# georgesterpu/avsr-tf1

Measured on AMD Instinct MI355X. Metric: utterances/sec (train step) at B=64 T_a=500 T_v=75, higher is better.
Workload: dtype f32; 1 GPU; c4: AV dual-attention (bimodal) video 1x256 + audio 3x256 uni-LSTM, scaled_luong, B=64 T_a=500x80 T_v=75 L=40; utterances_per_gpu=64, global_batch=64, T_a=500, F_a=80, T_v=75, F_v=128, T_dec=40, parallelism=dp1, video_frontend=resnet_cnn, launch=hipgraph, dropout=True

## Files before the change

### avsr-tf1_amd/_lib.py

```python
import ctypes as C
import os

import torch

from . import build as _build

MAX_LAYERS = 4
MAX_MECH = 4
MAX_STACKS = 4

_fp = C.POINTER(C.c_float)
_ip = C.POINTER(C.c_int32)


class AvsrError(RuntimeError):
    pass


class Mat(C.Structure):
    _fields_ = [("ptr", C.c_void_p), ("ld", C.c_int64), ("T", C.c_int32), ("pad_", C.c_int32), ("ldo", C.c_int64)]


class GemmDesc(C.Structure):
    _fields_ = [("A", Mat), ("B", Mat), ("C", Mat), ("bias", C.c_void_p),
                ("M", C.c_int32), ("N", C.c_int32), ("K", C.c_int32),
                ("trans_a", C.c_int32), ("trans_b", C.c_int32),
                ("alpha", C.c_float), ("beta", C.c_float), ("batch", C.c_int32),
                ("stride_a", C.c_int64), ("stride_b", C.c_int64), ("stride_c", C.c_int64),
                ("alpha_dev", C.c_void_p),
                ("splitk", C.c_int32), ("pad_", C.c_int32),
                ("workspace", C.c_void_p), ("workspace_floats", C.c_int64),
                ("colsum", C.c_void_p), ("colsum_beta", C.c_float), ("pad2_", C.c_int32)]


class RnnLayer(C.Structure):
    _fields_ = [("units", C.c_int32), ("in_dim", C.c_int32), ("hoisted", C.c_int32), ("out_col", C.c_int32),
                ("wt", C.c_void_p), ("w", C.c_void_p), ("bias", C.c_void_p),
                ("gates", C.c_void_p), ("cs", C.c_void_p), ("out", C.c_void_p), ("ld_out", C.c_int64),
                ("state", C.c_void_p), ("h_final", C.c_void_p), ("c_final", C.c_void_p),
                ("dgates", C.c_void_p), ("dstate", C.c_void_p), ("dout", C.c_void_p), ("ld_dout", C.c_int64),
                ("dout_col", C.c_int32), ("residual", C.c_int32), ("hs_seq", C.c_void_p), ("xt_seq", C.c_void_p),
                ("wt2", C.c_void_p), ("w2", C.c_void_p), ("bias2", C.c_void_p), ("rh_seq", C.c_void_p), ("dgates2", C.c_void_p)]


class RnnStack(C.Structure):
    _fields_ = [("B", C.c_int32), ("T", C.c_int32), ("reverse", C.c_int32), ("n_layers", C.c_int32),
                ("cell", C.c_int32), ("pad_", C.c_int32),
                ("len", C.c_void_p), ("dh_final", C.c_void_p), ("dc_final", C.c_void_p),
                ("seed", C.c_void_p), ("keep_in", C.c_float), ("keep_state", C.c_float), ("keep_out", C.c_float),
                ("consumer_keep", C.c_float), ("cell_id_base", C.c_int32), ("consumer_stream", C.c_int32),
                ("consumer_width", C.c_int32), ("pad2_", C.c_int32),
                ("layer", RnnLayer * MAX_LAYERS)]


class RnnLaunch(C.Structure):
    _fields_ = [(n, C.c_int32) for n in ("form", "stacks", "rows_per_group", "rows_per_slice", "launches", "wg_per_xcd", "crossing_edges",
                                         "top_tiles")]


class AttnMech(C.Structure):
    _fields_ = [("type", C.c_int32), ("T", C.c_int32), ("D", C.c_int32), ("chunk", C.c_int32),
                ("len", C.c_void_p), ("keys", C.c_void_p), ("values", C.c_void_p),
                ("values_sb", C.c_int64), ("values_st", C.c_int64),
                ("g", C.c_void_p), ("v", C.c_void_p), ("bq", C.c_void_p),
                ("wq_t", C.c_void_p), ("wq", C.c_void_p), ("watt_t", C.c_void_p), ("watt", C.c_void_p),
                ("scores", C.c_void_p), ("ctx", C.c_void_p), ("pq", C.c_void_p), ("pstat", C.c_void_p),
                ("pctx", C.c_void_p), ("dscores", C.c_void_p), ("dctx", C.c_void_p), ("dpq", C.c_void_p),
                ("pdq", C.c_void_p)]


class DecLayer(C.Structure):
    _fields_ = [("wt", C.c_void_p), ("w", C.c_void_p), ("bias", C.c_void_p), ("gates", C.c_void_p), ("cs", C.c_void_p),
                ("out", C.c_void_p), ("state", C.c_void_p), ("hs_seq", C.c_void_p), ("xin_seq", C.c_void_p),
                ("dgates", C.c_void_p), ("dstate", C.c_void_p), ("cell_id", C.c_int32), ("pad_", C.c_int32),
                ("wt2", C.c_void_p), ("w2", C.c_void_p), ("bias2", C.c_void_p), ("rh_seq", C.c_void_p), ("dgates2", C.c_void_p)]


MAX_DEC_EXTRA = 3


class AttnRnn(C.Structure):
    _fields_ = [("B", C.c_int32), ("L", C.c_int32), ("H", C.c_int32), ("E", C.c_int32),
                ("n_mech", C.c_int32), ("output_attention", C.c_int32), ("V", C.c_int32), ("mode", C.c_int32),
                ("go_id", C.c_int32), ("eos_id", C.c_int32),
                ("steplen", C.c_void_p), ("wt", C.c_void_p), ("w", C.c_void_p), ("bias", C.c_void_p),
                ("gates", C.c_void_p), ("cs", C.c_void_p), ("cell_out", C.c_void_p), ("att", C.c_void_p),
                ("h0", C.c_void_p), ("c0", C.c_void_p), ("state", C.c_void_p),
                ("h_final", C.c_void_p), ("c_final", C.c_void_p),
                ("mech", AttnMech * MAX_MECH),
                ("embedding", C.c_void_p), ("wout_t", C.c_void_p), ("bout", C.c_void_p),
                ("logits", C.c_void_p), ("ids", C.c_void_p), ("tok", C.c_void_p), ("n_unfinished", C.c_void_p),
                ("dgates", C.c_void_p), ("dstate", C.c_void_p), ("datt", C.c_void_p), ("dq", C.c_void_p),
                ("datt_ext", C.c_void_p), ("dcell_ext", C.c_void_p), ("dh0", C.c_void_p), ("dc0", C.c_void_p),
                ("dh_final", C.c_void_p), ("dc_final", C.c_void_p),
                ("seed", C.c_void_p), ("keep_in", C.c_float), ("keep_state", C.c_float), ("keep_out", C.c_float),
                ("sampling_prob", C.c_float), ("cell_id", C.c_int32), ("pad3_", C.c_int32),
                ("hs_seq", C.c_void_p), ("attd", C.c_void_p), ("xs", C.c_void_p), ("labels", C.c_void_p), ("fed", C.c_void_p),
                ("cell", C.c_int32), ("pad4_", C.c_int32), ("wt2", C.c_void_p), ("w2", C.c_void_p), ("bias2", C.c_void_p),
                ("rh_seq", C.c_void_p), ("dgates2", C.c_void_p),
                ("beam_width", C.c_int32), ("mem_shared", C.c_int32), ("length_penalty", C.c_float), ("pad6_", C.c_float),
                ("beam_logp", C.c_void_p), ("beam_fin", C.c_void_p), ("beam_len", C.c_void_p), ("step_ids", C.c_void_p),
                ("parent_ids", C.c_void_p), ("parent_rows", C.c_void_p),
                ("n_extra", C.c_int32), ("prof_tag", C.c_int32), ("out0", C.c_void_p), ("extra", DecLayer * MAX_DEC_EXTRA),
                ("fused_ws", C.c_void_p), ("fused_ws_floats", C.c_int64)]


MAX_LM_LAYERS = 4


class BeamLm(C.Structure):
    _fields_ = [("n_layers", C.c_int32), ("H", C.c_int32), ("E", C.c_int32), ("V", C.c_int32),
                ("one_hot", C.c_int32), ("n_rows", C.c_int32), ("lm_weight", C.c_float), ("pad_", C.c_int32),
                ("embedding", C.c_void_p), ("wt", C.c_void_p * MAX_LM_LAYERS), ("bias", C.c_void_p * MAX_LM_LAYERS),
                ("wout_t", C.c_void_p), ("bout", C.c_void_p), ("state_c", C.c_void_p), ("state_h", C.c_void_p), ("lm_logp", C.c_void_p)]


BEAM_CTC_MAX_T, BEAM_CTC_MAX_V = 2048, 256


class BeamCtc(C.Structure):
    _fields_ = [("n_utt", C.c_int32), ("beam_width", C.c_int32), ("T", C.c_int32), ("V", C.c_int32), ("eos_id", C.c_int32),
                ("weight", C.c_float), ("ld", C.c_int64)] + \
               [(n, C.c_void_p) for n in ("z", "in_len", "y", "state", "psi", "last", "term", "extra", "lm_logp")] + \
               [("lm_weight", C.c_float), ("pad_", C.c_int32)]


class ConvDesc(C.Structure):
    _fields_ = [(n, C.c_int32) for n in ("N", "H", "W", "Ci", "Co", "k", "stride", "pad_t", "pad_l", "Ho", "Wo", "pad_")] + \
               [("bn_scale", C.c_void_p), ("bn_shift", C.c_void_p)]


class ConvLaunch(C.Structure):
    _fields_ = [(n, C.c_int32) for n in ("kernel", "m", "ntc", "ch4", "rs", "fold", "ep", "nsp", "ntap", "t0", "F", "grid", "CsP", "lds_bytes",
                                         "slab", "pad_")]


class Conv3dDesc(C.Structure):
    _fields_ = [(n, C.c_int32) for n in ("B", "T", "H", "W", "Ci", "Co", "kt", "kh", "kw", "stride", "pad_f", "pad_t", "pad_l", "Ho", "Wo",
                                         "relu")] + [("scale", C.c_void_p), ("shift", C.c_void_p)]


class LogmelArgs(C.Structure):
    _fields_ = [(n, C.c_int32) for n in ("B", "N", "T_out", "F", "frame_length", "frame_step", "fft_length", "num_mel_bins", "window", "stride",
                                         "mel_nnz", "pad_")] + \
               [(n, C.c_void_p) for n in ("wav", "wav_len", "hann", "twiddle", "mel_lo", "mel_cnt", "mel_ptr", "mel_w", "out", "out_len")]


SPEC_AUGMENT_MAX_MASKS, SPEC_AUGMENT_MAX_T = 8, 65535


class SpecAugmentArgs(C.Structure):
    _fields_ = [(n, C.c_int32) for n in ("B", "T", "F_in", "F", "freq_masks", "freq_width", "freq_bins", "time_masks", "time_width",
                                         "ratio_q16", "video", "mean_fill")] + [("ld", C.c_int64)] + \
               [(n, C.c_void_p) for n in ("x", "len", "seed", "y", "ws")] + [("ws_floats", C.c_int64)]


class CtcArgs(C.Structure):
    _fields_ = [("B", C.c_int32), ("T", C.c_int32), ("L", C.c_int32), ("C", C.c_int32), ("ld", C.c_int64)] + \
               [(n, C.c_void_p) for n in ("z", "labels", "labels_len", "in_len", "denom")] + [("weight", C.c_float), ("pad_", C.c_int32)] + \
               [(n, C.c_void_p) for n in ("nll", "status", "utt_loss", "dz", "ws")] + [("ws_floats", C.c_int64)]


CTC_PREFIX_MAX_V, CTC_PREFIX_MAX_W, CTC_PREFIX_MAX_L = 256, 64, 512


class CtcPrefixArgs(C.Structure):
    _fields_ = [(n, C.c_int32) for n in ("B", "T", "V", "beam_width", "L_max", "pad_")] + [("ld", C.c_int64)] + \
               [(n, C.c_void_p) for n in ("z", "in_len", "ids", "lens", "score", "trace_parent", "trace_sym", "trace_pb", "trace_pnb")]


CTC_PREFIX_LM_MAX_W = 16


class CtcPrefixLm(C.Structure):
    _fields_ = [(n, C.c_int32) for n in ("n_layers", "H", "E", "V", "one_hot", "go_id", "eos_id")] + \
               [("weight", C.c_float), ("bonus", C.c_float), ("pad_", C.c_int32), ("embedding", C.c_void_p),
                ("wt", C.c_void_p * MAX_LM_LAYERS), ("bias", C.c_void_p * MAX_LM_LAYERS), ("wout_t", C.c_void_p), ("bout", C.c_void_p),
                ("ws", C.c_void_p), ("ws_bytes", C.c_int64), ("s_lm", C.c_void_p), ("lm_steps", C.c_void_p), ("lm_logp", C.c_void_p)]


CTC_PREFIX_NGRAM_MAX_ORDER = 16
CTC_PREFIX_NGRAM_MAX_NODES = 1 << 24
CTC_PREFIX_NGRAM_MAX_ARCS = 1 << 26


class CtcPrefixNgram(C.Structure):
    _fields_ = [(n, C.c_int32) for n in ("n_nodes", "n_arcs", "V", "start", "go_id", "eos_id")] + \
               [("weight", C.c_float), ("bonus", C.c_float)] + \
               [(n, C.c_void_p) for n in ("bow", "backoff", "arc_begin", "sym", "logp", "next", "s_lm", "lm_steps", "lm_logp")]


CTC_ALIGN_MAX_L = 512


class CtcAlignArgs(C.Structure):
    _fields_ = [(n, C.c_int32) for n in ("B", "T", "L", "V")] + [("ld", C.c_int64)] + \
               [(n, C.c_void_p) for n in ("z", "labels", "target_len", "in_len", "score", "status", "path", "frame_lp", "start", "end", "ws")] + \
               [("ws_bytes", C.c_int64)]


class ColsumJob(C.Structure):
    _fields_ = [("a", Mat), ("b", Mat), ("out", C.c_void_p), ("rows", C.c_int32), ("F", C.c_int32), ("alpha", C.c_float), ("beta", C.c_float)]


class TransposeJob(C.Structure):
    _fields_ = [("src", C.c_void_p), ("dst", C.c_void_p), ("rows", C.c_int32), ("cols", C.c_int32)]


_STRUCTS = {"avsr_dec_layer": DecLayer, "avsr_mat": Mat, "avsr_gemm_desc": GemmDesc, "avsr_rnn_layer": RnnLayer, "avsr_rnn_stack": RnnStack,
            "avsr_rnn_launch": RnnLaunch,
            "avsr_conv_desc": ConvDesc, "avsr_conv_launch": ConvLaunch, "avsr_conv3d_desc": Conv3dDesc, "avsr_logmel_args": LogmelArgs, "avsr_spec_augment_args": SpecAugmentArgs, "avsr_ctc_args": CtcArgs, "avsr_attn_mech": AttnMech, "avsr_attn_rnn": AttnRnn, "avsr_transpose_job": TransposeJob,
            "avsr_colsum_job": ColsumJob, "avsr_beam_lm": BeamLm, "avsr_beam_ctc": BeamCtc, "avsr_ctc_prefix_args": CtcPrefixArgs,
            "avsr_ctc_prefix_lm": CtcPrefixLm, "avsr_ctc_prefix_ngram": CtcPrefixNgram,
            "avsr_ctc_align_args": CtcAlignArgs}

_vp, _i32, _i64, _f32 = C.c_void_p, C.c_int32, C.c_int64, C.c_float
_SIGS = {
    "avsr_gemm": [C.POINTER(GemmDesc), _vp],
    "avsr_gemm_batch": [C.POINTER(GemmDesc), _i32, _vp],
    "avsr_rnn_fwd": [C.POINTER(RnnStack), _i32, _vp],
    "avsr_rnn_bwd": [C.POINTER(RnnStack), _i32, _vp],
    "avsr_rnn_set_persistent": [_vp, _i64],
    "avsr_rnn_set_persistent_mode": [_i32],
    "avsr_rnn_set_persistent_scratch": [_vp, _i64],
    "avsr_rnn_plan": [C.POINTER(RnnStack), _i32, _i32, _i32, _i64, _i64, C.POINTER(RnnLaunch), _i32],
    "avsr_attn_rnn_fwd": [C.POINTER(AttnRnn), _i32, _i32, _vp],
    "avsr_attn_rnn_fused_eligible": [C.POINTER(AttnRnn)],
    "avsr_attn_rnn_fused_fwd_active": [C.POINTER(AttnRnn)],
    "avsr_attn_rnn_set_fused": [_i32],
    "avsr_attn_rnn_set_beam_kernel": [_i32],
    "avsr_conv_set_mfma": [_i32],
    "avsr_conv_supported": [C.POINTER(ConvDesc)],
    "avsr_conv_fwd": [C.POINTER(ConvDesc), _vp, _vp, _vp, _vp, _vp, _vp, _vp, _vp, C.POINTER(_i32), _vp],
    "avsr_conv_bwd_data": [C.POINTER(ConvDesc), _vp, _vp, _vp, _f32, _vp],
    "avsr_conv_bwd_weight": [C.POINTER(ConvDesc), _vp, _vp, _vp, _vp, _f32, _vp, _i64, _vp],
    "avsr_conv_bwd_data_bn": [C.POINTER(ConvDesc), _vp, _vp, _vp, _f32, _vp, _vp, _vp, _vp, _vp, C.POINTER(_i32), _vp],
    "avsr_conv_bwd_data_bn_supported": [C.POINTER(ConvDesc)],
    "avsr_conv_bwd_weight_bn": [C.POINTER(ConvDesc), _vp, _vp, _vp, _vp, _vp, _vp, _vp, _f32, _vp, _i64, _vp],
    "avsr_conv_bwd_weight_bn_supported": [C.POINTER(ConvDesc)],
    "avsr_conv_plan": [C.POINTER(ConvDesc), _i32, _i32, _i64, C.POINTER(ConvLaunch), _i32],
    "avsr_bn_bwd_finalize": [_vp, _i32, _i32, _i64, _vp, _vp, _vp, _vp, _vp, _f32, _vp, _vp],
    "avsr_bn_bwd_apply": [_vp, _vp, _vp, _vp, _i64, _i32, _f32, _vp],
    "avsr_bn_bwd_stage1": [_vp, _vp, _vp, _vp, _vp, _vp, _i64, _i32, _vp, C.POINTER(_i32), _vp],
    "avsr_bn_partials_f64": [_vp, _i32, _i32, _vp, _vp],
    "avsr_bn_finalize_f64": [_vp, _i32, _f32, _f32, _vp, _vp, _vp, _vp, _vp, _vp, _vp, _vp, _vp],
    "avsr_bn_bwd_finalize_f64": [_vp, _vp, _i32, _vp, _vp, _vp, _vp, _vp, _f32, _vp, _vp],
    "avsr_bn_eval_affine": [_vp, _vp, _vp, _vp, _f32, _vp, _vp, _i32, _vp],
    "avsr_bn_finalize": [_vp, _i32, _i32, _i64, _f32, _f32, _vp, _vp, _vp, _vp, _vp, _vp, _vp, _vp, _vp],
    "avsr_conv3d_supported": [C.POINTER(Conv3dDesc)],
    "avsr_conv3d_fwd": [C.POINTER(Conv3dDesc), _vp, _vp, _vp, _vp, _vp, _vp, _vp, C.POINTER(_i32), _vp],
    "avsr_conv3d_bwd_data": [C.POINTER(Conv3dDesc), _vp, _vp, _vp, _f32, _vp],
    "avsr_conv3d_bwd_weight": [C.POINTER(Conv3dDesc), _vp, _vp, _vp, _f32, _vp, _i64, _vp],
    "avsr_conv3d_bn_finalize": [_vp, _i32, _i32, _i64, _f32, _f32, _vp, _vp, _vp, _vp, _vp, _vp, _vp, _vp, _vp],
    "avsr_logmel_supported": [_i32, _i32, _i32, _i32, _i32],
    "avsr_logmel_fwd": [C.POINTER(LogmelArgs), _vp],
    "avsr_spec_augment_supported": [_i32, _i32, _i32, _i32, _i32],
    "avsr_spec_augment": [C.POINTER(SpecAugmentArgs), _vp],
    "avsr_ctc_loss": [C.POINTER(CtcArgs), _vp],
    "avsr_ctc_best_path": [_vp, _i64, _vp, _i32, _i32, _i32, _vp, _vp],
    "avsr_ctc_prefix_search_supported": [_i32, _i32, _i32],
    "avsr_ctc_prefix_search": [C.POINTER(CtcPrefixArgs), _vp],
    "avsr_ctc_prefix_lm_supported": [_i32, _i32, _i32, _i32, _i32, _i32, _i32],
    "avsr_ctc_prefix_search_lm": [C.POINTER(CtcPrefixArgs), C.POINTER(CtcPrefixLm), _vp],
    "avsr_ctc_prefix_ngram_supported": [_i32, _i32, _i32, _i32, _i32],
    "avsr_ctc_prefix_search_ngram": [C.POINTER(CtcPrefixArgs), C.POINTER(CtcPrefixNgram), _vp],
    "avsr_ctc_align_supported": [_i32, _i32],
    "avsr_ctc_align": [C.POINTER(CtcAlignArgs), _vp],
    "avsr_seq_logprob": [_vp, _vp, _vp, _i32, _i32, _i32, _vp, _i64, _vp],
    "avsr_rescore_select": [_vp, _vp, _vp, _i32, _i32, _f32, _vp, _vp, _vp],
    "avsr_batchnorm_apply": [_vp, _vp, _i32, _i32, _vp, _vp, _vp, _vp, _i32, _vp],
    "avsr_attn_rnn_bwd": [C.POINTER(AttnRnn), _vp],
    "avsr_beam_gather_tree": [_vp, _vp, _vp, _vp, _i32, _i32, _i32, _i32, _vp],
    "avsr_beam_search_step": [_vp, _i32, _i32, _i32, _i32, _i32, _f32, _vp, _vp, _vp, _vp, _vp, _vp, _vp, _vp, _vp, _vp, _vp, _vp, _i64, _i32, _vp, _vp, _vp],
    "avsr_beam_lm_supported": [C.POINTER(BeamLm)],
    "avsr_beam_lm_step": [C.POINTER(BeamLm), _vp, _vp, _i32, _i32, _vp],
    "avsr_beam_search_step_lm": [_vp, _i32, _i32, _i32, _i32, _i32, _f32, _vp, _vp, _vp, _vp, _vp, _vp, _vp, _vp, _vp, _vp, _vp, _vp, _i64, _i32, _vp, _vp,
                                 _vp, _f32, _vp],
    "avsr_attn_rnn_fwd_lm": [C.POINTER(AttnRnn), C.POINTER(BeamLm), _i32, _i32, _vp],
    "avsr_beam_ctc_supported": [C.POINTER(BeamCtc)],
    "avsr_beam_ctc_begin": [C.POINTER(BeamCtc), _vp],
    "avsr_beam_ctc_step": [C.POINTER(BeamCtc), _vp, _vp, _vp, _i32, _vp],
    "avsr_beam_search_step_ctc": [_vp, _i32, _i32, _i32, _i32, _i32, _f32, _vp, _vp, _vp, _vp, _vp, _vp, _vp, _vp, _vp, _vp, _vp, _vp, _i64, _i32, _vp, _vp,
                                  _vp, _f32, _vp, _f32, _vp, _vp],
    "avsr_attn_rnn_fwd_ctc": [C.POINTER(AttnRnn), C.POINTER(BeamLm), C.POINTER(BeamCtc), _i32, _i32, _vp],
    "avsr_attn_alpha_rows": [_vp, _vp, _vp, _vp, _vp, _vp, _i32, _i32, _i32, _vp],
    "avsr_bahdanau_dkeys": [_vp, _vp, _i64, _i64, _vp, _vp, _vp, _vp, _vp, _vp, _i32, _i32, _i32, _i32, _vp],
    "avsr_transpose": [C.POINTER(TransposeJob), _i32, _vp],
    "avsr_colsum": [C.POINTER(Mat), C.POINTER(Mat), _i32, _i32, _f32, _f32, _vp, _vp, _i64, _vp],
    "avsr_batchnorm_fwd": [_vp, _vp, _i32, _i32, _vp, _vp, _vp, _vp, _vp, _vp, _i32, _vp, _i64, _vp],
    "avsr_batchnorm_xhat": [_vp, _vp, _vp, _vp, _i32, _i32, _vp],
    "avsr_batchnorm_fwd_ex": [_vp, _vp, _i32, _i32, _vp, _vp, _vp, _vp, _vp, _vp, _i32, _f32, _f32, _i32, _i32, _vp, _i64, _vp],
    "avsr_batchnorm_bwd": [_vp, _vp, _vp, _vp, _vp, _vp, _vp, _vp, _vp, _i32, _i32, _i32, _f32, _vp, _i64, _vp],
    "avsr_im2col": [_vp, _vp, _i32, _i32, _i32, _i32, _i32, _i32, _i32, _i32, _i32, _i32, _i32, _vp],
    "avsr_col2im": [_vp, _vp, _i32, _i32, _i32, _i32, _i32, _i32, _i32, _i32, _i32, _i32, _i32, _f32, _vp],
    "avsr_relu": [_vp, _vp, _i64, _vp],
    "avsr_relu_bwd": [_vp, _vp, _vp, _i64, _vp],
    "avsr_add": [_vp, _vp, _vp, _i64, _vp],
    "avsr_selu": [_vp, _vp, _i64, _vp],
    "avsr_selu_bwd": [_vp, _vp, _vp, _i64, _vp],
    "avsr_conv3x3_supported": [_i32, _i32, _i32, _i32],
    "avsr_conv3x3": [_vp, _vp, _vp, _vp, _i32, _i32, _i32, _i32, _i32, _i32, _i32, _i32, _i32, _i32, _i32, _f32, _vp],
    "avsr_conv3x3_bwd_data_s2": [_vp, _vp, _vp, _i32, _i32, _i32, _i32, _i32, _i32, _i32, _i32, _i32, _f32, _vp],
    "avsr_conv3x3_bwd_weight": [_vp, _vp, _vp, _i32, _i32, _i32, _i32, _i32, _i32, _i32, _i32, _i32, _i32, _f32, _vp, _i64, _vp],
    "avsr_embed_labels": [_vp, _vp, _i32, _vp, _vp, _i32, _i32, _i32, _i32, _vp],
    "avsr_embed_grad": [_vp, _vp, _vp, _i32, _i32, _i32, _i32, _vp, _i64, _vp],
    "avsr_dropout_rows": [C.POINTER(Mat), C.POINTER(Mat), _i32, _i32, _vp, _i32, _f32, _i32, _i32, _i32, _vp],
    "avsr_seq_loss": [_vp, _vp, _vp, _vp, _i32, _vp, _vp, _i32, _i32, _i32, _vp],
    "avsr_seq_loss_fun": [_vp, _vp, _vp, _vp, _i32, _vp, _vp, _i32, _i32, _i32, _i32, _f32, _vp],
    "avsr_au_loss": [_vp, _vp, _vp, _vp, _vp, _i32, _i32, _f32, _vp],
    "avsr_au_loss_dp": [_vp, _vp, _vp, _vp, _vp, _i32, _i32, _f32, _vp, _vp],
    "avsr_normed_v": [_vp, _vp, _vp, _i32, _vp],
    "avsr_normed_v_bwd": [_vp, _vp, _vp, _vp, _vp, _i32, _vp],
    "avsr_reduce_scalar": [_vp, _i32, _vp, _i32, _i32, _f32, _vp],
    "avsr_l2_regularise": [C.POINTER(_i64), C.POINTER(_i64), _i32, _vp, _vp, _f32, _vp, _vp, _vp],
    "avsr_global_norm": [_vp, _i64, _f32, _vp, _vp, _vp],
    "avsr_adam_step": [_vp, _vp, _vp, _vp, _i64, _vp, _vp, _f32, _i32, _f32, _f32, _vp],
    "avsr_batchnorm_sync_sum": [_vp, _i32, _i32, _vp, _vp, _i64, _vp],
    "avsr_batchnorm_sync_sqsum": [_vp, _i32, _i32, _vp, _vp, _vp, _vp, _vp, _i64, _vp],
    "avsr_batchnorm_sync_apply": [_vp, _vp, _i32, _i32, _vp, _vp, _vp, _vp, _vp, _vp, _vp, _vp, _f32, _f32, _i32, _vp],
    "avsr_batchnorm_sync_moments": [_vp, _i32, _i32, _vp, _vp, _i64, _vp],
    "avsr_dp_sync_unpack": [_vp, _vp, _i32, C.POINTER(_i32), C.POINTER(_i32), C.POINTER(_vp), C.POINTER(_vp), C.POINTER(_vp), _vp],
    "avsr_seq_loss_per_utterance": [_vp, _vp, _vp, _vp, _i32, _i32, _vp],
    "avsr_instnorm_fwd": [_vp, _vp, _i32, _i32, _i32, _vp, _vp, _vp, _vp, _f32, _vp],
    "avsr_instnorm_bwd": [_vp, _vp, _vp, _vp, _vp, _vp, _vp, _vp, _i32, _i32, _i32, _vp],
    "avsr_optimiser_step": [_vp, _vp, _vp, _vp, _i64, _vp, _vp, _f32, _i32, _i32, _f32, _f32, _i32, _f32, _vp],
    "avsr_highway_fwd": [_vp, _vp, _vp, _vp, _vp, _i32, _i32, _i32, _vp],
    "avsr_highway_bwd": [_vp, _vp, _vp, _vp, _vp, _vp, _vp, _vp, _i32, _i32, _i32, _i32, _vp],
    "avsr_copy_words": [_vp, _vp, _i64, _vp],
    "avsr_zero_words": [_vp, _i64, _vp],
    "avsr_zero_multi": [C.POINTER(_vp), C.POINTER(_i64), _i32, _vp],
    "avsr_add_int": [_vp, _i32, _vp, _vp],
    "avsr_colsum_multi": [C.POINTER(ColsumJob), _i32, _vp, _i64, _vp],
    "avsr_slab_defer_begin": [], "avsr_slab_defer_end": [_vp],
    "avsr_adam_step_decay": [_vp, _vp, _vp, _vp, _i64, _vp, _vp, _f32, _i32, _i32, _f32, _f32, _vp],
    "avsr_prof_begin": [_i32],
    "avsr_prof_end": [C.POINTER(_i32), C.POINTER(_f32), C.POINTER(C.c_double)],
}
EXPORTS = ["avsr_abi_version", "avsr_sizeof", "avsr_attn_rnn_fused_ws_floats", "avsr_conv3d_wgrad_scratch_floats", "avsr_ctc_ws_floats",
           "avsr_ctc_align_ws_bytes", "avsr_ctc_prefix_lm_ws_bytes", "avsr_spec_augment_ws_floats"] + list(_SIGS)

_lib = None


def lib_path():
    return _build.LIB


def load():
    global _lib
    if _lib is not None:
        return _lib
    path = os.environ.get("AVSR_LIB") or _build.LIB
    if path == _build.LIB and _build.needs_build():
        try:
            _build.build()
        except Exception as e:
            if not os.path.exists(path):
                raise AvsrError("libavsr_hip.so is missing and could not be built: %s" % e)
    lib = C.CDLL(path)
    lib.avsr_abi_version.restype = C.c_int
    lib.avsr_sizeof.restype = C.c_int64
    lib.avsr_sizeof.argtypes = [C.c_char_p]
    for sym in EXPORTS:
        if not hasattr(lib, sym):
            raise AvsrError("libavsr_hip.so does not export %s" % sym)
    for name, at in _SIGS.items():
        fn = getattr(lib, name)
        fn.argtypes = at
        fn.restype = C.c_int
    lib.avsr_attn_rnn_fused_ws_floats.argtypes = [_i32, _i32, _i32]
    lib.avsr_attn_rnn_fused_ws_floats.restype = C.c_int64
    lib.avsr_conv3d_wgrad_scratch_floats.argtypes = [C.POINTER(Conv3dDesc)]
    lib.avsr_conv3d_wgrad_scratch_floats.restype = C.c_int64
    lib.avsr_ctc_ws_floats.argtypes = [_i32, _i32, _i32]
    lib.avsr_ctc_ws_floats.restype = C.c_int64
    lib.avsr_spec_augment_ws_floats.argtypes = [_i32, _i32, _i32]
    lib.avsr_spec_augment_ws_floats.restype = C.c_int64
    lib.avsr_ctc_align_ws_bytes.argtypes = [_i32, _i32, _i32]
    lib.avsr_ctc_align_ws_bytes.restype = C.c_int64
    lib.avsr_ctc_prefix_lm_ws_bytes.argtypes = [_i32, _i32, _i32, _i32]
    lib.avsr_ctc_prefix_lm_ws_bytes.restype = C.c_int64
    for name, st in _STRUCTS.items():
        n = lib.avsr_sizeof(name.encode())
        if n != C.sizeof(st):
            raise AvsrError("ABI mismatch for %s: C %d vs ctypes %d" % (name, n, C.sizeof(st)))
    _lib = lib
    return lib


def check(rc, what):
    if rc != 0:
        raise AvsrError("%s failed with code %d" % (what, rc))


def ptr(t):
    return None if t is None else t.data_ptr()


def stream_ptr():
    return torch.cuda.current_stream().cuda_stream
```

### avsr-tf1_amd/csrc/conv_mfma.h

```cpp
#pragma once
#include "common.h"
#include "persist.h"
#include "prof.h"
#include "avsr_hip.h"

namespace avsr {

__device__ __forceinline__ int fdiv(int n, unsigned magic) { return magic ? (int)__umulhi((unsigned)n, magic) : n; }
static inline unsigned fmagic(int d) { return d <= 1 ? 0u : (unsigned)(((1ull << 32) / (unsigned)d) + 1ull); }
__device__ __forceinline__ unsigned fmagic_dev(int d) { return d <= 1 ? 0u : (unsigned)(((1ull << 32) / (unsigned)d) + 1ull); }

template <class SrcOff, class DstOff>
__device__ __forceinline__ void stage4(const float* __restrict__ src, float* __restrict__ lds, int nf4, int tid, SrcOff so, DstOff dof) {
  for (int base = 0; base < nf4; base += 256 * 16) {
    f32x4 v[16];
#pragma unroll
    for (int u = 0; u < 16; ++u) {
      const int idx = base + u * 256 + tid;
      v[u] = idx < nf4 ? ld4(src + so(idx)) : f32x4{0.f, 0.f, 0.f, 0.f};
    }
#pragma unroll
    for (int u = 0; u < 16; ++u) {
      const int idx = base + u * 256 + tid;
      if (idx < nf4) st4(lds + dof(idx), v[u]);
    }
  }
}

__device__ __forceinline__ void stage_rows(const float* __restrict__ src, float* __restrict__ dst, int rows, int rq, int dst_pitch, int tid,
                                           int my_row, int my_p4, int rpp) {
  if (my_row < 0) return;
  const float* sp = src + ((long)my_row * rq + my_p4) * 4;
  float* dp = dst + my_row * dst_pitch + my_p4 * 4;
  const int sstep = rpp * rq * 4, dstep = rpp * dst_pitch;
  int r = my_row;
  while (r < rows) {
    f32x4 v[16];
#pragma unroll
    for (int u = 0; u < 16; ++u) v[u] = (r + u * rpp < rows) ? ld4(sp + u * sstep) : f32x4{0.f, 0.f, 0.f, 0.f};
#pragma unroll
    for (int u = 0; u < 16; ++u) if (r + u * rpp < rows) st4(dp + u * dstep, v[u]);
    r += 16 * rpp; sp += 16 * sstep; dp += 16 * dstep;
  }
}

#define CG_MAXTAP 16
#define CONV_MAX_PARTS 512
struct CGTap { int da, db; short w[4]; };
static inline CGTap cgtap1(int da, int db, int widx) { CGTap t; t.da = da; t.db = db; t.w[0] = (short)widx; t.w[1] = t.w[2] = t.w[3] = -1; return t; }
struct CGArgs {
  const float* src; const float* w; const float* bias; float* dst; float* stats;
  const float* acc;
  const float* res;
  const float* bn_sc; const float* bn_sh;
  const float* res_sc; const float* res_sh;
  const float* bnb_x; const float* bnb_sc; const float* bnb_sh;
  int N, SH, SW, Cs, CsL;
  int CsP;
  int DH, DW, Cd;
  int OA, OB, S, OS, oh0, ow0;
  int nsp, SB, OSA, OSB, lin;
  signed char sp_dh[4], sp_dw[4];
  int ntap, wmode, F;
  float beta;
  unsigned m_opf, m_ob, m_rq, m_per, m_sw;
  CGTap tap[CG_MAXTAP];
};


#define WG_PAD 2
#define WG_WPC(tiles) ((tiles) > 16 ? 1 : ((tiles) <= 3 ? 4 : ((tiles) <= 6 ? 3 : 2)))
struct WGArgs {
  const float* x; const float* dy; float* part;
  int N, H, W, Ci, CiL, Ho, Wo, Co, S, pt, pl, F;
  int SW;
  int pad;
  unsigned m_opf, m_wo, m_rq, m_per, m_w;
  int t0, nt, kw;
  int slab, want_bias;
  const float* bn_sc; const float* bn_sh;
  const float* fy; const float* fk; int fC; float* fdx;
};


extern int g_conv_mfma;

struct ConvPlanRec { avsr_conv_launch* out; int cap, n; };
extern thread_local ConvPlanRec* g_conv_plan;
static inline void conv_plan_note(const avsr_conv_launch& L) {
  ConvPlanRec* R = g_conv_plan;
  if (!R) return;
  if (R->n < R->cap) R->out[R->n] = L;
  ++R->n;
}

}

#define S_(x) ((hipStream_t)(x))

static inline int cg_frames(int sh, int sw, int csl, int opf, int extra_floats_per_frame = 0) {
  const long per = (long)(sh + 2) * (sw + 2) * csl + extra_floats_per_frame;
  int F = (int)((63 * 1024 / 4) / per);
  if (F < 1) F = 1;
  int want = (1024 + opf - 1) / opf;
  if (want < 1) want = 1;
  if (F > want) F = want;
  if (F > 16) F = 16;
  return F;
}

static inline bool cd_ok(const avsr_conv_desc* c) {
  return c && c->N > 0 && (c->k == 1 || c->k == 3) && (c->stride == 1 || c->stride == 2) && c->Co % 4 == 0 && (c->Ci % 4 == 0 || c->Ci < 4) &&
         c->Ci > 0 && c->Co > 0 && c->Co <= 64 && c->pad_t >= 0 && c->pad_t <= 1 && c->pad_l >= 0 && c->pad_l <= 1 && (c->k == 3 || (c->pad_t == 0 && c->pad_l == 0));
}

int conv_fwd_impl(const avsr_conv_desc* c, const float* x, const float* w, const float* bias, const float* res, const float* res_sc,
                  const float* res_sh, float* y, float* stats, int32_t* nparts, void* stream, bool dry);
int conv_bwd_data_impl(const avsr_conv_desc* c, const float* dy, const float* w, float* dx, float beta, void* stream, bool dry,
                       const float* acc = nullptr, const float* bnb_x = nullptr, const float* bnb_sc = nullptr,
                       const float* bnb_sh = nullptr, float* stats = nullptr, int32_t* nparts = nullptr);
int conv_bwd_weight_impl(const avsr_conv_desc* c, const float* x, const float* dy, float* dw, float* dbias, float beta, float* scratch,
                         long scratch_floats, void* stream, bool dry, const float* fold_y = nullptr, const float* fold_k = nullptr,
                         float* fold_dx = nullptr);
```

### avsr-tf1_amd/csrc/conv_mfma.hip

```cpp
#include "conv_mfma.h"

namespace avsr {

template <int MAXCH, bool CH4, int EP>
__global__ __launch_bounds__(256, 2) void conv_gen_kernel(const CGArgs A) {
  extern __shared__ __attribute__((aligned(16))) float lds[];
  const int tid = threadIdx.x, lane = tid & 63, wave = __builtin_amdgcn_readfirstlane(tid >> 6);
  const int i = lane & 15, q = lane >> 4;
  const int Cs = A.Cs, CsL = A.CsL, CsP = A.CsP, Cd = A.Cd, C4 = CsL >> 2;
  const int PH = A.SH + 2, PW = A.SW + 2, fstride = PH * PW * CsP;
  const int KQ = A.ntap * C4, nch = (KQ + 3) >> 2;
  const int NC = A.nsp * Cd;
  const int NT = (NC + 15) >> 4;
  const int nt = wave % NT, mslot = wave / NT, mstep = 4 / NT;
  const f32x4 zero4 = {0.f, 0.f, 0.f, 0.f};
  const bool lin = A.lin != 0;
  const int opf = A.OA * A.OB;
  const int pixf = A.DH * A.DW;
  const int rows_all = A.F * opf, rows_pad = ((rows_all + 15) >> 4) << 4;
  int* const rowtab = reinterpret_cast<int*>(lds + A.F * fstride);
  int* const dsttab = rowtab + rows_pad;
  int* const taptab = dsttab + rows_pad;
  const int tapword = reinterpret_cast<const int*>(A.tap)[tid & (CG_MAXTAP * 4 - 1)];

  for (int idx = tid; idx < A.F * fstride; idx += 256) lds[idx] = 0.f;
  if (tid < CG_MAXTAP * 4) taptab[tid] = tapword;
  for (int m = tid; m < rows_pad; m += 256) {
    int ro = 0, dt = 4;
    if (m < rows_all) {
      const int f = fdiv(m, A.m_opf), r = m - f * opf, a = fdiv(r, A.m_ob), b = r - a * A.OB;
      ro = f * fstride + ((a * A.S + 1) * PW + (b * A.SB + 1)) * CsP;
      const int ph = a * A.OSA + A.oh0, pw = b * A.OSB + A.ow0;
      dt = lin ? (m * NC) << 2
               : (ph < A.DH && pw < A.DW) ? ((((f * A.DH + ph) * A.DW + pw) * Cd) << 2) | (ph + 1 >= A.DH ? 1 : 0) | (pw + 1 >= A.DW ? 2 : 0) : 4;
    }
    rowtab[m] = ro;
    dsttab[m] = dt;
  }

  __syncthreads();
  const __amdgpu_buffer_rsrc_t w_rs = make_rsrc(A.w);
  f32x4 wreg[MAXCH];
  int koff[MAXCH];
  {
    const int cn = nt * 16 + i;
    const bool colok = cn < NC;
    const int sp = colok ? cn / Cd : 0, co = colok ? cn - sp * Cd : 0;
#pragma unroll
    for (int c = 0; c < MAXCH; ++c) {
      const int kq = 4 * c + q;
      const bool in = c < nch && kq < KQ;
      const int t = in ? kq / C4 : 0, cs4 = in ? kq - t * C4 : 0;
      const i32x4_ tp = *reinterpret_cast<const i32x4_*>(taptab + 4 * t);
      koff[c] = in ? (tp[0] * PW + tp[1]) * CsP + cs4 * 4 : 0;
      const int wpair = (sp & 2) ? tp[3] : tp[2];
      const int widx = (int)(short)((sp & 1) ? (wpair >> 16) : (wpair & 0xffff));
      f32x4 wv;
#pragma unroll
      for (int e = 0; e < 4; ++e) {
        const int cs = cs4 * 4 + e;
        const long wo = A.wmode ? ((long)widx * Cd + co) * Cs + cs : ((long)widx * Cs + cs) * Cd + co;
        wv[e] = ldb1(w_rs, (in && colok && widx >= 0 && cs < Cs) ? (int)(wo * 4) : P_OOB);
      }
      wreg[c] = wv;
    }
  }
  const int cD0 = nt * 16 + q * 4;
  const bool colok = cD0 < NC;
  const int spD = colok ? cD0 / Cd : 0, coD = colok ? cD0 - spD * Cd : 0;
  int sdh = 0, sdw = 0;
#pragma unroll
  for (int k = 0; k < 4; ++k) { sdh = (k == spD) ? (int)A.sp_dh[k] : sdh; sdw = (k == spD) ? (int)A.sp_dw[k] : sdw; }
  const f32x4 bias4 = (A.bias && colok) ? ld4(A.bias + coD) : zero4;
  const bool bnb = A.bnb_x != nullptr;
  const bool rbn = !bnb && A.res_sc != nullptr;
  const float* const e_map = bnb ? A.bnb_x : A.res;
  const float* const e_scp = bnb ? A.bnb_sc : A.res_sc;
  const float* const e_shp = bnb ? A.bnb_sh : A.res_sh;
  const f32x4 esc4 = ((bnb || rbn) && colok) ? ld4(e_scp + coD) : zero4;
  const f32x4 esh4 = ((bnb || rbn) && colok) ? ld4(e_shp + coD) : zero4;
  f32x4 ssum = zero4, ssq = zero4;
  const __amdgpu_buffer_rsrc_t e_rs = make_rsrc(e_map), dst_rs = make_rsrc(A.dst), acc_rs = make_rsrc(A.acc ? A.acc : A.dst);
  const int lane_o = lin ? cD0 * 4 : ((sdh * A.DW + sdw) * Cd + coD) * 4;

  const int st_rq = (A.SW * Cs) >> 2;
  const int st_rpp = st_rq > 0 ? (256 / st_rq > 0 ? 256 / st_rq : 1) : 1;
  const int st_row = (st_rq > 0 && st_rq <= 256) ? (tid < st_rpp * st_rq ? fdiv(tid, A.m_rq) : -1) : -1;
  const int st_p4 = st_row >= 0 ? tid - st_row * st_rq : 0;
  const int st_px = (CH4 && CsP != Cs) ? (st_p4 * 4) / Cs : 0;
  const int st_lo = (CH4 && CsP != Cs) ? st_px * CsP + (st_p4 * 4 - st_px * Cs) : st_p4 * 4;
  f32x4 bsc = {1.f, 1.f, 1.f, 1.f}, bsh = zero4;
  const bool bn_on = CH4 && A.bn_sc != nullptr;
  if (bn_on && st_row >= 0) { const int cb = (st_p4 * 4) % Cs; bsc = ld4(A.bn_sc + cb); bsh = ld4(A.bn_sh + cb); }
  const int rowf = A.SW * Cs;

  constexpr int PF = CH4 ? (MAXCH > 9 ? 10 : 12) : 4;
  f32x4 pre[PF];
  constexpr bool c4 = CH4;
  const int ppf = c4 ? (A.SH + st_rpp - 1) / st_rpp : 0;
  const unsigned m_ppf = fmagic_dev(ppf > 0 ? ppf : 1);
  const int per3 = A.SH * A.SW * Cs;
  const i32x4_ src_rs = make_rsrc_words(A.src);
  const int fs_per = A.N / (int)gridDim.x, fs_extra = A.N - fs_per * (int)gridDim.x;
  const int fs_cnt = fs_per + ((int)blockIdx.x < fs_extra ? 1 : 0), fs_np = (fs_cnt + A.F - 1) / A.F;
  const bool fs_rr = A.F == 1;
  const int FP = fs_rr ? 1 : (fs_np > 0 ? (fs_cnt + fs_np - 1) / fs_np : A.F);
  const int n_begin = fs_rr ? (int)blockIdx.x : (int)blockIdx.x * fs_per + min((int)blockIdx.x, fs_extra);
  const int n_end = fs_rr ? A.N : n_begin + fs_cnt, n_step = fs_rr ? (int)gridDim.x : FP;
  auto fetch = [&](int n0) {
    const int fcur = min(FP, n_end - n0);
    if (c4) {
#pragma unroll
      for (int u = 0; u < PF; ++u) {
        const int f = fdiv(u, m_ppf), k = u - f * ppf, r = st_row + k * st_rpp;
        ldb4_hidden(pre[u], src_rs, (st_row >= 0 && f < fcur && r < A.SH) ? (int)((((unsigned)(n0 + f) * A.SH + r) * rowf + st_p4 * 4) * 4u) : P_OOB);
      }
    } else {
      const unsigned so = (unsigned)n0 * per3 * 4u;
      const int tot4 = (fcur * per3) >> 2;
#pragma unroll
      for (int u = 0; u < PF; ++u) {
        const int idx = u * 256 + tid;
        ldb4_hidden(pre[u], src_rs, idx < tot4 ? (int)(so + idx * 16u) : P_OOB);
      }
    }
  };
  auto commit = [&](int n0) {
    const int fcur = min(FP, n_end - n0);
    vm_wait_all();
#pragma unroll
    for (int u = 0; u < PF; ++u) vm_landed(pre[u]);
    if (c4) {
#pragma unroll
      for (int u = 0; u < PF; ++u) {
        const int f = fdiv(u, m_ppf), k = u - f * ppf, r = st_row + k * st_rpp;
        if (st_row >= 0 && f < fcur && r < A.SH) {
          f32x4 v = pre[u];
          if (bn_on) {
#pragma unroll
            for (int e = 0; e < 4; ++e) v[e] = fmaxf(fmaf(v[e], bsc[e], bsh[e]), 0.f);
          }
          st4(lds + f * fstride + ((r + 1) * PW + 1) * CsP + st_lo, v);
        }
      }
    } else {
      const int tot = fcur * per3, tot4 = tot >> 2;
      auto put = [&](int e, float v) {
        const int f = fdiv(e, A.m_per), r = e - f * per3, px = fdiv(r, A.m_rq), c = r - px * Cs, h = fdiv(px, A.m_sw), pw = px - h * A.SW;
        lds[f * fstride + ((h + 1) * PW + pw + 1) * CsP + c] = v;
      };
#pragma unroll
      for (int u = 0; u < PF; ++u) {
        const int idx = u * 256 + tid;
        if (idx < tot4) { put(idx * 4, pre[u][0]); put(idx * 4 + 1, pre[u][1]); put(idx * 4 + 2, pre[u][2]); put(idx * 4 + 3, pre[u][3]); }
      }
      const float* sp = A.src + (long)n0 * per3;
      for (int e = tot4 * 4 + tid; e < tot; e += 256) put(e, sp[e]);
    }
  };
  int n0 = n_begin;
  if (n0 < n_end) fetch(n0);
  for (; n0 < n_end; n0 += n_step) {
    const int fcur = min(FP, n_end - n0);
    __syncthreads();
    commit(n0);
    __syncthreads();
    if (n0 + n_step < n_end) fetch(n0 + n_step);
    const int Mtot = fcur * opf, mtiles = (Mtot + 15) >> 4;
    const unsigned pass_o = (unsigned)((long)n0 * pixf * Cd * 4);
    constexpr int CB = MAXCH <= 6 ? MAXCH : 3;
    constexpr bool XT = MAXCH <= 6;
    f32x4 bufa[CB], bufb[CB];
    const int last = mtiles - 1;
    int rb_cur = rowtab[(mslot < mtiles ? mslot : 0) * 16 + i];
    int rb_nxt = rowtab[(mslot + mstep < mtiles ? mslot + mstep : (last > 0 ? last : 0)) * 16 + i];
    int dt_cur = dsttab[(mslot < mtiles ? mslot : 0) * 16 + i];
    if (XT && mslot < mtiles) {
#pragma unroll
      for (int c = 0; c < CB; ++c) bufa[c] = ld4(lds + rb_cur + koff[c]);
    }
    typedef unsigned int u32x4_ __attribute__((ext_vector_type(4)));
    auto epilogue = [&](const f32x4 a0, const f32x4 a1, const int dbo, const bool ok, const f32x4 ev, const f32x4 ov) {
      f32x4 v = (a0 + a1) + bias4;
      if ((EP & 1) && !bnb) {
        if (rbn) {
#pragma unroll
          for (int r = 0; r < 4; ++r) v[r] += fmaxf(fmaf(ev[r], esc4[r], esh4[r]), 0.f);
        } else v += ev;
      }
      if (EP & 2) v += A.beta * ov;
      if ((EP & 1) && bnb) {
#pragma unroll
        for (int r = 0; r < 4; ++r) v[r] = fmaf(ev[r], esc4[r], esh4[r]) > 0.f ? v[r] : 0.f;
      }
      __builtin_amdgcn_raw_buffer_store_b128(__builtin_bit_cast(u32x4_, v), dst_rs, dbo, 0, 0);
      const f32x4 vs = ok ? v : zero4;
      ssum += vs;
      ssq += ((EP & 1) && bnb) ? vs * ev : vs * vs;
    };
    auto dest = [&](const int mt, const int dt, bool& ok) {
      const int bad = (dt & 4) | ((dt & 1) & sdh) | (((dt >> 1) & 1) & sdw);
      ok = (mt * 16 + i < Mtot) & colok & (bad == 0);
      return (int)(pass_o + (unsigned)((dt & ~15) + lane_o)) | (ok ? 0 : P_OOB);
    };
    auto tile = [&](f32x4 (&cur)[CB], f32x4 (&nxt)[CB], const int mt) {
      const int t1 = mt + mstep < mtiles ? mt + mstep : last;
      const int dt_nxt = dsttab[t1 * 16 + i];
      const float* base = lds + rb_cur;
      bool ok;
      const int dbo = dest(mt, dt_cur, ok);
      f32x4 ev = zero4, ov = zero4;
      if (EP & 1) ev = ldb4(e_rs, dbo);
      if (EP & 2) ov = ldb4(acc_rs, dbo);
      f32x4 acc0 = zero4, acc1 = zero4;
#pragma unroll
      for (int c = 0; c < CB; ++c) cur[c] = ld4(base + koff[c]);
#pragma unroll
      for (int b0 = 0; b0 < MAXCH; b0 += CB) {
#pragma unroll
        for (int c = 0; c < CB; ++c)
          if (b0 + CB + c < MAXCH) nxt[c] = ld4(base + koff[b0 + CB + c]);
        __builtin_amdgcn_sched_barrier(0);
#pragma unroll
        for (int c = 0; c < CB; ++c)
          if (b0 + c < MAXCH) {
#pragma unroll
            for (int e = 0; e < 4; ++e) {
              if (e & 1) acc1 = __builtin_amdgcn_mfma_f32_16x16x4f32(wreg[b0 + c][e], cur[c][e], acc1, 0, 0, 0);
              else acc0 = __builtin_amdgcn_mfma_f32_16x16x4f32(wreg[b0 + c][e], cur[c][e], acc0, 0, 0, 0);
              __builtin_amdgcn_sched_barrier(0x7F6);
            }
          }
        __builtin_amdgcn_sched_barrier(0);
#pragma unroll
        for (int c = 0; c < CB; ++c) cur[c] = nxt[c];
      }
      epilogue(acc0, acc1, dbo, ok, ev, ov);
      rb_cur = rb_nxt;
      rb_nxt = rowtab[(mt + 2 * mstep < mtiles ? mt + 2 * mstep : last) * 16 + i];
      dt_cur = dt_nxt;
    };
    f32x4 pa0 = zero4, pa1 = zero4, pev = zero4, pov = zero4;
    int pdbo = P_OOB, poki = 0;
    auto tile_x = [&](f32x4 (&cur)[CB], f32x4 (&nxt)[CB], const int mt) {
      const int t1 = mt + mstep < mtiles ? mt + mstep : last, t2 = mt + 2 * mstep < mtiles ? mt + 2 * mstep : last;
      int rb_nn = 0, dt_nxt = 0, dbo = P_OOB, oki = 0;
      bool ok = false;
      f32x4 ev = zero4, ov = zero4, v = zero4, vs = zero4, acc0 = zero4, acc1 = zero4;
      constexpr int W_RD = 1, W_DEST = W_RD + CB, W_EPI = W_DEST + 2, NWORK = W_EPI + 9, NM = 4 * MAXCH;
      auto work = [&](const int k) {
        if (k == 0) { rb_nn = rowtab[t2 * 16 + i]; dt_nxt = dsttab[t1 * 16 + i]; }
        else if (k < W_DEST) {
          nxt[k - W_RD] = ld4(lds + rb_nxt + koff[k - W_RD]);
        } else if (k == W_DEST) {
          dbo = dest(mt, dt_cur, ok);
          oki = ok ? 1 : 0;
          asm volatile("" : "+v"(dbo), "+v"(oki));
        }
        else if (k == W_DEST + 1) {
          if (EP & 1) ev = ldb4(e_rs, dbo);
          if (EP & 2) ov = ldb4(acc_rs, dbo);
        }
        else if (k == W_EPI) v = pa0 + pa1;
        else if (k == W_EPI + 1) v += bias4;
        else if (k == W_EPI + 2) {
          if ((EP & 1) && !bnb) {
            if (rbn) { v[0] += fmaxf(fmaf(pev[0], esc4[0], esh4[0]), 0.f); v[1] += fmaxf(fmaf(pev[1], esc4[1], esh4[1]), 0.f); }
            else v += pev;
          }
        } else if (k == W_EPI + 3) {
          if ((EP & 1) && !bnb && rbn) { v[2] += fmaxf(fmaf(pev[2], esc4[2], esh4[2]), 0.f); v[3] += fmaxf(fmaf(pev[3], esc4[3], esh4[3]), 0.f); }
        } else if (k == W_EPI + 4) {
          if (EP & 2) v += A.beta * pov;
        } else if (k == W_EPI + 5) {
          if ((EP & 1) && bnb) {
#pragma unroll
            for (int r = 0; r < 4; ++r) v[r] = fmaf(pev[r], esc4[r], esh4[r]) > 0.f ? v[r] : 0.f;
          }
        } else if (k == W_EPI + 6) {
          __builtin_amdgcn_raw_buffer_store_b128(__builtin_bit_cast(u32x4_, v), dst_rs, pdbo, 0, 0);
        } else if (k == W_EPI + 7) { vs = poki != 0 ? v : zero4; ssum += vs; }
        else if (k == W_EPI + 8) ssq += ((EP & 1) && bnb) ? vs * pev : vs * vs;
      };
#pragma unroll
      for (int k = 0; k < NM; ++k) {
        const int c = k >> 2, e = k & 3;
        if (e & 1) acc1 = __builtin_amdgcn_mfma_f32_16x16x4f32(wreg[c][e], cur[c][e], acc1, 0, 0, 0);
        else acc0 = __builtin_amdgcn_mfma_f32_16x16x4f32(wreg[c][e], cur[c][e], acc0, 0, 0, 0);
        if (k < NWORK) work(k);
        __builtin_amdgcn_sched_barrier(0);
      }
#pragma unroll
      for (int k = NM; k < NWORK; ++k) work(k);
      pa0 = acc0; pa1 = acc1; pdbo = dbo; poki = oki; pev = ev; pov = ov;
      rb_cur = rb_nxt; rb_nxt = rb_nn; dt_cur = dt_nxt;
    };
    if (XT) {
      for (int mt = mslot; mt < mtiles; mt += 2 * mstep) {
        tile_x(bufa, bufb, mt);
        if (mt + mstep < mtiles) tile_x(bufb, bufa, mt + mstep);
        else break;
      }
      epilogue(pa0, pa1, pdbo, poki != 0, pev, pov);
    } else {
      for (int mt = mslot; mt < mtiles; mt += mstep) tile(bufa, bufb, mt);
    }
  }
  if (A.stats) {
    __syncthreads();
#pragma unroll
    for (int r = 0; r < 4; ++r) { ssum[r] = group16_sum(ssum[r]); ssq[r] = group16_sum(ssq[r]); }
    float* red = lds;
    if (i == 0) {
#pragma unroll
      for (int r = 0; r < 4; ++r) { red[((wave * 4 + q) * 2) * 4 + r] = ssum[r]; red[((wave * 4 + q) * 2 + 1) * 4 + r] = ssq[r]; }
    }
    __syncthreads();
    if (tid < Cd) {
      float s = 0.f, s2 = 0.f;
      for (int w = 0; w < 4; ++w)
        for (int qq = 0; qq < 4; ++qq)
          for (int r = 0; r < 4; ++r) {
            const int cD = (w % NT) * 16 + qq * 4 + r;
            if (cD < NC && cD % Cd == tid) { s += red[((w * 4 + qq) * 2) * 4 + r]; s2 += red[((w * 4 + qq) * 2 + 1) * 4 + r]; }
          }
      A.stats[(long)blockIdx.x * 2 * Cd + tid] = s;
      A.stats[(long)blockIdx.x * 2 * Cd + Cd + tid] = s2;
    }
  }
}

template <int NTAP, int C4T, bool CH4, int EP>
__global__ __launch_bounds__(256, 2) void conv_q4_kernel(const CGArgs A) {
  extern __shared__ __attribute__((aligned(16))) float lds[];
  const int tid = threadIdx.x, lane = tid & 63, wave = __builtin_amdgcn_readfirstlane(tid >> 6);
  constexpr int NQ = NTAP * C4T, NA = (4 * NQ + 15) / 16, MAXCH = 6;
  const int Cs = A.Cs, CsL = A.CsL;
  constexpr int Cd = 8;
  const int PH = A.SH + 2, PW = A.SW + 2, fstride = PH * PW * CsL;
  const f32x4 zero4 = {0.f, 0.f, 0.f, 0.f};
  const int opf = A.OA * A.OB, pixf = A.DH * A.DW;
  const int rows_all = A.F * opf, rows_pad = ((rows_all + 63) >> 6) << 6;
  int* const rowtab = reinterpret_cast<int*>(lds + A.F * fstride);
  int* const taptab = rowtab + rows_pad;
  const int tapword = reinterpret_cast<const int*>(A.tap)[tid & (CG_MAXTAP * 4 - 1)];
  for (int idx = tid; idx < A.F * fstride; idx += 256) lds[idx] = 0.f;
  if (tid < CG_MAXTAP * 4) taptab[tid] = tapword;
  for (int m = tid; m < rows_pad; m += 256) {
    int ro = ((PW + 1) * CsL) | (1 << 24);
    if (m < rows_all) {
      const int f = fdiv(m, A.m_opf), r = m - f * opf, a = fdiv(r, A.m_ob), b = r - a * A.OB;
      ro = (f * fstride + ((a + 1) * PW + (b + 1)) * CsL) | ((b + 1) << 24);
    }
    rowtab[m] = ro;
  }
  __syncthreads();
  float wA[2][NA];
  {
    const int bb = lane >> 2, i = lane & 3;
    const __amdgpu_buffer_rsrc_t w_rs = make_rsrc(A.w);
#pragma unroll
    for (int a = 0; a < NA; ++a) {
      const int k = 16 * a + bb, kq = k >> 2, e = k & 3;
      const bool in = kq < NQ;
      const int t = in ? kq / C4T : 0, cs = (kq - t * C4T) * 4 + e;
      const int widx = in ? (int)(short)(taptab[4 * t + 2] & 0xffff) : -1;
#pragma unroll
      for (int h = 0; h < 2; ++h) {
        const int co = 4 * h + i;
        const long wo = A.wmode ? ((long)widx * Cd + co) * Cs + cs : ((long)widx * Cs + cs) * Cd + co;
        wA[h][a] = ldb1(w_rs, (in && widx >= 0 && cs < Cs) ? (int)(wo * 4) : P_OOB);
      }
    }
  }
  int koff[NQ];
#pragma unroll
  for (int t = 0; t < NTAP; ++t) {
#pragma unroll
    for (int c = 0; c < C4T; ++c) koff[t * C4T + c] = (A.tap[t].da * PW + A.tap[t].db) * CsL;
  }
  const f32x4 bias0 = A.bias ? ld4(A.bias) : zero4, bias1 = A.bias ? ld4(A.bias + 4) : zero4;
  const bool bnb = A.bnb_x != nullptr;
  const bool rbn = !bnb && A.res_sc != nullptr;
  const float* const e_map = bnb ? A.bnb_x : A.res;
  const float* const e_scp = bnb ? A.bnb_sc : A.res_sc;
  const float* const e_shp = bnb ? A.bnb_sh : A.res_sh;
  const f32x4 esc0 = (bnb || rbn) ? ld4(e_scp) : zero4, esc1 = (bnb || rbn) ? ld4(e_scp + 4) : zero4;
  const f32x4 esh0 = (bnb || rbn) ? ld4(e_shp) : zero4, esh1 = (bnb || rbn) ? ld4(e_shp + 4) : zero4;
  f32x4 ssum0 = zero4, ssum1 = zero4, ssq0 = zero4, ssq1 = zero4;
  const __amdgpu_buffer_rsrc_t e_rs = make_rsrc(e_map), dst_rs = make_rsrc(A.dst), acc_rs = make_rsrc(A.acc ? A.acc : A.dst);
  typedef unsigned int u32x4_ __attribute__((ext_vector_type(4)));

  const int st_rq = (A.SW * Cs) >> 2;
  const int st_rpp = st_rq > 0 ? (256 / st_rq > 0 ? 256 / st_rq : 1) : 1;
  const int st_row = (st_rq > 0 && st_rq <= 256) ? (tid < st_rpp * st_rq ? fdiv(tid, A.m_rq) : -1) : -1;
  const int st_p4 = st_row >= 0 ? tid - st_row * st_rq : 0;
  f32x4 bsc = {1.f, 1.f, 1.f, 1.f}, bsh = zero4;
  const bool bn_on = CH4 && A.bn_sc != nullptr;
  if (bn_on && st_row >= 0) { const int cb = (st_p4 * 4) % Cs; bsc = ld4(A.bn_sc + cb); bsh = ld4(A.bn_sh + cb); }
  const int rowf = A.SW * Cs;

  constexpr int PF = CH4 ? 12 : 4;
  f32x4 pre[PF];
  constexpr bool c4 = CH4;
  const int ppf = c4 ? (A.SH + st_rpp - 1) / st_rpp : 0;
  const unsigned m_ppf = fmagic_dev(ppf > 0 ? ppf : 1);
  const int per3 = A.SH * A.SW * Cs;
  const i32x4_ src_rs = make_rsrc_words(A.src);
  const int fs_per = A.N / (int)gridDim.x, fs_extra = A.N - fs_per * (int)gridDim.x;
  const int fs_cnt = fs_per + ((int)blockIdx.x < fs_extra ? 1 : 0), fs_np = (fs_cnt + A.F - 1) / A.F;
  const bool fs_rr = A.F == 1;
  const int FP = fs_rr ? 1 : (fs_np > 0 ? (fs_cnt + fs_np - 1) / fs_np : A.F);
  const int n_begin = fs_rr ? (int)blockIdx.x : (int)blockIdx.x * fs_per + min((int)blockIdx.x, fs_extra);
  const int n_end = fs_rr ? A.N : n_begin + fs_cnt, n_step = fs_rr ? (int)gridDim.x : FP;
  auto fetch = [&](int n0) {
    const int fcur = min(FP, n_end - n0);
    if (c4) {
#pragma unroll
      for (int u = 0; u < PF; ++u) {
        const int f = fdiv(u, m_ppf), k = u - f * ppf, r = st_row + k * st_rpp;
        ldb4_hidden(pre[u], src_rs, (st_row >= 0 && f < fcur && r < A.SH) ? (int)((((unsigned)(n0 + f) * A.SH + r) * rowf + st_p4 * 4) * 4u) : P_OOB);
      }
    } else {
      const unsigned so = (unsigned)n0 * per3 * 4u;
      const int tot4 = (fcur * per3) >> 2;
#pragma unroll
      for (int u = 0; u < PF; ++u) {
        const int idx = u * 256 + tid;
        ldb4_hidden(pre[u], src_rs, idx < tot4 ? (int)(so + idx * 16u) : P_OOB);
      }
    }
  };
  auto commit = [&](int n0) {
    const int fcur = min(FP, n_end - n0);
    vm_wait_all();
#pragma unroll
    for (int u = 0; u < PF; ++u) vm_landed(pre[u]);
    if (c4) {
#pragma unroll
      for (int u = 0; u < PF; ++u) {
        const int f = fdiv(u, m_ppf), k = u - f * ppf, r = st_row + k * st_rpp;
        if (st_row >= 0 && f < fcur && r < A.SH) {
          f32x4 v = pre[u];
          if (bn_on) {
#pragma unroll
            for (int e = 0; e < 4; ++e) v[e] = fmaxf(fmaf(v[e], bsc[e], bsh[e]), 0.f);
          }
          const int px1 = 1 + (st_p4 >> 1), qd = (st_p4 & 1) ^ (C4T == 2 ? (px1 >> 2) & 1 : 0);
          st4(lds + f * fstride + ((r + 1) * PW) * CsL + (C4T == 2 ? px1 * 8 + qd * 4 : 4 + st_p4 * 4), v);
        }
      }
    } else {
      const int tot = fcur * per3, tot4 = tot >> 2;
      auto put = [&](int e, float v) {
        const int f = fdiv(e, A.m_per), r = e - f * per3, px = fdiv(r, A.m_rq), c = r - px * Cs, h = fdiv(px, A.m_sw), pw = px - h * A.SW;
        lds[f * fstride + ((h + 1) * PW + pw + 1) * CsL + c] = v;
      };
#pragma unroll
      for (int u = 0; u < PF; ++u) {
        const int idx = u * 256 + tid;
        if (idx < tot4) { put(idx * 4, pre[u][0]); put(idx * 4 + 1, pre[u][1]); put(idx * 4 + 2, pre[u][2]); put(idx * 4 + 3, pre[u][3]); }
      }
      const float* sp = A.src + (long)n0 * per3;
      for (int e = tot4 * 4 + tid; e < tot; e += 256) put(e, sp[e]);
    }
  };
  int n0 = n_begin;
  if (n0 < n_end) fetch(n0);
  for (; n0 < n_end; n0 += n_step) {
    const int fcur = min(FP, n_end - n0);
    __syncthreads();
    commit(n0);
    __syncthreads();
    if (n0 + n_step < n_end) fetch(n0 + n_step);
    const int Mtot = fcur * opf, mtiles = (Mtot + 63) >> 6;
    const unsigned pass_o = (unsigned)((long)n0 * pixf * Cd * 4);
    constexpr int NH = (NQ + 1) / 2;
    f32x4 xq[NQ];
    int h0[3], h1[3];
    auto window = [&](const int rt) {
      const int rb = rt & 0xffffff, bcol = rt >> 24;
#pragma unroll
      for (int d = 0; d < 3; ++d) {
        const int o = C4T == 2 ? (((bcol + d - 1) >> 2) & 1) << 2 : 0;
        h0[d] = rb + o; h1[d] = rb + 4 - o;
      }
      if (A.wmode) { const int x0 = h0[0]; h0[0] = h0[2]; h0[2] = x0; const int x1 = h1[0]; h1[0] = h1[2]; h1[2] = x1; }
    };
#define Q4C_LD(KQ_) xq[KQ_] = ld4(lds + (((KQ_) % C4T ? h1[((KQ_) / C4T) % 3] : h0[((KQ_) / C4T) % 3]) + koff[KQ_]));
#define Q4C_E(KQ_, E_)                                                                                              \
        acc0 = __builtin_amdgcn_mfma_f32_4x4x1f32(wA[0][(4 * (KQ_) + (E_)) >> 4], x4[E_], acc0, 4, (4 * (KQ_) + (E_)) & 15, 0);   \
        acc1 = __builtin_amdgcn_mfma_f32_4x4x1f32(wA[1][(4 * (KQ_) + (E_)) >> 4], x4[E_], acc1, 4, (4 * (KQ_) + (E_)) & 15, 0);
#define Q4C_MFMA(KQ_) { const f32x4 x4 = xq[KQ_]; Q4C_E(KQ_, 0) Q4C_E(KQ_, 1) Q4C_E(KQ_, 2) Q4C_E(KQ_, 3) }
    int rt_cur = rowtab[(wave < mtiles ? wave : 0) * 64 + lane];
    window(rt_cur);
    if constexpr (NQ == 18) { Q4C_LD(0) Q4C_LD(1) Q4C_LD(2) Q4C_LD(3) Q4C_LD(4) Q4C_LD(5) Q4C_LD(6) Q4C_LD(7) Q4C_LD(8) } else { Q4C_LD(0) Q4C_LD(1) Q4C_LD(2) Q4C_LD(3) Q4C_LD(4) }
    for (int mt = wave; mt < mtiles; mt += 4) {
      const int rt_nxt = rowtab[(mt + 4 < mtiles ? mt + 4 : mt) * 64 + lane];
      const int m = mt * 64 + lane;
      const bool ok = m < Mtot;
      const int dbo = (int)(pass_o + (unsigned)(m * 32)) | (ok ? 0 : P_OOB);
      f32x4 ev0 = zero4, ev1 = zero4, ov0 = zero4, ov1 = zero4;
      if (EP & 1) { ev0 = ldb4(e_rs, dbo); ev1 = ldb4(e_rs, dbo | 16); }
      if (EP & 2) { ov0 = ldb4(acc_rs, dbo); ov1 = ldb4(acc_rs, dbo | 16); }
      f32x4 acc0 = zero4, acc1 = zero4;
      if constexpr (NQ == 18) { Q4C_LD(9) Q4C_LD(10) Q4C_LD(11) Q4C_LD(12) Q4C_LD(13) Q4C_LD(14) Q4C_LD(15) Q4C_LD(16) Q4C_LD(17) } else { Q4C_LD(5) Q4C_LD(6) Q4C_LD(7) Q4C_LD(8) }
      __builtin_amdgcn_sched_barrier(0);
      if constexpr (NQ == 18) { Q4C_MFMA(0) Q4C_MFMA(1) Q4C_MFMA(2) Q4C_MFMA(3) Q4C_MFMA(4) Q4C_MFMA(5) Q4C_MFMA(6) Q4C_MFMA(7) Q4C_MFMA(8) } else { Q4C_MFMA(0) Q4C_MFMA(1) Q4C_MFMA(2) Q4C_MFMA(3) Q4C_MFMA(4) }
      __builtin_amdgcn_sched_barrier(0);
      window(rt_nxt);
      if constexpr (NQ == 18) { Q4C_LD(0) Q4C_LD(1) Q4C_LD(2) Q4C_LD(3) Q4C_LD(4) Q4C_LD(5) Q4C_LD(6) Q4C_LD(7) Q4C_LD(8) } else { Q4C_LD(0) Q4C_LD(1) Q4C_LD(2) Q4C_LD(3) Q4C_LD(4) }
      __builtin_amdgcn_sched_barrier(0);
      if constexpr (NQ == 18) { Q4C_MFMA(9) Q4C_MFMA(10) Q4C_MFMA(11) Q4C_MFMA(12) Q4C_MFMA(13) Q4C_MFMA(14) Q4C_MFMA(15) Q4C_MFMA(16) Q4C_MFMA(17) } else { static_assert(NQ == 9, "3x3 taps, 4- or 8-channel sources"); Q4C_MFMA(5) Q4C_MFMA(6) Q4C_MFMA(7) Q4C_MFMA(8) }
      __builtin_amdgcn_sched_barrier(0);
      f32x4 v0 = acc0 + bias0, v1 = acc1 + bias1;
      if ((EP & 1) && !bnb) {
        if (rbn) {
#pragma unroll
          for (int r = 0; r < 4; ++r) { v0[r] += fmaxf(fmaf(ev0[r], esc0[r], esh0[r]), 0.f); v1[r] += fmaxf(fmaf(ev1[r], esc1[r], esh1[r]), 0.f); }
        } else { v0 += ev0; v1 += ev1; }
      }
      if (EP & 2) { v0 += A.beta * ov0; v1 += A.beta * ov1; }
      if ((EP & 1) && bnb) {
#pragma unroll
        for (int r = 0; r < 4; ++r) {
          v0[r] = fmaf(ev0[r], esc0[r], esh0[r]) > 0.f ? v0[r] : 0.f;
          v1[r] = fmaf(ev1[r], esc1[r], esh1[r]) > 0.f ? v1[r] : 0.f;
        }
      }
      __builtin_amdgcn_raw_buffer_store_b128(__builtin_bit_cast(u32x4_, v0), dst_rs, dbo, 0, 0);
      __builtin_amdgcn_raw_buffer_store_b128(__builtin_bit_cast(u32x4_, v1), dst_rs, dbo | 16, 0, 0);
      const f32x4 s0 = ok ? v0 : zero4, s1 = ok ? v1 : zero4;
      ssum0 += s0; ssum1 += s1;
      ssq0 += ((EP & 1) && bnb) ? s0 * ev0 : s0 * s0;
      ssq1 += ((EP & 1) && bnb) ? s1 * ev1 : s1 * s1;
    }
  }
#undef Q4C_LD
#undef Q4C_MFMA
#undef Q4C_E
  if (A.stats) {
    __syncthreads();
    float* red = lds;
#pragma unroll
    for (int r = 0; r < 4; ++r) {
      const float a0 = wave_sum(ssum0[r]), a1 = wave_sum(ssum1[r]), q0 = wave_sum(ssq0[r]), q1 = wave_sum(ssq1[r]);
      if (lane == 0) { red[wave * 16 + r] = a0; red[wave * 16 + 4 + r] = a1; red[wave * 16 + 8 + r] = q0; red[wave * 16 + 12 + r] = q1; }
    }
    __syncthreads();
    if (tid < 16) A.stats[(long)blockIdx.x * 2 * Cd + tid] = (red[tid] + red[16 + tid]) + (red[32 + tid] + red[48 + tid]);
  }
}

int g_conv_mfma = 1;
thread_local ConvPlanRec* g_conv_plan = nullptr;

}

using namespace avsr;

extern "C" int avsr_conv_set_mfma(int32_t on) { g_conv_mfma = on ? 1 : 0; return AVSR_OK; }

static bool cg_q4_ok(const CGArgs& A, int ntaps) {
  return A.Cd == 8 && A.S == 1 && A.OS == 1 && !A.oh0 && !A.ow0 && A.DH == A.OA && A.DW == A.OB && ntaps == 9 &&
         (A.Cs == 8 || A.Cs == 3) && A.SW + 1 < 256;
}
static bool cg_q4_taps_ok(const CGArgs& A) {
  for (int t = 0; t < 9; ++t)
    if (A.tap[t].db != (A.wmode ? 1 - t % 3 : t % 3 - 1)) return false;
  return true;
}
static int cg_dry(const CGArgs& A, int kernel, int m, int c4t, int grid, size_t lds) {
  if (!g_conv_plan) return grid;
  if (A.res && A.bnb_x) return AVSR_ERR_ARG;
  const int ep = ((A.res || A.bnb_x) ? 1 : 0) | (A.beta != 0.f ? 2 : 0);
  if (A.Cs % 4 && ep) return AVSR_ERR_UNSUPPORTED;
  avsr_conv_launch L = {};
  L.kernel = kernel; L.m = m; L.ntc = c4t; L.ch4 = A.Cs % 4 == 0; L.ep = ep; L.nsp = A.nsp; L.ntap = A.ntap; L.F = A.F; L.grid = grid;
  L.CsP = kernel == 0 ? A.CsP : A.CsL; L.lds_bytes = (int32_t)lds;
  conv_plan_note(L);
  return grid;
}
static int cg_launch_q4(CGArgs& A, hipStream_t s, int kind, double flops, bool dry) {
  int Fcap = 16;
  if (A.Cs == 8) {
    const int rq = A.SW * A.Cs / 4;
    if (rq > 256 || rq < 1) return AVSR_ERR_UNSUPPORTED;
    const int rpp = 256 / rq;
    Fcap = 12 / ((A.SH + rpp - 1) / rpp);
    A.m_rq = fmagic(rq); A.m_per = fmagic(A.SH * rq); A.m_sw = fmagic(A.SW);
  } else {
    Fcap = (4 * 256 * 4) / (A.SH * A.SW * A.Cs);
    while (Fcap > 0 && (long)Fcap * A.SH * A.SW * A.Cs >= 65536) --Fcap;
    A.m_rq = fmagic(A.Cs); A.m_per = fmagic(A.SH * A.SW * A.Cs); A.m_sw = fmagic(A.SW);
  }
  if (Fcap < 1) return AVSR_ERR_UNSUPPORTED;
  if ((long)A.N * A.DH * A.DW * A.Cd * 4 >= (1L << 31) || (long)A.N * A.SH * A.SW * A.Cs * 4 >= (1L << 31)) return AVSR_ERR_UNSUPPORTED;
  A.m_opf = fmagic(A.OA * A.OB); A.m_ob = fmagic(A.OB);
  const int opf = A.OA * A.OB;
  const size_t frame_b = sizeof(float) * (size_t)(A.SH + 2) * (A.SW + 2) * A.CsL;
  auto lds_bytes = [&](int F) { return F * frame_b + 4 * ((((size_t)F * opf + 63) / 64) * 64) + sizeof(CGTap) * CG_MAXTAP; };
  double best = -1.0;
  int bestF = 0;
  for (int F = (Fcap < 16 ? Fcap : 16); F >= 1; --F) {
    if (lds_bytes(F) > 64 * 1024 || (long)F * frame_b / 4 >= (1 << 14) * 4 || (long)F * opf >= (1 << 24)) continue;
    const long units = (A.N + F - 1) / F, grid = units < CONV_MAX_PARTS ? units : CONV_MAX_PARTS;
    const long cnt = (A.N + grid - 1) / grid, np = (cnt + F - 1) / F, fp = (cnt + np - 1) / np;
    const long tiles = (fp * opf + 63) / 64, per_wave = (tiles + 3) / 4;
    const double cost = (double)np * (double)(per_wave * 8 + 4);
    if (best < 0.0 || cost < 0.97 * best) { best = cost; bestF = F; }
  }
  if (!bestF) return AVSR_ERR_UNSUPPORTED;
  A.F = bestF;
  size_t lds = lds_bytes(A.F);
  if (lds < 256) lds = 256;
  int grid = (A.N + A.F - 1) / A.F;
  if (grid > CONV_MAX_PARTS) grid = CONV_MAX_PARTS;
  if (dry) return cg_dry(A, 1, 9, A.Cs == 3 ? 1 : 2, grid, lds);
  ProfScope ps(kind, s, flops);
  const bool emap = A.res != nullptr || A.bnb_x != nullptr;
  if (A.res && A.bnb_x) return AVSR_ERR_ARG;
  const int ep = (emap ? 1 : 0) | (A.beta != 0.f ? 2 : 0);
  if (A.Cs == 3) {
    if (ep) return AVSR_ERR_UNSUPPORTED;
    hipLaunchKernelGGL((conv_q4_kernel<9, 1, false, 0>), dim3(grid), dim3(256), lds, s, A);
  } else switch (ep) {
    case 0: hipLaunchKernelGGL((conv_q4_kernel<9, 2, true, 0>), dim3(grid), dim3(256), lds, s, A); break;
    case 1: hipLaunchKernelGGL((conv_q4_kernel<9, 2, true, 1>), dim3(grid), dim3(256), lds, s, A); break;
    case 2: hipLaunchKernelGGL((conv_q4_kernel<9, 2, true, 2>), dim3(grid), dim3(256), lds, s, A); break;
    default: hipLaunchKernelGGL((conv_q4_kernel<9, 2, true, 3>), dim3(grid), dim3(256), lds, s, A); break;
  }
  if (hipGetLastError() != hipSuccess) return AVSR_ERR_HIP;
  return grid;
}

static int cg_launch(CGArgs& A, hipStream_t s, int kind, double flops, bool dry = false) {
  if (A.nsp == 0) {
    A.nsp = 1; A.SB = A.S; A.OSA = A.OS; A.OSB = A.OS;
    A.lin = (A.OS == 1 && A.oh0 == 0 && A.ow0 == 0 && A.DH == A.OA && A.DW == A.OB) ? 1 : 0;
  }
  if (cg_q4_ok(A, A.ntap) && A.nsp == 1 && A.lin && cg_q4_taps_ok(A)) return cg_launch_q4(A, s, kind, flops, dry);
  const int KQ = A.ntap * (A.CsL / 4), nch = (KQ + 3) / 4;
  const int NT = (A.nsp * A.Cd + 15) / 16;
  if (!(NT == 1 || NT == 2 || NT == 4) || nch > 20) return AVSR_ERR_UNSUPPORTED;
  if (A.Cs % 4 && nch > 5) return AVSR_ERR_UNSUPPORTED;
  int Fcap = 16;
  if (A.Cs % 4 == 0) {
    const int rq = A.SW * A.Cs / 4;
    if (rq > 256 || rq < 1) return AVSR_ERR_UNSUPPORTED;
    const int rpp = 256 / rq, pfmax = nch > 9 ? 10 : 12;
    Fcap = pfmax / ((A.SH + rpp - 1) / rpp);
    A.m_rq = fmagic(rq); A.m_per = fmagic(A.SH * rq); A.m_sw = fmagic(A.SW);
  } else {
    Fcap = (4 * 256 * 4) / (A.SH * A.SW * A.Cs);
    while (Fcap > 0 && (long)Fcap * A.SH * A.SW * A.Cs >= 65536) --Fcap;
    A.m_rq = fmagic(A.Cs); A.m_per = fmagic(A.SH * A.SW * A.Cs); A.m_sw = fmagic(A.SW);
  }
  if (Fcap < 1) return AVSR_ERR_UNSUPPORTED;
  if ((long)A.N * A.DH * A.DW * A.Cd * 4 >= (1L << 31)) return AVSR_ERR_UNSUPPORTED;
  if ((long)A.N * A.SH * A.SW * A.Cs * 4 >= (1L << 31)) return AVSR_ERR_UNSUPPORTED;
  A.m_opf = fmagic(A.OA * A.OB); A.m_ob = fmagic(A.OB);
  const int opf = A.OA * A.OB, mstep = 4 / NT;
  A.CsP = A.CsL;
  if (A.Cs % 4 == 0) {
    for (int p = 0; p < 4; ++p)
      if ((A.SB * (A.CsL / 4 + p)) % 4 == 2) { A.CsP = A.CsL + 4 * p; break; }
  }
  size_t frame_b = sizeof(float) * (size_t)(A.SH + 2) * (A.SW + 2) * A.CsP;
  auto lds_bytes = [&](int F) {
    const size_t rows_pad = (((size_t)F * opf + 15) / 16) * 16;
    return F * frame_b + 4 * rows_pad * 2 + sizeof(CGTap) * CG_MAXTAP;
  };
  auto pick = [&](size_t budget, int slots) {
    double best = -1.0;
    int bestF = 0;
    for (int F = (Fcap < 16 ? Fcap : 16); F >= 1; --F) {
      if (lds_bytes(F) > budget || (long)F * opf >= 65536) continue;
      const long units = (A.N + F - 1) / F, grid = units < slots ? units : slots;
      const long cnt = (A.N + grid - 1) / grid, np = (cnt + F - 1) / F, fp = (cnt + np - 1) / np;
      const long tiles = (fp * opf + 15) / 16, per_wave = (tiles + mstep - 1) / mstep;
      const double cost = (double)np * (double)(per_wave * 8 + 16);
      if (best < 0.0 || cost < 0.97 * best) { best = cost; bestF = F; }
    }
    return bestF;
  };
  A.F = pick(64 * 1024, CONV_MAX_PARTS);
  if (!A.F && A.CsP != A.CsL) {
    A.CsP = A.CsL;
    frame_b = sizeof(float) * (size_t)(A.SH + 2) * (A.SW + 2) * A.CsP;
    A.F = pick(64 * 1024, CONV_MAX_PARTS);
  }
  if (!A.F) return AVSR_ERR_UNSUPPORTED;
  size_t lds = lds_bytes(A.F);
  if (lds < sizeof(float) * 4 * 4 * 2 * 4) lds = sizeof(float) * 4 * 4 * 2 * 4;
  int grid = (A.N + A.F - 1) / A.F;
  if (grid > CONV_MAX_PARTS) grid = CONV_MAX_PARTS;
  if (dry) return cg_dry(A, 0, A.Cs % 4 ? 5 : (nch <= 2 ? 2 : (nch <= 6 ? 6 : (nch <= 9 ? 9 : (nch <= 18 ? 18 : 20)))), 0, grid, lds);
  ProfScope ps(kind, s, flops);
  const bool emap = A.res != nullptr || A.bnb_x != nullptr;
  if (A.res && A.bnb_x) return AVSR_ERR_ARG;
  const int ep = (emap ? 1 : 0) | (A.beta != 0.f ? 2 : 0);
  if (A.Cs % 4 && ep != 0) return AVSR_ERR_UNSUPPORTED;
#define CG_ONE(M_, C_, E_)                                                                                          \
  {                                                                                                                 \
    hipLaunchKernelGGL((conv_gen_kernel<M_, C_, E_>), dim3(grid), dim3(256), lds, s, A);                            \
  }
#define CG_GO(M_, C_)                                                                                              \
  switch (ep) {                                                                                                    \
    case 0: CG_ONE(M_, C_, 0) break;                                                                               \
    case 1: CG_ONE(M_, C_, 1) break;                                                                               \
    case 2: CG_ONE(M_, C_, 2) break;                                                                               \
    default: CG_ONE(M_, C_, 3) break;                                                                              \
  }
  if (A.Cs % 4) CG_ONE(5, false, 0)
  else if (nch <= 2) { CG_GO(2, true) }
  else if (nch <= 6) { CG_GO(6, true) }
  else if (nch <= 9) { CG_GO(9, true) }
  else if (nch <= 18) { CG_GO(18, true) }
  else if (nch <= 20) { CG_GO(20, true) }
  else return AVSR_ERR_UNSUPPORTED;
#undef CG_GO
#undef CG_ONE
  if (hipGetLastError() != hipSuccess) return AVSR_ERR_HIP;
  return grid;
}


static int cg_run(CGArgs A, const CGTap* taps, int ntaps, hipStream_t s, int kind, double flops_per_tap, bool dry, int* grid_out) {
  const int C4 = A.CsL / 4;
  int G = (20 * 4) / C4;
  if (G < 1) return AVSR_ERR_UNSUPPORTED;
  if (G > CG_MAXTAP) G = CG_MAXTAP;
  { const int ng = (ntaps + G - 1) / G; G = (ntaps + ng - 1) / ng; }
  const float* res = A.res; float* stats = A.stats; const float* bias = A.bias; const float beta = A.beta;
  const float* acc = A.acc; const float* bnb_x = A.bnb_x;
  int grid = 0;
  for (int t0 = 0; t0 < ntaps; t0 += G) {
    const int nt = ntaps - t0 < G ? ntaps - t0 : G;
    const bool first = t0 == 0, last = t0 + nt >= ntaps;
    CGArgs B = A;
    for (int t = 0; t < nt; ++t) B.tap[t] = taps[t0 + t];
    B.ntap = nt;
    B.bias = first ? bias : nullptr; B.beta = first ? beta : 1.f; B.acc = first ? acc : nullptr;
    B.res = last ? res : nullptr; B.stats = last ? stats : nullptr; B.bnb_x = last ? bnb_x : nullptr;
    if (!last) { B.res_sc = nullptr; B.res_sh = nullptr; }
    const int rc = cg_launch(B, s, kind, flops_per_tap * nt, dry);
    if (rc < 0) return rc;
    grid = rc;
  }
  if (grid_out) *grid_out = grid;
  return AVSR_OK;
}

static int cg_pair_taps(CGArgs& A, const CGTap* taps, int ntaps, CGTap* wide) {
  if (A.Cd != 8 || A.S != 1 || A.OS != 1 || (A.OB & 1) || A.oh0 || A.ow0 || A.DH != A.OA || A.DW != A.OB) return 0;
  if (cg_q4_ok(A, ntaps)) return 0;
  int nw = 0;
  for (int t = 0; t < ntaps; ++t)
    for (int pp = 0; pp < 2; ++pp) {
      const int da = taps[t].da, db = taps[t].db + pp;
      int k = 0;
      for (; k < nw; ++k)
        if (wide[k].da == da && wide[k].db == db) break;
      if (k == nw) {
        if (nw == CG_MAXTAP) return 0;
        wide[nw] = cgtap1(da, db, -1);
        ++nw;
      }
      wide[k].w[pp] = taps[t].w[0];
    }
  A.nsp = 2; A.SB = 2; A.OSA = 1; A.OSB = 2; A.lin = 1;
  A.sp_dh[0] = A.sp_dh[1] = 0; A.sp_dw[0] = 0; A.sp_dw[1] = 1;
  A.OB /= 2;
  return nw;
}

static int cg_run_paired(CGArgs& A, const CGTap* taps, int nt, hipStream_t s, int kind, double flops_per_tap, bool dry, int* grid_out) {
  CGTap wide[CG_MAXTAP];
  const int nw = cg_pair_taps(A, taps, nt, wide);
  return nw ? cg_run(A, wide, nw, s, kind, flops_per_tap * nt / nw, dry, grid_out) : cg_run(A, taps, nt, s, kind, flops_per_tap, dry, grid_out);
}

int conv_fwd_impl(const avsr_conv_desc* c, const float* x, const float* w, const float* bias, const float* res, const float* res_sc,
                         const float* res_sh, float* y, float* stats, int32_t* nparts, void* stream, bool dry) {
  if (c->Ci % 4 && c->bn_scale) return AVSR_ERR_UNSUPPORTED;
  CGArgs A = {};
  A.src = x; A.w = w; A.bias = bias; A.dst = y; A.stats = stats; A.res = res; A.bn_sc = c->bn_scale; A.bn_sh = c->bn_shift;
  A.res_sc = res ? res_sc : nullptr; A.res_sh = res ? res_sh : nullptr;
  A.N = c->N; A.SH = c->H; A.SW = c->W; A.Cs = c->Ci; A.CsL = (c->Ci + 3) & ~3;
  A.DH = c->Ho; A.DW = c->Wo; A.Cd = c->Co; A.OA = c->Ho; A.OB = c->Wo; A.S = c->stride; A.OS = 1; A.oh0 = 0; A.ow0 = 0;
  A.wmode = 0; A.beta = 0.f;
  CGTap taps[9];
  const int nt = c->k * c->k;
  for (int t = 0; t < nt; ++t) taps[t] = cgtap1(t / c->k - c->pad_t, t % c->k - c->pad_l, t);
  A.F = cg_frames(c->H, c->W, A.CsL, c->Ho * c->Wo);
  return cg_run_paired(A, taps, nt, S_(stream), PROF_CONV_FWD, 2.0 * c->N * c->Ho * c->Wo * (double)c->Ci * c->Co, dry, nparts);
}

static int cg_class_taps(const avsr_conv_desc* c, int ph, int pw, CGTap* taps) {
  int nt = 0;
  for (int i = 0; i < c->k; ++i) {
    if ((ph + c->pad_t - i) & 1) continue;
    for (int j = 0; j < c->k; ++j) {
      if ((pw + c->pad_l - j) & 1) continue;
      taps[nt++] = cgtap1((ph + c->pad_t - i) >> 1, (pw + c->pad_l - j) >> 1, i * c->k + j);
    }
  }
  return nt;
}

int conv_bwd_data_impl(const avsr_conv_desc* c, const float* dy, const float* w, float* dx, float beta, void* stream, bool dry,
                              const float* acc, const float* bnb_x, const float* bnb_sc,
                              const float* bnb_sh, float* stats, int32_t* nparts) {
  if (c->Ci % 4) return AVSR_ERR_UNSUPPORTED;
  const int k = c->k;
  auto args = [&](int OA, int OB, int OS, int oh0, int ow0) {
    CGArgs A = {};
    A.src = dy; A.w = w; A.dst = dx;
    A.N = c->N; A.SH = c->Ho; A.SW = c->Wo; A.Cs = c->Co; A.CsL = c->Co;
    A.DH = c->H; A.DW = c->W; A.Cd = c->Ci; A.OA = OA; A.OB = OB; A.S = 1; A.OS = OS; A.oh0 = oh0; A.ow0 = ow0;
    A.wmode = 1; A.beta = beta;
    A.acc = acc; A.bnb_x = bnb_x; A.bnb_sc = bnb_sc; A.bnb_sh = bnb_sh; A.stats = stats;
    A.F = cg_frames(c->Ho, c->Wo, A.CsL, OA * OB);
    return A;
  };
  if (c->stride == 1) {
    CGArgs A = args(c->H, c->W, 1, 0, 0);
    CGTap taps[9];
    for (int t = 0; t < k * k; ++t) taps[t] = cgtap1(c->pad_t - t / k, c->pad_l - t % k, t);
    return cg_run_paired(A, taps, k * k, S_(stream), PROF_CONV_BWD_DATA, 2.0 * c->N * c->H * c->W * (double)c->Ci * c->Co, dry, nparts);
  }
  if (k == 3 && c->Ci * 4 <= 64) {
    CGArgs A = args((c->H + 1) / 2, (c->W + 1) / 2, 2, 0, 0);
    A.nsp = 4; A.SB = 1; A.OSA = 2; A.OSB = 2; A.lin = 0;
    CGTap wide[CG_MAXTAP], cls[9];
    int nw = 0, ntot = 0;
    bool fits = true;
    for (int sp = 0; sp < 4 && fits; ++sp) {
      const int ph = sp >> 1, pw = sp & 1;
      A.sp_dh[sp] = (signed char)ph; A.sp_dw[sp] = (signed char)pw;
      const int nc = cg_class_taps(c, ph, pw, cls);
      for (int t = 0; t < nc && fits; ++t) {
        int kk = 0;
        for (; kk < nw; ++kk)
          if (wide[kk].da == cls[t].da && wide[kk].db == cls[t].db) break;
        if (kk == nw) {
          if (nw == CG_MAXTAP) { fits = false; break; }
          wide[nw++] = cgtap1(cls[t].da, cls[t].db, -1);
        }
        wide[kk].w[sp] = cls[t].w[0];
        ++ntot;
      }
    }
    if (fits && nw > 0) {
      const int rc = cg_run(A, wide, nw, S_(stream), PROF_CONV_BWD_DATA, 2.0 * c->N * A.OA * A.OB * (double)c->Ci * c->Co * ntot / nw, dry, nparts);
      if (rc != AVSR_ERR_UNSUPPORTED) return rc;
    }
  }
  if (acc || bnb_x) return AVSR_ERR_UNSUPPORTED;
  if (beta != 1.f) {
    CGTap taps[9];
    for (int ph = 0; ph < 2; ++ph)
      for (int pw = 0; pw < 2; ++pw)
        if ((c->H - ph + 1) / 2 > 0 && (c->W - pw + 1) / 2 > 0 && cg_class_taps(c, ph, pw, taps) == 0) return AVSR_ERR_UNSUPPORTED;
  }
  for (int ph = 0; ph < 2; ++ph)
    for (int pw = 0; pw < 2; ++pw) {
      const int OA = (c->H - ph + 1) / 2, OB = (c->W - pw + 1) / 2;
      if (OA <= 0 || OB <= 0) continue;
      CGArgs A = args(OA, OB, 2, ph, pw);
      CGTap taps[9];
      const int nt = cg_class_taps(c, ph, pw, taps);
      if (nt == 0) continue;
      const int rc = cg_run(A, taps, nt, S_(stream), PROF_CONV_BWD_DATA, 2.0 * c->N * A.OA * A.OB * (double)c->Ci * c->Co, dry, nullptr);
      if (rc < 0) return rc;
    }
  return AVSR_OK;
}

extern "C" int avsr_conv_supported(const avsr_conv_desc* c) {
  if (!g_conv_mfma || !cd_ok(c)) return 0;
  if (conv_fwd_impl(c, nullptr, nullptr, nullptr, nullptr, nullptr, nullptr, nullptr, nullptr, nullptr, nullptr, true) != AVSR_OK) return 0;
  if (c->Ci >= 4 && conv_bwd_data_impl(c, nullptr, nullptr, nullptr, 1.f, nullptr, true) != AVSR_OK) return 0;
  if (conv_bwd_weight_impl(c, nullptr, nullptr, nullptr, nullptr, 1.f, nullptr, 1L << 40, nullptr, true) != AVSR_OK) return 0;
  return 1;
}

extern "C" int avsr_conv_plan(const avsr_conv_desc* c, int32_t op, int32_t flags, int64_t scratch_floats, avsr_conv_launch* out, int32_t cap) {
  if (!cd_ok(c) || op < 0 || op > 2 || cap < 0 || (cap > 0 && !out)) return AVSR_ERR_ARG;
  const int allowed = op == 0 ? (AVSR_CONV_PLAN_BIAS | AVSR_CONV_PLAN_RES | AVSR_CONV_PLAN_STATS)
                    : op == 1 ? (AVSR_CONV_PLAN_BETA | AVSR_CONV_PLAN_ACC | AVSR_CONV_PLAN_BNB)
                              : (AVSR_CONV_PLAN_BETA | AVSR_CONV_PLAN_DBIAS | AVSR_CONV_PLAN_FOLD | AVSR_CONV_PLAN_FOLD_DX);
  if (flags & ~allowed) return AVSR_ERR_ARG;
  if ((flags & AVSR_CONV_PLAN_FOLD_DX) && !(flags & AVSR_CONV_PLAN_FOLD)) return AVSR_ERR_ARG;
  if (!g_conv_mfma) return AVSR_ERR_UNSUPPORTED;
  static float dummy;
  auto opt = [&](int bit) -> float* { return (flags & bit) ? &dummy : nullptr; };
  const float beta = (flags & AVSR_CONV_PLAN_BETA) ? 1.f : 0.f;
  ConvPlanRec R = {out, cap, 0};
  int32_t n = 0;
  g_conv_plan = &R;
  int rc;
  if (op == 0)
    rc = conv_fwd_impl(c, &dummy, &dummy, opt(AVSR_CONV_PLAN_BIAS), opt(AVSR_CONV_PLAN_RES), nullptr, nullptr, &dummy, opt(AVSR_CONV_PLAN_STATS), &n,
                       nullptr, true);
  else if (op == 1)
    rc = conv_bwd_data_impl(c, &dummy, &dummy, &dummy, beta, nullptr, true, opt(AVSR_CONV_PLAN_ACC), opt(AVSR_CONV_PLAN_BNB), opt(AVSR_CONV_PLAN_BNB),
                            opt(AVSR_CONV_PLAN_BNB), opt(AVSR_CONV_PLAN_BNB), &n);
  else
    rc = conv_bwd_weight_impl(c, &dummy, &dummy, &dummy, opt(AVSR_CONV_PLAN_DBIAS), beta, &dummy, scratch_floats, nullptr, true,
                              opt(AVSR_CONV_PLAN_FOLD), opt(AVSR_CONV_PLAN_FOLD), opt(AVSR_CONV_PLAN_FOLD_DX));
  g_conv_plan = nullptr;
  return rc < 0 ? rc : R.n;
}

extern "C" int avsr_conv_fwd(const avsr_conv_desc* c, const float* x, const float* w, const float* bias, const float* res, const float* res_scale,
                             const float* res_shift, float* y, float* stats, int32_t* nparts, void* stream) {
  if (!cd_ok(c) || !x || !w || !y) return AVSR_ERR_ARG;
  if (!g_conv_mfma) return AVSR_ERR_UNSUPPORTED;
  return conv_fwd_impl(c, x, w, bias, res, res_scale, res_shift, y, stats, nparts, stream, false);
}

extern "C" int avsr_conv_bwd_data(const avsr_conv_desc* c, const float* dy, const float* w, float* dx, float beta, void* stream) {
  if (!cd_ok(c) || !dy || !w || !dx) return AVSR_ERR_ARG;
  if (!g_conv_mfma) return AVSR_ERR_UNSUPPORTED;
  return conv_bwd_data_impl(c, dy, w, dx, beta, stream, false);
}

extern "C" int avsr_conv_bwd_data_bn(const avsr_conv_desc* c, const float* dy, const float* w, float* dx, float beta, const float* acc,
                                     const float* bn_x, const float* bn_scale, const float* bn_shift, float* stats, int32_t* nparts,
                                     void* stream) {
  if (!cd_ok(c) || !dy || !w || !dx || (bn_x && (!bn_scale || !bn_shift || !stats || !nparts))) return AVSR_ERR_ARG;
  if (!g_conv_mfma) return AVSR_ERR_UNSUPPORTED;
  return conv_bwd_data_impl(c, dy, w, dx, beta, stream, false, acc, bn_x, bn_scale, bn_shift, bn_x ? stats : nullptr, nparts);
}

extern "C" int avsr_conv_bwd_data_bn_supported(const avsr_conv_desc* c) {
  if (!g_conv_mfma || !cd_ok(c) || c->Ci < 4) return 0;
  static float dummy;
  int32_t n = 0;
  return conv_bwd_data_impl(c, nullptr, nullptr, nullptr, 1.f, nullptr, true, &dummy, &dummy, &dummy, &dummy, &dummy, &n) == AVSR_OK;
}
```

### avsr-tf1_amd/csrc/conv_wgrad.hip

```cpp
#include "conv_mfma.h"
#include "reduce.h"

namespace avsr {

template <int MT, int NTC, bool CH4, bool RS = false, int FOLD = 0>
__global__ __launch_bounds__(256, WG_WPC(MT * NTC)) void conv_wgrad_kernel(const WGArgs A) {
  extern __shared__ __attribute__((aligned(16))) float lds[];
  const int tid = threadIdx.x, lane = tid & 63, wave = __builtin_amdgcn_readfirstlane(tid >> 6);
  const int i = lane & 15, q = lane >> 4;
  const int Ci = A.Ci, CiL = A.CiL, Co = A.Co;
  const int CsP = CiL + A.pad;
  const int PH = A.H + 2, PW = A.W + 2, xstride = PH * PW * CsP;
  const int opf = A.Ho * A.Wo;
  float* const xs = lds;
  const int Mrows = A.nt * CiL;
  const f32x4 zero4 = {0.f, 0.f, 0.f, 0.f};
  for (int idx = tid; idx < A.F * xstride; idx += 256) xs[idx] = 0.f;

  int roff[MT];
#pragma unroll
  for (int mt = 0; mt < MT; ++mt) {
    const int row = (RS ? wave * MT * 16 : 0) + mt * 16 + i;
    const bool ok = row < Mrows;
    const int tl = ok ? row / CiL : 0, ci = ok ? row - tl * CiL : 0, t = A.t0 + tl, ti = t / A.kw, tj = t - ti * A.kw;
    roff[mt] = ok ? ((ti - A.pt) * PW + (tj - A.pl)) * CsP + ci : 0;
  }
  f32x4 acc[MT][NTC];
#pragma unroll
  for (int mt = 0; mt < MT; ++mt)
#pragma unroll
    for (int nt = 0; nt < NTC; ++nt) acc[mt][nt] = zero4;
  const int rowf = A.W * Ci;
  const int st_rq = rowf >> 2;
  const int st_rpp = (CH4 && st_rq > 0) ? (256 / st_rq > 0 ? 256 / st_rq : 1) : 1;
  const int st_row = CH4 ? (tid < st_rpp * st_rq ? fdiv(tid, A.m_rq) : -1) : -1;
  const int st_p4 = st_row >= 0 ? tid - st_row * st_rq : 0;
  const int st_pad = (CH4 && st_row >= 0) ? (st_p4 / (Ci >> 2)) * A.pad : 0;
  const bool st_odd = (A.pad & 1) != 0;
  f32x4 bsc = {1.f, 1.f, 1.f, 1.f}, bsh = zero4;
  const bool bn_on = CH4 && A.bn_sc != nullptr;
  if (bn_on && st_row >= 0) { const int cb = (st_p4 * 4) % Ci; bsc = ld4(A.bn_sc + cb); bsh = ld4(A.bn_sh + cb); }
  float bsum[NTC];
#pragma unroll
  for (int nt = 0; nt < NTC; ++nt) bsum[nt] = 0.f;
  constexpr int PF = CH4 ? 12 : 4;
  f32x4 pre[PF];
  const int ppf = CH4 ? (A.H + st_rpp - 1) / st_rpp : 0;
  const unsigned m_ppf = fmagic_dev(ppf > 0 ? ppf : 1);
  const int per3 = A.H * A.W * Ci;
  const int fs_per = A.N / (int)gridDim.x, fs_extra = A.N - fs_per * (int)gridDim.x;
  const int fs_cnt = fs_per + ((int)blockIdx.x < fs_extra ? 1 : 0), fs_np = (fs_cnt + A.F - 1) / A.F;
  const bool fs_rr = A.F == 1;
  const int FP = fs_rr ? 1 : (fs_np > 0 ? (fs_cnt + fs_np - 1) / fs_np : A.F);
  const int n_begin = fs_rr ? (int)blockIdx.x : (int)blockIdx.x * fs_per + min((int)blockIdx.x, fs_extra);
  const int n_end = fs_rr ? A.N : n_begin + fs_cnt, n_step = fs_rr ? (int)gridDim.x : FP;
  auto fetch = [&](int n0) {
    const int fcur = min(FP, n_end - n0);
    if (CH4) {
#pragma unroll
      for (int u = 0; u < PF; ++u) {
        const int f = fdiv(u, m_ppf), k = u - f * ppf, r = st_row + k * st_rpp;
        pre[u] = (st_row >= 0 && f < fcur && r < A.H) ? ld4(A.x + ((long)(n0 + f) * A.H + r) * rowf + st_p4 * 4) : zero4;
      }
    } else {
      const float* sp = A.x + (long)n0 * per3;
      const int tot4 = (fcur * per3) >> 2;
#pragma unroll
      for (int u = 0; u < PF; ++u) { const int idx = u * 256 + tid; pre[u] = idx < tot4 ? ld4(sp + idx * 4) : zero4; }
    }
  };
  auto commit = [&](int n0) {
    const int fcur = min(FP, n_end - n0);
    if (CH4) {
#pragma unroll
      for (int u = 0; u < PF; ++u) {
        const int f = fdiv(u, m_ppf), k = u - f * ppf, r = st_row + k * st_rpp;
        if (st_row >= 0 && f < fcur && r < A.H) {
          f32x4 v = pre[u];
          if (bn_on) {
#pragma unroll
            for (int e = 0; e < 4; ++e) v[e] = fmaxf(fmaf(v[e], bsc[e], bsh[e]), 0.f);
          }
          float* const dpx = xs + f * xstride + ((r + 1) * PW + 1) * CsP + st_pad + st_p4 * 4;
          if (st_odd) { dpx[0] = v[0]; dpx[1] = v[1]; dpx[2] = v[2]; dpx[3] = v[3]; }
          else {
            *reinterpret_cast<float2*>(dpx) = float2{v[0], v[1]};
            *reinterpret_cast<float2*>(dpx + 2) = float2{v[2], v[3]};
          }
        }
      }
    } else {
      const int tot = fcur * per3, tot4 = tot >> 2;
      auto put = [&](int e, float v) {
        const int f = fdiv(e, A.m_per), r = e - f * per3, px = fdiv(r, A.m_rq), c = r - px * Ci, h = fdiv(px, A.m_w), pw = px - h * A.W;
        xs[f * xstride + ((h + 1) * PW + pw + 1) * CsP + c] = v;
      };
#pragma unroll
      for (int u = 0; u < PF; ++u) {
        const int idx = u * 256 + tid;
        if (idx < tot4) { put(idx * 4, pre[u][0]); put(idx * 4 + 1, pre[u][1]); put(idx * 4 + 2, pre[u][2]); put(idx * 4 + 3, pre[u][3]); }
      }
      const float* sp = A.x + (long)n0 * per3;
      for (int e = tot4 * 4 + tid; e < tot; e += 256) put(e, sp[e]);
    }
  };

  const __amdgpu_buffer_rsrc_t dy_rs = make_rsrc(A.dy);
  const __amdgpu_buffer_rsrc_t fy_rs = make_rsrc(FOLD ? A.fy : A.dy);
  const __amdgpu_buffer_rsrc_t fdx_rs = make_rsrc(FOLD == 2 ? A.fdx : A.part);
  float fk1[NTC], fk2[NTC], fk3[NTC];
#pragma unroll
  for (int nt = 0; nt < NTC; ++nt) {
    fk1[nt] = 1.f; fk2[nt] = 0.f; fk3[nt] = 0.f;
    if (FOLD) {
      const int col = nt * 16 + i, ch = col % A.fC;
      const bool okc = col < Co;
      fk1[nt] = okc ? A.fk[ch] : 0.f; fk2[nt] = okc ? A.fk[A.fC + ch] : 0.f; fk3[nt] = okc ? A.fk[2 * A.fC + ch] : 0.f;
    }
  }
  const int cpf = (opf + 15) >> 4;
  const unsigned m_cpf = fmagic_dev(cpf);
  int n0 = n_begin;
  if (n0 < n_end) fetch(n0);
  for (; n0 < n_end; n0 += n_step) {
    const int fcur = min(FP, n_end - n0);
    __syncthreads();
    commit(n0);
    const int kch = fcur * cpf;
    const unsigned dyo = (unsigned)((long)n0 * opf * Co * 4);
    float bn[NTC][4], byn[FOLD ? NTC : 1][4];
    auto load_b = [&](int kc, float (&b)[NTC][4]) {
      const int f = fdiv(kc, m_cpf), r0 = (kc - f * cpf) * 16 + q * 4;
      const unsigned o = dyo + (unsigned)(((f * opf + r0) * Co + i) * 4);
#pragma unroll
      for (int e = 0; e < 4; ++e)
#pragma unroll
        for (int nt = 0; nt < NTC; ++nt) {
          const int off = (r0 + e < opf && nt * 16 + i < Co) ? (int)(o + (unsigned)((e * Co + nt * 16) * 4)) : P_OOB;
          b[nt][e] = ldb1(dy_rs, off);
          if (FOLD) byn[nt][e] = ldb1(fy_rs, off);
        }
    };
    constexpr int KC0 = RS ? 0 : -1, KCS = RS ? 1 : 4;
    const int kc0 = KC0 < 0 ? wave : KC0;
    if (kc0 < kch) load_b(kc0, bn);
    __syncthreads();
    if (n0 + n_step < n_end) fetch(n0 + n_step);
    for (int kc = kc0; kc < kch; kc += KCS) {
      float av[MT][4], bv[NTC][4];
      const int f = fdiv(kc, m_cpf), r0 = (kc - f * cpf) * 16 + q * 4;
#pragma unroll
      for (int nt = 0; nt < NTC; ++nt)
#pragma unroll
        for (int e = 0; e < 4; ++e) {
          bv[nt][e] = bn[nt][e];
          if (FOLD) bv[nt][e] = (r0 + e < opf) ? fmaf(fk1[nt], bn[nt][e], fmaf(fk2[nt], byn[nt][e], fk3[nt])) : 0.f;
          if (FOLD == 2 && (!RS || wave == 0))
            __builtin_amdgcn_raw_buffer_store_b32(__builtin_bit_cast(unsigned, bv[nt][e]), fdx_rs,
                                                  (r0 + e < opf && nt * 16 + i < Co) ? (int)(dyo + (unsigned)(((f * opf + r0 + e) * Co + nt * 16 + i) * 4)) : P_OOB, 0, 0);
        }
#pragma unroll
      for (int nt = 0; nt < NTC; ++nt) bsum[nt] += (bv[nt][0] + bv[nt][1]) + (bv[nt][2] + bv[nt][3]);
      if (kc + KCS < kch) load_b(kc + KCS, bn);
      int ho = fdiv(min(r0, opf - 1), A.m_wo), wo = min(r0, opf - 1) - ho * A.Wo;
      const float* xf = xs + f * xstride + (PW + 1) * CsP;
#pragma unroll
      for (int e = 0; e < 4; ++e) {
        const float* xb = xf + (ho * A.S * PW + wo * (A.SW ? A.SW : A.S)) * CsP;
#pragma unroll
        for (int mt = 0; mt < MT; ++mt) av[mt][e] = xb[roff[mt]];
        if (++wo == A.Wo) { wo = 0; ++ho; }
        if (ho >= A.Ho) { ho = A.Ho - 1; }
      }
      __builtin_amdgcn_sched_barrier(0);
#pragma unroll
      for (int e = 0; e < 4; ++e)
#pragma unroll
        for (int mt = 0; mt < MT; ++mt)
#pragma unroll
          for (int nt = 0; nt < NTC; ++nt) acc[mt][nt] = __builtin_amdgcn_mfma_f32_16x16x4f32(av[mt][e], bv[nt][e], acc[mt][nt], 0, 0, 0);
      __builtin_amdgcn_sched_barrier(0);
    }
  }
  float* red = lds;
  const int rr = tid >> 4, cc = tid & 15;
  if (RS) {
    __syncthreads();
#pragma unroll
    for (int mt = 0; mt < MT; ++mt)
#pragma unroll
      for (int r = 0; r < 4; ++r) {
        const int row = wave * MT * 16 + mt * 16 + q * 4 + r;
        if (row < Mrows) {
          const int t = row / CiL, ci = row - t * CiL;
          if (ci < Ci) {
#pragma unroll
            for (int nt = 0; nt < NTC; ++nt)
              if (nt * 16 + i < Co) A.part[(long)blockIdx.x * A.slab + ((long)t * Ci + ci) * Co + nt * 16 + i] = acc[mt][nt][r];
          }
        }
      }
  } else
#pragma unroll
  for (int mt = 0; mt < MT; ++mt)
#pragma unroll
    for (int nt = 0; nt < NTC; ++nt) {
      __syncthreads();
#pragma unroll
      for (int r = 0; r < 4; ++r) red[(wave * 16 + q * 4 + r) * 16 + i] = acc[mt][nt][r];
      __syncthreads();
      const int row = mt * 16 + rr, co = nt * 16 + cc;
      if (row < Mrows && co < Co) {
        const int t = row / CiL, ci = row - t * CiL;
        if (ci < Ci) A.part[(long)blockIdx.x * A.slab + ((long)t * Ci + ci) * Co + co] = (red[rr * 16 + cc] + red[(16 + rr) * 16 + cc]) + (red[(32 + rr) * 16 + cc] + red[(48 + rr) * 16 + cc]);
      }
    }
  if (A.want_bias) {
    __syncthreads();
#pragma unroll
    for (int nt = 0; nt < NTC; ++nt) red[((wave * 4 + q) * NTC + nt) * 16 + i] = (RS && wave) ? 0.f : bsum[nt];
    __syncthreads();
    if (tid < NTC * 16) {
      const int nt = tid >> 4, ci = tid & 15;
      float s = 0.f;
      for (int g = 0; g < 16; ++g) s += red[(g * NTC + nt) * 16 + ci];
      if (nt * 16 + ci < Co) A.part[(long)blockIdx.x * A.slab + (long)A.nt * Ci * Co + nt * 16 + ci] = s;
    }
  }
}

}

using namespace avsr;

static int wg_occupancy(int tiles, int H, int W, int CiL, int* pad) {
  *pad = WG_PAD;
  const int cap = WG_WPC(tiles);
  auto frame = [&](int p) { return sizeof(float) * (size_t)(H + 2) * (W + 2) * (CiL + p); };
  if (2 * frame(WG_PAD) <= 64 * 1024) return 2;
  for (int w = cap; w > 2; --w) {
    if (w * (frame(WG_PAD) + 512) <= 160 * 1024) return w;
    if (w * (frame(1) + 512) <= 160 * 1024) { *pad = 1; return w; }
  }
  return 2;
}

static int wg_pick_frames(int N, int Fmax, int slots) {
  double best = -1.0;
  int bestF = Fmax;
  for (int F = Fmax; F >= 1; --F) {
    const long units = (N + F - 1) / F, grid = units < slots ? units : slots;
    const long cnt = (N + grid - 1) / grid, np = (cnt + F - 1) / F, fp = (cnt + np - 1) / np;
    const double cost = (double)np * (8.0 * fp + 1.0);
    if (best < 0.0 || cost < best) { best = cost; bestF = F; }
  }
  return bestF;
}

struct WGPlan { size_t lds; int wpc, wpc_cap; };
static bool wg_plan(WGArgs& A, int occ_tiles, int slab_floats, bool shrink, WGPlan* P) {
  const int N = A.N, H = A.H, W = A.W, Ci = A.Ci, opf = A.Ho * A.Wo;
  P->wpc_cap = occ_tiles ? wg_occupancy(occ_tiles, H, W, A.CiL, &A.pad) : (A.pad = WG_PAD, 2);
  A.F = cg_frames(H, W, A.CiL + A.pad, opf);
  A.m_opf = fmagic(opf); A.m_wo = fmagic(A.Wo); A.m_w = fmagic(W);
  if (Ci % 4 == 0) {
    const int rq = W * Ci / 4;
    if (rq > 256 || rq < 1) return false;
    const int rpp = 256 / rq;
    while (A.F > 1 && A.F * ((H + rpp - 1) / rpp) > 12) --A.F;
    if (A.F * ((H + rpp - 1) / rpp) > 12) return false;
    A.m_rq = fmagic(rq); A.m_per = fmagic(H * rq);
  } else {
    if (A.bn_sc) return false;
    while (A.F > 1 && (A.F * H * W * Ci / 4 + 255) / 256 > 4) --A.F;
    if ((A.F * H * W * Ci / 4 + 255) / 256 > 4 || (long)A.F * H * W * Ci >= 65536) return false;
    A.m_rq = fmagic(Ci); A.m_per = fmagic(H * W * Ci);
  }
  const size_t frame = sizeof(float) * (size_t)(H + 2) * (W + 2) * (A.CiL + A.pad);
  if (shrink) while (A.F > 1 && A.F * frame > 64 * 1024) --A.F;
  A.F = wg_pick_frames(N, A.F, slab_floats > 2048 ? 256 : 256 * P->wpc_cap);
  if ((long)A.F * ((opf + 15) / 16) >= 65536 || (long)N * opf * A.Co * 4 >= (1L << 31)) return false;
  P->lds = A.F * frame;
  if (P->lds < sizeof(float) * 4 * 256) P->lds = sizeof(float) * 4 * 256;
  if (P->lds > 64 * 1024) return false;
  P->wpc = (int)((160 * 1024) / (P->lds + 512));
  if (P->wpc > P->wpc_cap) P->wpc = P->wpc_cap;
  if (P->wpc < 1) P->wpc = 1;
  return true;
}

static int wg_grid(int N, int F, int slab, int wpc, long scratch_floats) {
  int grid = (N + F - 1) / F;
  const int cap = 256 * (slab > 2048 ? 1 : wpc);
  if (grid > cap) grid = cap;
  if ((long)grid * slab > scratch_floats) grid = (int)(scratch_floats / slab);
  return grid;
}

static void wg_note(const WGArgs& A, int m, int ntc, bool rs, int fold, int nsp, int grid, size_t lds) {
  if (!g_conv_plan) return;
  avsr_conv_launch L = {};
  L.kernel = 2; L.m = m; L.ntc = ntc; L.ch4 = A.Ci % 4 == 0; L.rs = rs; L.fold = fold; L.nsp = nsp; L.ntap = A.nt; L.t0 = A.t0; L.F = A.F;
  L.grid = grid; L.CsP = A.CiL + A.pad; L.lds_bytes = (int32_t)lds; L.slab = A.slab;
  conv_plan_note(L);
}

int conv_bwd_weight_impl(const avsr_conv_desc* c, const float* x, const float* dy, float* dw, float* dbias, float beta, float* scratch,
                                long scratch_floats, void* stream, bool dry, const float* fold_y, const float* fold_k,
                                float* fold_dx) {
  const int Ci = c->Ci, Co = c->Co, H = c->H, W = c->W, Ho = c->Ho, Wo = c->Wo, N = c->N, k = c->k;
  const bool fold = fold_k != nullptr;
  if (Co == 8 && c->stride == 1 && k == 3 && (Wo & 1) == 0 && Wo == W && Ho == H) {
    WGArgs A = {};
    A.x = x; A.dy = dy; A.part = scratch; A.N = N; A.H = H; A.W = W; A.Ci = Ci; A.CiL = (Ci + 3) & ~3; A.Ho = Ho; A.Wo = Wo / 2; A.Co = 16;
    A.S = 1; A.SW = 2; A.pt = c->pad_t; A.pl = c->pad_l; A.kw = 4; A.bn_sc = c->bn_scale; A.bn_sh = c->bn_shift;
    A.t0 = 0; A.nt = 12; A.want_bias = dbias ? 1 : 0;
    A.fy = fold_y; A.fk = fold_k; A.fC = 8; A.fdx = fold_dx;
    A.slab = 12 * Ci * 16 + (A.want_bias ? 16 : 0);
    const int MT = (12 * A.CiL + 15) / 16;
    WGPlan P;
    if ((Ci % 4 == 0 ? MT <= 6 : MT <= 3) && wg_plan(A, MT, A.slab, false, &P)) {
      const int grid = wg_grid(N, A.F, A.slab, P.wpc, scratch_floats);
      if (grid < 1) return AVSR_ERR_ARG;
      if (dry) { wg_note(A, Ci % 4 ? 3 : 6, 1, false, fold ? (fold_dx ? 2 : 1) : 0, 2, grid, P.lds); return AVSR_OK; }
      hipStream_t s = S_(stream);
      {
        ProfScope ps(PROF_CONV_BWD_WEIGHT, s, 2.0 * N * Ho * Wo * 9.0 * Ci * Co);
#define WG_PAIR(M_, C_, F_) hipLaunchKernelGGL((conv_wgrad_kernel<M_, 1, C_, false, F_>), dim3(grid), dim3(256), P.lds, s, A)
        const int fm = fold ? (fold_dx ? 2 : 1) : 0;
        if (Ci % 4) { if (fm == 2) WG_PAIR(3, false, 2); else if (fm == 1) WG_PAIR(3, false, 1); else WG_PAIR(3, false, 0); }
        else { if (fm == 2) WG_PAIR(6, true, 2); else if (fm == 1) WG_PAIR(6, true, 1); else WG_PAIR(6, true, 0); }
#undef WG_PAIR
        if (hipGetLastError() != hipSuccess) return AVSR_ERR_HIP;
      }
      return slab_reduce(scratch, A.slab, grid, 9 * Ci * 8 + 8, dw, dbias, 0, 1, Ci, 1.0f, beta, s);
    }
  }
  WGArgs A = {};
  A.x = x; A.dy = dy; A.part = scratch; A.N = N; A.H = H; A.W = W; A.Ci = Ci; A.CiL = (Ci + 3) & ~3; A.Ho = Ho; A.Wo = Wo; A.Co = Co;
  A.S = c->stride; A.pt = c->pad_t; A.pl = c->pad_l; A.kw = k; A.bn_sc = c->bn_scale; A.bn_sh = c->bn_shift;
  A.fy = fold_y; A.fk = fold_k; A.fC = Co; A.fdx = fold_dx;
  const int NTC = (Co + 15) / 16;
  if (NTC == 3) return AVSR_ERR_UNSUPPORTED;
  const int mt_max = NTC == 4 ? 9 : 18;
  int G = mt_max * 16 / A.CiL;
  if (G < 1) return AVSR_ERR_UNSUPPORTED;
  const int mt_first = ((k * k < G ? k * k : G) * A.CiL + 15) / 16;
  const int tiles_first = (mt_first <= 5 ? 5 : (mt_first <= 9 ? 9 : 18)) * (NTC == 1 ? 1 : (NTC == 2 ? 2 : 4));
  WGPlan P;
  {
    const int nt0 = k * k < G ? k * k : G;
    if (!wg_plan(A, Ci % 4 == 0 ? tiles_first : 0, nt0 * Ci * Co + Co, true, &P)) return AVSR_ERR_UNSUPPORTED;
  }
  const size_t lds = P.lds;
  hipStream_t s = S_(stream);
  bool bias_done = dbias == nullptr;
  const int Mall = k * k * A.CiL;
  const bool rs = NTC == 4 && Ci % 4 == 0 && G < k * k && Mall <= 4 * 9 * 16;
  if (rs) G = k * k;
  if (fold) {
    const int MT1 = rs ? ((k * k * A.CiL + 3) / 4 + 15) / 16 : (k * k * A.CiL + 15) / 16;
    const bool okf = G >= k * k && Ci % 4 == 0 && (rs ? MT1 <= 5 : (NTC == 1 ? MT1 <= 5 : (NTC == 2 && MT1 <= 9)));
    if (!okf) return AVSR_ERR_UNSUPPORTED;
  }
  for (int t0 = 0; t0 < k * k; t0 += G) {
    A.t0 = t0; A.nt = k * k - t0 < G ? k * k - t0 : G;
    A.want_bias = bias_done ? 0 : 1;
    const int wF = A.nt * Ci * Co;
    A.slab = wF + (A.want_bias ? Co : 0);
    const int MT = rs ? ((A.nt * A.CiL + 3) / 4 + 15) / 16 : (A.nt * A.CiL + 15) / 16;
    if (Ci % 4 && (MT > 3 || NTC != 1)) return AVSR_ERR_UNSUPPORTED;
    const int grid = wg_grid(N, A.F, A.slab, P.wpc, scratch_floats);
    if (grid < 1) return AVSR_ERR_ARG;
    if (dry) {
      const int m = fold ? (rs || NTC == 1 ? 5 : 9) : (Ci % 4 ? 3 : (MT <= 5 ? 5 : (MT <= 9 || NTC == 4 ? 9 : 18)));
      wg_note(A, m, Ci % 4 ? 1 : NTC, rs, fold ? (fold_dx ? 2 : 1) : 0, 1, grid, lds);
      bias_done = true;
      continue;
    }
    {
      ProfScope ps(PROF_CONV_BWD_WEIGHT, s, 2.0 * N * Ho * Wo * (double)A.nt * Ci * Co);
#define WG_GO(M_, N_, C_) hipLaunchKernelGGL((conv_wgrad_kernel<M_, N_, C_>), dim3(grid), dim3(256), lds, s, A)
      if (fold) {
#define WG_FOLD(M_, N_, R_) { if (fold_dx) hipLaunchKernelGGL((conv_wgrad_kernel<M_, N_, true, R_, 2>), dim3(grid), dim3(256), lds, s, A); \
                              else hipLaunchKernelGGL((conv_wgrad_kernel<M_, N_, true, R_, 1>), dim3(grid), dim3(256), lds, s, A); }
        if (rs) WG_FOLD(5, 4, true)
        else if (NTC == 1) WG_FOLD(5, 1, false)
        else WG_FOLD(9, 2, false)
#undef WG_FOLD
      } else if (rs) {
        if (MT <= 5) hipLaunchKernelGGL((conv_wgrad_kernel<5, 4, true, true>), dim3(grid), dim3(256), lds, s, A);
        else hipLaunchKernelGGL((conv_wgrad_kernel<9, 4, true, true>), dim3(grid), dim3(256), lds, s, A);
      } else if (Ci % 4) WG_GO(3, 1, false);
      else if (NTC == 1) { if (MT <= 5) WG_GO(5, 1, true); else if (MT <= 9) WG_GO(9, 1, true); else WG_GO(18, 1, true); }
      else if (NTC == 2) { if (MT <= 5) WG_GO(5, 2, true); else if (MT <= 9) WG_GO(9, 2, true); else WG_GO(18, 2, true); }
      else { if (MT <= 5) WG_GO(5, 4, true); else WG_GO(9, 4, true); }
#undef WG_GO
      if (hipGetLastError() != hipSuccess) return AVSR_ERR_HIP;
    }
    const int rc = slab_reduce(scratch, A.slab, grid, A.slab, dw + (long)t0 * Ci * Co, A.want_bias ? dbias : nullptr,
                               A.want_bias ? wF : 0x7fffffff, 0, 0, 1.0f, beta, s);
    bias_done = true;
    if (rc != AVSR_OK) return rc;
    if (avsr::slab_deferring()) { scratch += (long)grid * A.slab; scratch_floats -= (long)grid * A.slab; A.part = scratch; }
  }
  return AVSR_OK;
}

extern "C" int avsr_conv_bwd_weight_bn(const avsr_conv_desc* c, const float* x, const float* dz, const float* y, const float* k, float* dx_out,
                                       float* dw, float* dbias, float beta, float* scratch, int64_t scratch_floats, void* stream) {
  if (!cd_ok(c) || !x || !dz || !y || !k || !dw || !scratch) return AVSR_ERR_ARG;
  if (!g_conv_mfma) return AVSR_ERR_UNSUPPORTED;
  return conv_bwd_weight_impl(c, x, dz, dw, dbias, beta, scratch, scratch_floats, stream, false, y, k, dx_out);
}
extern "C" int avsr_conv_bwd_weight_bn_supported(const avsr_conv_desc* c) {
  if (!g_conv_mfma || !cd_ok(c)) return 0;
  static float dummy;
  return conv_bwd_weight_impl(c, nullptr, nullptr, nullptr, nullptr, 1.f, nullptr, 1L << 40, nullptr, true, &dummy, &dummy) == AVSR_OK;
}

extern "C" int avsr_conv_bwd_weight(const avsr_conv_desc* c, const float* x, const float* dy, float* dw, float* dbias, float beta, float* scratch,
                                    int64_t scratch_floats, void* stream) {
  if (!cd_ok(c) || !x || !dy || !dw || !scratch) return AVSR_ERR_ARG;
  if (!g_conv_mfma) return AVSR_ERR_UNSUPPORTED;
  return conv_bwd_weight_impl(c, x, dy, dw, dbias, beta, scratch, scratch_floats, stream, false);
}
```

### avsr-tf1_amd/ops.py

```python
import ctypes as C
import os

import torch

from . import _lib
from ._lib import (AttnMech, AttnRnn, GemmDesc, Mat, RnnLayer, RnnStack, TransposeJob, check, stream_ptr)


def fptr(t, offset=0):
    if t is None:
        return None
    assert t.is_cuda, "HIP engine buffers must live on the GPU"
    return t.data_ptr() + t.element_size() * int(offset)


def mat(t, ld, T=0, ldo=0, offset=0):
    assert t.dtype == torch.float32
    return Mat(fptr(t, offset), int(ld), int(T), 0, int(ldo))


def _L():
    return _lib.load()


# ... 317 lines not shown
    check(_L().avsr_dropout_rows(C.byref(x), C.byref(y), rows, cols, fptr(seed), int(stream_id), float(keep), int(idx_width),
                                 int(idx_coff), int(accumulate), _s()), "avsr_dropout_rows")


LOSS_FUN = {None: 0, "label_smoothing": 1, "focal_loss": 2, "mc_loss": 3}


def seq_loss(logits, labels, labels_len, denom, compute_denom, row_loss, dlogits, B, L, V, loss_fun=0, label_smoothing=0.0):
    check(_L().avsr_seq_loss_fun(fptr(logits), fptr(labels), fptr(labels_len), fptr(denom), int(compute_denom),
                                 fptr(row_loss), fptr(dlogits), B, L, V, int(loss_fun), float(label_smoothing), _s()), "avsr_seq_loss_fun")


def au_loss(z, aus, lens, row_loss, dz, B, T, weight, total_count=None):
    check(_L().avsr_au_loss_dp(fptr(z), fptr(aus), fptr(lens), fptr(row_loss), fptr(dz), B, T, float(weight), fptr(total_count), _s()),
          "avsr_au_loss_dp")


def ctc_ws_floats(B, T, L):
    return int(_L().avsr_ctc_ws_floats(int(B), int(T), int(L)))


def ctc_loss(z, ld, labels, labels_len, in_len, denom, weight, nll, status, utt_loss, dz, ws, B, T, L, n_classes):
    from ._lib import CtcArgs
    a = CtcArgs()
    a.B, a.T, a.L, a.C, a.ld = int(B), int(T), int(L), int(n_classes), int(ld)
    a.z, a.labels, a.labels_len, a.in_len, a.denom = fptr(z), fptr(labels), fptr(labels_len), fptr(in_len), fptr(denom)
    a.weight = float(weight)
    a.nll, a.status, a.utt_loss, a.dz, a.ws, a.ws_floats = fptr(nll), fptr(status), fptr(utt_loss), fptr(dz), fptr(ws), int(ws.numel())
    check(_L().avsr_ctc_loss(C.byref(a), _s()), "avsr_ctc_loss")


def ctc_best_path(z, ld, in_len, B, T, n_classes, ids):
    check(_L().avsr_ctc_best_path(fptr(z), int(ld), fptr(in_len), int(B), int(T), int(n_classes), fptr(ids), _s()), "avsr_ctc_best_path")


def ctc_prefix_search_supported(V, beam_width, L_max):
    return bool(_L().avsr_ctc_prefix_search_supported(int(V), int(beam_width), int(L_max)))


def _ctc_prefix_args(z, ld, in_len, B, T, V, beam_width, L_max, ids, lens, score, trace):
    from ._lib import CtcPrefixArgs
    a = CtcPrefixArgs()
    a.B, a.T, a.V, a.beam_width, a.L_max, a.ld = int(B), int(T), int(V), int(beam_width), int(L_max), int(ld)
    a.z, a.in_len, a.ids, a.lens, a.score = fptr(z), fptr(in_len), fptr(ids), fptr(lens), fptr(score)
    if trace is not None:
        a.trace_parent, a.trace_sym, a.trace_pb, a.trace_pnb = (fptr(t) for t in trace)
    return a


def ctc_prefix_search(z, ld, in_len, B, T, V, beam_width, L_max, ids, lens, score, trace=None):
    a = _ctc_prefix_args(z, ld, in_len, B, T, V, beam_width, L_max, ids, lens, score, trace)
    check(_L().avsr_ctc_prefix_search(C.byref(a), _s()), "avsr_ctc_prefix_search")


def ctc_prefix_lm_supported(V, beam_width, L_max, n_layers, H, E, one_hot):
    return bool(_L().avsr_ctc_prefix_lm_supported(int(V), int(beam_width), int(L_max), int(n_layers), int(H), int(E), int(one_hot)))


def ctc_prefix_lm_ws_bytes(B, beam_width, n_layers, H):
    return int(_L().avsr_ctc_prefix_lm_ws_bytes(int(B), int(beam_width), int(n_layers), int(H)))


def ctc_prefix_search_lm(z, ld, in_len, B, T, V, beam_width, L_max, ids, lens, score, lm, trace=None):
    a = _ctc_prefix_args(z, ld, in_len, B, T, V, beam_width, L_max, ids, lens, score, trace)
    check(_L().avsr_ctc_prefix_search_lm(C.byref(a), C.byref(lm), _s()), "avsr_ctc_prefix_search_lm")


def ctc_prefix_ngram_supported(V, beam_width, L_max, n_nodes, n_arcs):
    return bool(_L().avsr_ctc_prefix_ngram_supported(int(V), int(beam_width), int(L_max), int(n_nodes), int(n_arcs)))


def ctc_prefix_search_ngram(z, ld, in_len, B, T, V, beam_width, L_max, ids, lens, score, ng, trace=None):
    a = _ctc_prefix_args(z, ld, in_len, B, T, V, beam_width, L_max, ids, lens, score, trace)
    check(_L().avsr_ctc_prefix_search_ngram(C.byref(a), C.byref(ng), _s()), "avsr_ctc_prefix_search_ngram")


def ctc_align_supported(V, L):
    return bool(_L().avsr_ctc_align_supported(int(V), int(L)))


def ctc_align_ws_bytes(B, T, L):
    return int(_L().avsr_ctc_align_ws_bytes(int(B), int(T), int(L)))


def ctc_align(z, ld, labels, target_len, in_len, B, T, L, V, score, status, path, frame_lp, start, end, ws):
    from ._lib import CtcAlignArgs
    a = CtcAlignArgs()
    a.B, a.T, a.L, a.V, a.ld = int(B), int(T), int(L), int(V), int(ld)
    a.z, a.labels, a.target_len, a.in_len = fptr(z), fptr(labels), fptr(target_len), fptr(in_len)
    a.score, a.status, a.path, a.frame_lp, a.start, a.end = fptr(score), fptr(status), fptr(path), fptr(frame_lp), fptr(start), fptr(end)
    a.ws, a.ws_bytes = fptr(ws), int(ws.numel() * ws.element_size())
    check(_L().avsr_ctc_align(C.byref(a), _s()), "avsr_ctc_align")


def seq_logprob(logits, labels, labels_len, B, L, V, out, out_stride=1, out_offset=0):
    assert out_offset >= 0 and out_stride >= 1 and out_offset + (int(B) - 1) * int(out_stride) < out.numel()
    check(_L().avsr_seq_logprob(fptr(logits), fptr(labels), fptr(labels_len), int(B), int(L), int(V), fptr(out, out_offset),
                                int(out_stride), _s()), "avsr_seq_logprob")


def rescore_select(s_att, s_ctc, n, B, K, weight, order, final):
    assert min(s_att.numel(), s_ctc.numel(), order.numel(), final.numel()) >= int(B) * int(K) and n.numel() >= int(B)
    check(_L().avsr_rescore_select(fptr(s_att), fptr(s_ctc), fptr(n), int(B), int(K), float(weight), fptr(order), fptr(final), _s()),
          "avsr_rescore_select")


def normed_v(v, g, vn, H):
    check(_L().avsr_normed_v(fptr(v), fptr(g), fptr(vn), H, _s()), "avsr_normed_v")


def normed_v_bwd(v, g, dvn, dv, dg, H):
    check(_L().avsr_normed_v_bwd(fptr(v), fptr(g), fptr(dvn), fptr(dv), fptr(dg), H, _s()), "avsr_normed_v_bwd")


def reduce_scalar(part, n, out, do_sqrt=False, accumulate=False, scale=1.0, out_offset=0):
    check(_L().avsr_reduce_scalar(fptr(part), n, fptr(out, out_offset), int(do_sqrt), int(accumulate), float(scale),
                                  _s()), "avsr_reduce_scalar")


def l2_regularise(segments, params, grads, l2, loss_accum, scratch):
    n = len(segments)
    if n == 0:
        return
    off = (C.c_int64 * n)(*[int(o) for o, _ in segments])
    cnt = (C.c_int64 * n)(*[int(c) for _, c in segments])
    check(_L().avsr_l2_regularise(off, cnt, n, fptr(params), fptr(grads), float(l2), fptr(loss_accum), fptr(scratch),
                                  _s()), "avsr_l2_regularise")


def global_norm(grads, n, norm_out, scratch, grad_scale=1.0):
    check(_L().avsr_global_norm(fptr(grads), n, float(grad_scale), fptr(norm_out), fptr(scratch), _s()),
          "avsr_global_norm")


def seq_loss_per_utterance(row_loss, labels_len, denom, out, B, L):
    check(_L().avsr_seq_loss_per_utterance(fptr(row_loss), fptr(labels_len), fptr(denom), fptr(out), B, L, _s()),
          "avsr_seq_loss_per_utterance")


def highway_fwd(x, h, cpre, y, lens, B, T, H):
    check(_L().avsr_highway_fwd(C.byref(x), C.byref(h), C.byref(cpre), C.byref(y), fptr(lens), B, T, H, _s()), "avsr_highway_fwd")


def highway_bwd(x, h, cpre, dy, dh, dcpre, dx, lens, B, T, H, accumulate_dx=False):
    check(_L().avsr_highway_bwd(C.byref(x), C.byref(h), C.byref(cpre), C.byref(dy), C.byref(dh), C.byref(dcpre), C.byref(dx), fptr(lens),
                                B, T, H, int(accumulate_dx), _s()), "avsr_highway_bwd")


def copy_(dst, src):
    assert dst.is_cuda and src.is_cuda and dst.numel() == src.numel() and dst.element_size() == 4 and src.element_size() == 4
    assert dst.is_contiguous() and src.is_contiguous() and dst.dtype == src.dtype
    check(_L().avsr_copy_words(dst.data_ptr(), src.data_ptr(), dst.numel(), _s()), "avsr_copy_words")


def zero_(dst):
    assert dst.is_cuda and dst.element_size() == 4 and dst.is_contiguous()
    check(_L().avsr_zero_words(dst.data_ptr(), dst.numel(), _s()), "avsr_zero_words")


def zero_multi(tensors):
    ts = [t for t in tensors if t is not None and t.numel()]
    if not ts:
        return
    for t in ts:
        assert t.is_cuda and t.element_size() == 4 and t.is_contiguous()
    ptrs = (C.c_void_p * len(ts))(*[t.data_ptr() for t in ts])
    cnt = (C.c_int64 * len(ts))(*[t.numel() for t in ts])
    check(_L().avsr_zero_multi(ptrs, cnt, len(ts), _s()), "avsr_zero_multi")


def add_int(a, b, out):
    check(_L().avsr_add_int(fptr(a), int(b), fptr(out), _s()), "avsr_add_int")


def instnorm_fwd(x, y, B, T, F, gamma, beta, mean_out, invstd_out, eps=1e-6):
    check(_L().avsr_instnorm_fwd(fptr(x), fptr(y), B, T, F, fptr(gamma), fptr(beta), fptr(mean_out), fptr(invstd_out), float(eps), _s()),
          "avsr_instnorm_fwd")


def instnorm_bwd(x, dy, gamma, mean, invstd, dx, dgamma_part, dbeta_part, B, T, F):
    check(_L().avsr_instnorm_bwd(fptr(x), fptr(dy), fptr(gamma), fptr(mean), fptr(invstd), fptr(dx), fptr(dgamma_part), fptr(dbeta_part),
                                 B, T, F, _s()), "avsr_instnorm_bwd")


OPTIMISER = {"Adam": 0, "Nadam": 1, "AdamW": 2, "Momentum": 3}


def adam_step(params, grads, m, v, n, gnorm, step, lr, warmup_steps, clip_norm, grad_scale=1.0, first_decay_steps=0, optimiser="Adam",
              weight_decay=0.0):
    check(_L().avsr_optimiser_step(fptr(params), fptr(grads), fptr(m), fptr(v), n, fptr(gnorm), fptr(step), float(lr),
                                   int(warmup_steps), int(first_decay_steps), float(clip_norm), float(grad_scale), OPTIMISER[optimiser],
                                   float(weight_decay), _s()), "avsr_optimiser_step")


PROF_KINDS = ("gemm", "step_lstm_fwd", "step_lstm_bwd", "step_dense", "attn_fwd", "attn_bwd", "rnn_persist_fwd", "rnn_persist_bwd", "dec_persist_fwd", "dec_persist_bwd",
              "conv_fwd", "conv_bwd_data", "conv_bwd_weight", "align_persist_fwd", "align_persist_bwd")


def prof_begin(max_launches=65536):
    check(_L().avsr_prof_begin(int(max_launches)), "avsr_prof_begin")


def prof_end():
    cnt = (C.c_int32 * len(PROF_KINDS))()
    ms = (C.c_float * len(PROF_KINDS))()
    fl = (C.c_double * len(PROF_KINDS))()
    check(_L().avsr_prof_end(cnt, ms, fl), "avsr_prof_end")
    return {k: (int(cnt[i]), float(ms[i]), float(fl[i])) for i, k in enumerate(PROF_KINDS)}


_persist_sync = None
_persist_scratch = None


def rnn_set_persistent(on, device="cuda", ints=1 << 20, mode=3, scratch_floats=64 << 20):
    global _persist_sync, _persist_scratch
    check(_L().avsr_rnn_set_persistent_mode(int(mode)), "avsr_rnn_set_persistent_mode")
    if on:
        if _persist_sync is None:
            _persist_sync = torch.zeros(ints, dtype=torch.int32, device=device)
        if (mode & 6) == 2 and _persist_scratch is None:
            _persist_scratch = torch.zeros(scratch_floats, dtype=torch.float32, device=device)
        if _persist_scratch is not None:
            check(_L().avsr_rnn_set_persistent_scratch(_persist_scratch.data_ptr(), _persist_scratch.numel()), "avsr_rnn_set_persistent_scratch")
        _persist_sync[:1].zero_()
        check(_L().avsr_rnn_set_persistent(_persist_sync.data_ptr(), ints), "avsr_rnn_set_persistent")
    else:
        check(_L().avsr_rnn_set_persistent(None, 0), "avsr_rnn_set_persistent")


def rnn_persistent_clear():
    if _persist_sync is not None:
        _persist_sync[:1].zero_()


def attn_rnn_fused_ws_floats(B, n_mech, Dmax=256):
    return int(_L().avsr_attn_rnn_fused_ws_floats(int(B), int(n_mech), int(Dmax)))


def attn_rnn_fused_eligible(desc):
    return bool(_L().avsr_attn_rnn_fused_eligible(C.byref(desc)))


def attn_rnn_fused_fwd_active(desc):
    return bool(_L().avsr_attn_rnn_fused_fwd_active(C.byref(desc)))


def attn_rnn_set_fused(on):
    check(_L().avsr_attn_rnn_set_fused(int(on)), "avsr_attn_rnn_set_fused")


def attn_rnn_set_beam_kernel(on):
    check(_L().avsr_attn_rnn_set_beam_kernel(int(on)), "avsr_attn_rnn_set_beam_kernel")


def rnn_persistent_error():
    return bool(_persist_sync is not None and int(_persist_sync[:1].item()) != 0)


def batchnorm_fwd_ex(x, y, rows, F, gamma, beta, mov_mean, mov_var, save_mean, save_invstd, training, eps, momentum, relu, scratch, bessel=1):
    check(_L().avsr_batchnorm_fwd_ex(fptr(x), fptr(y), rows, F, fptr(gamma), fptr(beta), fptr(mov_mean), fptr(mov_var), fptr(save_mean),
                                     fptr(save_invstd), int(training), float(eps), float(momentum), int(relu), int(bessel), fptr(scratch),
                                     scratch.numel(), _s()), "avsr_batchnorm_fwd_ex")


def batchnorm_bwd(x, dy, gamma, beta, mean, invstd, dx, dgamma, dbeta, rows, F, relu, scratch, dx_beta=0.0):
    check(_L().avsr_batchnorm_bwd(fptr(x), fptr(dy), fptr(gamma), fptr(beta), fptr(mean), fptr(invstd), fptr(dx), fptr(dgamma), fptr(dbeta),
                                  rows, F, int(relu), float(dx_beta), fptr(scratch), scratch.numel(), _s()), "avsr_batchnorm_bwd")


def im2col(x, col, N, H, W, Cc, kh, kw, stride, pad_t, pad_l, Ho, Wo):
    check(_L().avsr_im2col(fptr(x), fptr(col), N, H, W, Cc, kh, kw, stride, pad_t, pad_l, Ho, Wo, _s()), "avsr_im2col")


def col2im(dcol, dx, N, H, W, Cc, kh, kw, stride, pad_t, pad_l, Ho, Wo, beta=0.0):
    check(_L().avsr_col2im(fptr(dcol), fptr(dx), N, H, W, Cc, kh, kw, stride, pad_t, pad_l, Ho, Wo, float(beta), _s()), "avsr_col2im")


def relu(x, y, n):
    check(_L().avsr_relu(fptr(x), fptr(y), int(n), _s()), "avsr_relu")


def relu_bwd(y, dy, dx, n):
    check(_L().avsr_relu_bwd(fptr(y), fptr(dy), fptr(dx), int(n), _s()), "avsr_relu_bwd")


def add(a, b, out, n):
    check(_L().avsr_add(fptr(a), fptr(b), fptr(out), int(n), _s()), "avsr_add")


def conv3x3_supported(Ci, Co, H, W):
    return bool(_L().avsr_conv3x3_supported(Ci, Co, H, W))


def conv3x3(x, w, bias, y, N, H, W, Ci, Co, stride, pad_t, pad_l, Ho, Wo, flip=0, beta=0.0):
    check(_L().avsr_conv3x3(fptr(x), fptr(w), fptr(bias), fptr(y), N, H, W, Ci, Co, stride, pad_t, pad_l, Ho, Wo, int(flip), float(beta), _s()),
          "avsr_conv3x3")


def conv_set_mfma(on):
    check(_L().avsr_conv_set_mfma(int(on)), "avsr_conv_set_mfma")


def conv_desc(N, H, W, Ci, Co, k, stride, pad_t, pad_l, Ho, Wo, bn=None):
    from ._lib import ConvDesc
    d = ConvDesc(N, H, W, Ci, Co, k, stride, pad_t, pad_l, Ho, Wo, 0, None, None)
    if bn is not None:
        d.bn_scale, d.bn_shift = fptr(bn[0]), fptr(bn[1])
    return d


def conv_supported(d):
    return bool(_L().avsr_conv_supported(C.byref(d)))


def conv_fwd(d, x, w, bias, y, res=None, res_bn=None, stats=None):
    n = C.c_int32(0)
    check(_L().avsr_conv_fwd(C.byref(d), fptr(x), fptr(w), fptr(bias), fptr(res), fptr(res_bn[0]) if res_bn else None,
                             fptr(res_bn[1]) if res_bn else None, fptr(y), fptr(stats), C.byref(n), _s()), "avsr_conv_fwd")
    return int(n.value)


def conv_bwd_data(d, dy, w, dx, beta=0.0):
    check(_L().avsr_conv_bwd_data(C.byref(d), fptr(dy), fptr(w), fptr(dx), float(beta), _s()), "avsr_conv_bwd_data")


def conv_bwd_data_bn_supported(d):
    return bool(_L().avsr_conv_bwd_data_bn_supported(C.byref(d)))


def conv_bwd_data_bn(d, dy, w, dx, beta=0.0, acc=None, bn_x=None, bn=None, stats=None):
    n = C.c_int32(0)
    check(_L().avsr_conv_bwd_data_bn(C.byref(d), fptr(dy), fptr(w), fptr(dx), float(beta), fptr(acc), fptr(bn_x),
                                     fptr(bn[0]) if bn else None, fptr(bn[1]) if bn else None, fptr(stats), C.byref(n), _s()), "avsr_conv_bwd_data_bn")
    return int(n.value)


def bn_bwd_finalize(part, nparts, Cn, count, mean, invstd, gamma, dgamma, dbeta, k, grad_beta=1.0):
    check(_L().avsr_bn_bwd_finalize(fptr(part), int(nparts), int(Cn), int(count), fptr(mean), fptr(invstd), fptr(gamma), fptr(dgamma), fptr(dbeta),
                                    float(grad_beta), fptr(k), _s()), "avsr_bn_bwd_finalize")


def bn_partials_f64(part, nparts, Cn, out64):
    check(_L().avsr_bn_partials_f64(fptr(part), int(nparts), int(Cn), out64.data_ptr(), _s()), "avsr_bn_partials_f64")


def bn_finalize_f64(sums64, Cn, eps, momentum, mean, invstd, mov_mean, mov_var, gamma=None, beta=None, scale=None, shift=None):
    check(_L().avsr_bn_finalize_f64(sums64.data_ptr(), int(Cn), float(eps), float(momentum), fptr(mean), fptr(invstd), fptr(mov_mean), fptr(mov_var),
                                    fptr(gamma), fptr(beta), fptr(scale), fptr(shift), _s()), "avsr_bn_finalize_f64")


def bn_bwd_finalize_f64(local64, global64, Cn, mean, invstd, gamma, dgamma, dbeta, k, grad_beta=1.0):
    check(_L().avsr_bn_bwd_finalize_f64(local64.data_ptr(), global64.data_ptr(), int(Cn), fptr(mean), fptr(invstd), fptr(gamma), fptr(dgamma),
                                        fptr(dbeta), float(grad_beta), fptr(k), _s()), "avsr_bn_bwd_finalize_f64")


def bn_eval_affine(gamma, beta, mov_mean, mov_var, eps, scale, shift, Cn):
    check(_L().avsr_bn_eval_affine(fptr(gamma), fptr(beta), fptr(mov_mean), fptr(mov_var), float(eps), fptr(scale), fptr(shift), int(Cn), _s()),
          "avsr_bn_eval_affine")


def bn_bwd_apply(dz, x, k, dx, rows, Cn, beta=0.0):
    check(_L().avsr_bn_bwd_apply(fptr(dz), fptr(x), fptr(k), fptr(dx), int(rows), int(Cn), float(beta), _s()), "avsr_bn_bwd_apply")


def bn_bwd_stage1(dy, x, dz, rows, Cn, part, scale=None, shift=None, y=None):
    n = C.c_int32(0)
    check(_L().avsr_bn_bwd_stage1(fptr(dy), fptr(x), fptr(scale), fptr(shift), fptr(y), fptr(dz), int(rows), int(Cn), fptr(part), C.byref(n), _s()),
          "avsr_bn_bwd_stage1")
    return int(n.value)


def conv_bwd_weight(d, x, dy, dw, dbias, scratch, beta=1.0):
    check(_L().avsr_conv_bwd_weight(C.byref(d), fptr(x), fptr(dy), fptr(dw), fptr(dbias), float(beta), fptr(scratch), scratch.numel(), _s()),
          "avsr_conv_bwd_weight")


def conv_bwd_weight_bn(d, x, dz, y, k, dw, dbias, scratch, beta=1.0, dx_out=None):
    check(_L().avsr_conv_bwd_weight_bn(C.byref(d), fptr(x), fptr(dz), fptr(y), fptr(k), fptr(dx_out), fptr(dw), fptr(dbias), float(beta),
                                       fptr(scratch), scratch.numel(), _s()), "avsr_conv_bwd_weight_bn")


def conv_bwd_weight_bn_supported(d):
    return bool(_L().avsr_conv_bwd_weight_bn_supported(C.byref(d)))


CONV_PLAN_OPS = {"fwd": 0, "bwd_data": 1, "bwd_weight": 2}
CONV_PLAN_FLAGS = {"bias": 1, "res": 2, "stats": 4, "beta": 8, "acc": 16, "bnb": 32, "fold": 64, "fold_dx": 128, "dbias": 256}


def conv_plan(d, op, flags=(), scratch_floats=1 << 40, cap=16):
    from ._lib import ConvLaunch
    bits = flags if isinstance(flags, int) else sum(CONV_PLAN_FLAGS[f] for f in set(flags))
    out = (ConvLaunch * cap)()
    n = _L().avsr_conv_plan(C.byref(d), CONV_PLAN_OPS[op] if isinstance(op, str) else int(op), bits, int(scratch_floats), out, cap)
    if n < 0:
        check(n, "avsr_conv_plan")
    assert n <= cap
    return [{f: getattr(out[i], f) for f, _ in ConvLaunch._fields_ if f != "pad_"} for i in range(n)]


def slab_defer_begin():
    check(_L().avsr_slab_defer_begin(), "avsr_slab_defer_begin")


def conv3d_desc(B, T, H, W, Ci, Co, k, stride, pads, Ho, Wo, tf=None, relu=1):
    from ._lib import Conv3dDesc
    d = Conv3dDesc(B, T, H, W, Ci, Co, k[0], k[1], k[2], stride, pads[0], pads[1], pads[2], Ho, Wo, int(relu), None, None)
    if tf is not None:
        d.scale, d.shift = fptr(tf[0]), fptr(tf[1])
    return d


def conv3d_supported(d):
    return bool(_L().avsr_conv3d_supported(C.byref(d)))


def conv3d_wgrad_scratch_floats(d):
    n = int(_L().avsr_conv3d_wgrad_scratch_floats(C.byref(d)))
    if n < 0:
        raise _lib.AvsrError("avsr_conv3d_wgrad_scratch_floats: unsupported geometry")
    return n


def conv3d_fwd(d, x, w, y, res=None, res_tf=None, stats=None):
    n = C.c_int32(0)
    check(_L().avsr_conv3d_fwd(C.byref(d), fptr(x), fptr(w), fptr(res), fptr(res_tf[0]) if res_tf else None, fptr(res_tf[1]) if res_tf else None,
                               fptr(y), fptr(stats), C.byref(n), _s()), "avsr_conv3d_fwd")
    return int(n.value)


def conv3d_bwd_data(d, dy, w, dx, beta=0.0):
    check(_L().avsr_conv3d_bwd_data(C.byref(d), fptr(dy), fptr(w), fptr(dx), float(beta), _s()), "avsr_conv3d_bwd_data")


def conv3d_bwd_weight(d, x, dy, dw, scratch, beta=1.0):
    check(_L().avsr_conv3d_bwd_weight(C.byref(d), fptr(x), fptr(dy), fptr(dw), float(beta), fptr(scratch), scratch.numel(), _s()),
          "avsr_conv3d_bwd_weight")


def logmel_supported(frame_length, fft_length, num_mel_bins, window, stride):
    return bool(_L().avsr_logmel_supported(int(frame_length), int(fft_length), int(num_mel_bins), int(window), int(stride)))


def logmel_fwd(spec, tables, wav, wav_len, out, out_len=None):
    a = _lib.LogmelArgs(B=wav.shape[0], N=wav.shape[1], T_out=out.shape[1], F=out.shape[2], frame_length=spec.frame_length,
                        frame_step=spec.frame_step, fft_length=spec.fft_length, num_mel_bins=spec.num_mel_bins, window=spec.window,
                        stride=spec.stride, mel_nnz=tables["mel_w"].numel(), wav=fptr(wav), wav_len=fptr(wav_len), hann=fptr(tables["hann"]),
                        twiddle=fptr(tables["twiddle"]), mel_lo=fptr(tables["mel_lo"]), mel_cnt=fptr(tables["mel_cnt"]),
                        mel_ptr=fptr(tables["mel_ptr"]), mel_w=fptr(tables["mel_w"]), out=fptr(out), out_len=fptr(out_len))
    check(_L().avsr_logmel_fwd(C.byref(a), _s()), "avsr_logmel_fwd")


def spec_augment_supported(B, T, F, freq_masks, time_masks):
    return bool(_L().avsr_spec_augment_supported(int(B), int(T), int(F), int(freq_masks), int(time_masks)))


def spec_augment_ws_floats(B, T, F_in):
    return int(_L().avsr_spec_augment_ws_floats(int(B), int(T), int(F_in)))


def spec_augment(x, F_in, lens, seed, y, ws, video=False, freq_masks=0, freq_width=0, freq_bins=0, time_masks=0, time_width=0,
                 ratio_q16=65536, mean_fill=True):
    assert x.dim() == 3 and y.dim() == 3 and x.is_contiguous() and y.is_contiguous() and x.dtype == y.dtype == torch.float32
    assert x.shape[:2] == y.shape[:2] and F_in <= x.shape[2] and F_in <= y.shape[2] and x.data_ptr() != y.data_ptr()
    assert lens.dtype == torch.int32 and lens.is_contiguous() and lens.numel() == x.shape[0] and seed.dtype == torch.int32
    a = _lib.SpecAugmentArgs(B=x.shape[0], T=x.shape[1], F_in=int(F_in), F=y.shape[2], freq_masks=int(freq_masks), freq_width=int(freq_width),
                             freq_bins=int(freq_bins), time_masks=int(time_masks), time_width=int(time_width), ratio_q16=int(ratio_q16),
                             video=int(bool(video)), mean_fill=int(bool(mean_fill)), ld=x.shape[2], x=fptr(x), len=fptr(lens),
                             seed=fptr(seed), y=fptr(y), ws=fptr(ws), ws_floats=0 if ws is None else ws.numel())
    check(_L().avsr_spec_augment(C.byref(a), _s()), "avsr_spec_augment")


def conv3d_bn_finalize(part, nparts, Cn, count, eps, momentum, mean, invstd, mov_mean, mov_var, gamma=None, beta=None, scale=None, shift=None):
    check(_L().avsr_conv3d_bn_finalize(fptr(part), int(nparts), int(Cn), int(count), float(eps), float(momentum), fptr(mean), fptr(invstd),
                                       fptr(mov_mean), fptr(mov_var), fptr(gamma), fptr(beta), fptr(scale), fptr(shift), _s()),
          "avsr_conv3d_bn_finalize")


def slab_defer_end():
    check(_L().avsr_slab_defer_end(_s()), "avsr_slab_defer_end")


def bn_finalize(part, nparts, Cn, count, eps, momentum, mean, invstd, mov_mean, mov_var, gamma=None, beta=None, scale=None, shift=None):
    check(_L().avsr_bn_finalize(fptr(part), int(nparts), int(Cn), int(count), float(eps), float(momentum), fptr(mean), fptr(invstd),
                                fptr(mov_mean), fptr(mov_var), fptr(gamma), fptr(beta), fptr(scale), fptr(shift), _s()), "avsr_bn_finalize")


def batchnorm_apply(x, y, rows, F, gamma, beta, mean, invstd, relu):
    check(_L().avsr_batchnorm_apply(fptr(x), fptr(y), rows, F, fptr(gamma), fptr(beta), fptr(mean), fptr(invstd), int(relu), _s()),
          "avsr_batchnorm_apply")


def conv3x3_bwd_data_s2(dy, w, dx, N, H, W, Ci, Co, pad_t, pad_l, Ho, Wo, beta=0.0):
    check(_L().avsr_conv3x3_bwd_data_s2(fptr(dy), fptr(w), fptr(dx), N, H, W, Ci, Co, pad_t, pad_l, Ho, Wo, float(beta), _s()),
          "avsr_conv3x3_bwd_data_s2")


def conv3x3_bwd_weight(x, dy, dw, N, H, W, Ci, Co, stride, pad_t, pad_l, Ho, Wo, scratch, beta=1.0):
    check(_L().avsr_conv3x3_bwd_weight(fptr(x), fptr(dy), fptr(dw), N, H, W, Ci, Co, stride, pad_t, pad_l, Ho, Wo, float(beta), fptr(scratch),
                                       scratch.numel(), _s()), "avsr_conv3x3_bwd_weight")


def selu(z, y, n):
    check(_L().avsr_selu(fptr(z), fptr(y), int(n), _s()), "avsr_selu")


def selu_bwd(z, dy, dz, n):
    check(_L().avsr_selu_bwd(fptr(z), fptr(dy), fptr(dz), int(n), _s()), "avsr_selu_bwd")
```

### include/avsr_hip.h

```cpp
#ifndef AVSR_HIP_H
#define AVSR_HIP_H
#include <stdint.h>

#ifdef __cplusplus
extern "C" {
#endif
#if defined(__GNUC__) || defined(__clang__)
#pragma GCC visibility push(default)
#endif

#define AVSR_OK 0
#define AVSR_ERR_ARG (-1)
#define AVSR_ERR_HIP (-2)
#define AVSR_ERR_UNSUPPORTED (-3)

#define AVSR_MAX_LAYERS 4
#define AVSR_MAX_MECH 4
#define AVSR_MAX_STACKS 4
#define AVSR_HAVE_ATTN 1
#define AVSR_MAX_TRANSPOSE 16
#define AVSR_MAX_SEGMENTS 32

int avsr_abi_version(void);
int64_t avsr_sizeof(const char* name);
// ... 100 lines not shown
  const float* bq;
  const float* wq_t;
  const float* wq;
  const float* watt_t;
  const float* watt;
  float* scores;
  float* ctx;
  float* pq;
  float* pstat;
  float* pctx;
  float* dscores;
  float* dctx;
  float* dpq;
  float* pdq;
} avsr_attn_mech;

typedef struct avsr_dec_layer {
  const float* wt;
  const float* w;
  const float* bias;
  float* gates;
  float* cs;
  float* out;
  float* state;
  float* hs_seq;
  float* xin_seq;
  float* dgates;
  float* dstate;
  int32_t cell_id, pad_;
  const float* wt2;
  const float* w2;
  const float* bias2;
  float* rh_seq;
  float* dgates2;
} avsr_dec_layer;
#define AVSR_MAX_DEC_EXTRA 3

typedef struct avsr_attn_rnn {
  int32_t B, L, H, E, n_mech, output_attention, V, mode;
  int32_t go_id, eos_id;
  int32_t* steplen;
  const float* wt;
  const float* w;
  const float* bias;
  float* gates;
  float* cs;
  float* cell_out;
  float* att;
  const float* h0;
  const float* c0;
  float* state;
  float* h_final;
  float* c_final;
  avsr_attn_mech mech[AVSR_MAX_MECH];
  const float* embedding;
  const float* wout_t;
  const float* bout;
  float* logits;
  int32_t* ids;
  int32_t* tok;
  int32_t* n_unfinished;
  float* dgates;
  float* dstate;
  float* datt;
  float* dq;
  const float* datt_ext;
  const float* dcell_ext;
  float* dh0;
  float* dc0;
  const float* dh_final;
  const float* dc_final;
  const int32_t* seed;
  float keep_in, keep_state, keep_out, sampling_prob;
  int32_t cell_id, pad3_;
  float* hs_seq;
  float* attd;
  float* xs;
  const int32_t* labels;
  int32_t* fed;
  int32_t cell, pad4_;
  const float* wt2;
  const float* w2;
  const float* bias2;
  float* rh_seq;
  float* dgates2;
  int32_t beam_width, mem_shared;
  float length_penalty;
  float pad6_;
  float* beam_logp;
  int32_t* beam_fin;
  int32_t* beam_len;
  int32_t* step_ids;
  int32_t* parent_ids;
  int32_t* parent_rows;
  int32_t n_extra, prof_tag;
  float* out0;
  avsr_dec_layer extra[AVSR_MAX_DEC_EXTRA];
  float* fused_ws;
  int64_t fused_ws_floats;
} avsr_attn_rnn;
int64_t avsr_attn_rnn_fused_ws_floats(int32_t B, int32_t n_mech, int32_t Dmax);
int avsr_attn_rnn_fused_eligible(const avsr_attn_rnn* d);
int avsr_attn_rnn_fused_fwd_active(const avsr_attn_rnn* d);
int avsr_attn_rnn_set_fused(int32_t on);
int avsr_attn_rnn_set_beam_kernel(int32_t on);

int avsr_attn_rnn_fwd(const avsr_attn_rnn* d, int32_t l_begin, int32_t l_end, void* stream);
int avsr_attn_rnn_bwd(const avsr_attn_rnn* d, void* stream);
int avsr_beam_gather_tree(const int32_t* step_ids, const int32_t* parent_ids, const int32_t* beam_len, int32_t* out,
                          int32_t n_utt, int32_t beam_width, int32_t T, int32_t eos_id, void* stream);

int avsr_beam_search_step(float* logits, int32_t n_utt, int32_t beam_width, int32_t V, int32_t step, int32_t eos_id,
                          float length_penalty_weight, const float* logp_in, const int32_t* fin_in, const int32_t* len_in,
                          float* logp_out, int32_t* fin_out, int32_t* len_out, int32_t* tok, int32_t* parent_rows,
                          int32_t* step_ids, int32_t* parent_ids, int32_t* n_unfinished, const float* x, int64_t x_stride,
                          int32_t O, const float* wout_t, const float* bout, void* stream);

#define AVSR_MAX_LM_LAYERS 4
typedef struct avsr_beam_lm {
  int32_t n_layers, H, E, V;
  int32_t one_hot, n_rows;
  float lm_weight;
  int32_t pad_;
  const float* embedding;
  const float* wt[AVSR_MAX_LM_LAYERS];
  const float* bias[AVSR_MAX_LM_LAYERS];
  const float* wout_t;
  const float* bout;
  float* state_c;
  float* state_h;
  float* lm_logp;
} avsr_beam_lm;
int avsr_beam_lm_supported(const avsr_beam_lm* lm);
int avsr_beam_lm_step(const avsr_beam_lm* lm, const int32_t* tok, const int32_t* parent_rows, int32_t n_rows, int32_t step, void* stream);
int avsr_beam_search_step_lm(float* logits, int32_t n_utt, int32_t beam_width, int32_t V, int32_t step, int32_t eos_id,
                             float length_penalty_weight, const float* logp_in, const int32_t* fin_in, const int32_t* len_in,
                             float* logp_out, int32_t* fin_out, int32_t* len_out, int32_t* tok, int32_t* parent_rows,
                             int32_t* step_ids, int32_t* parent_ids, int32_t* n_unfinished, const float* x, int64_t x_stride,
                             int32_t O, const float* wout_t, const float* bout, const float* lm_logp, float lm_weight, void* stream);
int avsr_attn_rnn_fwd_lm(const avsr_attn_rnn* d, const avsr_beam_lm* lm, int32_t l_begin, int32_t l_end, void* stream);

#define AVSR_BEAM_CTC_MAX_T 2048
#define AVSR_BEAM_CTC_MAX_V 256
typedef struct avsr_beam_ctc {
  int32_t n_utt, beam_width, T, V;
  int32_t eos_id;
  float weight;
  int64_t ld;
  const float* z;
  const int32_t* in_len;
  float* y;
  float* state;
  float* psi;
  int32_t* last;
  float* term;
  float* extra;
  const float* lm_logp;
  float lm_weight;
  int32_t pad_;
} avsr_beam_ctc;
int avsr_beam_ctc_supported(const avsr_beam_ctc* ctc);
int avsr_beam_ctc_begin(const avsr_beam_ctc* ctc, void* stream);
int avsr_beam_ctc_step(const avsr_beam_ctc* ctc, const int32_t* tok, const int32_t* parent_rows, const int32_t* fin, int32_t step,
                       void* stream);
int avsr_beam_search_step_ctc(float* logits, int32_t n_utt, int32_t beam_width, int32_t V, int32_t step, int32_t eos_id,
                              float length_penalty_weight, const float* logp_in, const int32_t* fin_in, const int32_t* len_in,
                              float* logp_out, int32_t* fin_out, int32_t* len_out, int32_t* tok, int32_t* parent_rows,
                              int32_t* step_ids, int32_t* parent_ids, int32_t* n_unfinished, const float* x, int64_t x_stride,
                              int32_t O, const float* wout_t, const float* bout, const float* lm_logp, float lm_weight,
                              const float* ctc_term, float ctc_weight, float* extra, void* stream);
int avsr_attn_rnn_fwd_ctc(const avsr_attn_rnn* d, const avsr_beam_lm* lm, const avsr_beam_ctc* ctc, int32_t l_begin, int32_t l_end,
                          void* stream);

#define AVSR_CTC_PREFIX_MAX_V 256
#define AVSR_CTC_PREFIX_MAX_W 64
#define AVSR_CTC_PREFIX_MAX_L 512
typedef struct avsr_ctc_prefix_args {
  int32_t B, T, V, beam_width, L_max;
  int32_t pad_;
  int64_t ld;
  const float* z;
  const int32_t* in_len;
  int32_t* ids;
  int32_t* lens;
  float* score;
  int32_t* trace_parent;
  int32_t* trace_sym;
  float* trace_pb;
  float* trace_pnb;
} avsr_ctc_prefix_args;
int avsr_ctc_prefix_search_supported(int32_t V, int32_t beam_width, int32_t L_max);
int avsr_ctc_prefix_search(const avsr_ctc_prefix_args* a, void* stream);

#define AVSR_CTC_PREFIX_LM_MAX_W 16
typedef struct avsr_ctc_prefix_lm {
  int32_t n_layers, H, E, V;
  int32_t one_hot, go_id, eos_id;
  float weight, bonus;
  int32_t pad_;
  const float* embedding;
  const float* wt[AVSR_MAX_LM_LAYERS];
  const float* bias[AVSR_MAX_LM_LAYERS];
  const float* wout_t;
  const float* bout;
  void* ws;
  int64_t ws_bytes;
  float* s_lm;
  int32_t* lm_steps;
  float* lm_logp;
} avsr_ctc_prefix_lm;
int avsr_ctc_prefix_lm_supported(int32_t V, int32_t beam_width, int32_t L_max, int32_t n_layers, int32_t H, int32_t E, int32_t one_hot);
int64_t avsr_ctc_prefix_lm_ws_bytes(int32_t B, int32_t beam_width, int32_t n_layers, int32_t H);
int avsr_ctc_prefix_search_lm(const avsr_ctc_prefix_args* a, const avsr_ctc_prefix_lm* lm, void* stream);

#define AVSR_CTC_PREFIX_NGRAM_MAX_ORDER 16
#define AVSR_CTC_PREFIX_NGRAM_MAX_NODES (1 << 24)
#define AVSR_CTC_PREFIX_NGRAM_MAX_ARCS (1 << 26)
typedef struct avsr_ctc_prefix_ngram {
  int32_t n_nodes, n_arcs, V, start;
  int32_t go_id, eos_id;
  float weight, bonus;
  const float* bow;
  const int32_t* backoff;
  const int32_t* arc_begin;
  const int32_t* sym;
  const float* logp;
  const int32_t* next;
  float* s_lm;
  int32_t* lm_steps;
  float* lm_logp;
} avsr_ctc_prefix_ngram;
int avsr_ctc_prefix_ngram_supported(int32_t V, int32_t beam_width, int32_t L_max, int32_t n_nodes, int32_t n_arcs);
int avsr_ctc_prefix_search_ngram(const avsr_ctc_prefix_args* a, const avsr_ctc_prefix_ngram* ng, void* stream);

#define AVSR_CTC_ALIGN_MAX_L 512
typedef struct avsr_ctc_align_args {
  int32_t B, T, L, V;
  int64_t ld;
  const float* z;
  const int32_t* labels;
  const int32_t* target_len;
  const int32_t* in_len;
  float* score;
  int32_t* status;
  int32_t* path;
  float* frame_lp;
  int32_t* start;
  int32_t* end;
  void* ws;
  int64_t ws_bytes;
} avsr_ctc_align_args;
int avsr_ctc_align_supported(int32_t V, int32_t L);
int64_t avsr_ctc_align_ws_bytes(int32_t B, int32_t T, int32_t L);
int avsr_ctc_align(const avsr_ctc_align_args* a, void* stream);

int avsr_seq_logprob(const float* logits, const int32_t* labels, const int32_t* labels_len, int32_t B, int32_t L, int32_t V,
                     float* out, int64_t out_stride, void* stream);
int avsr_rescore_select(const float* s_att, const float* s_ctc, const int32_t* n, int32_t B, int32_t K, float weight,
                        int32_t* order, float* final_out, void* stream);

int avsr_attn_alpha_rows(float* scores, const float* dscores, const int32_t* len, const int32_t* steplen,
                         const float* g, float* rowdot, int32_t B, int32_t L, int32_t T, void* stream);
int avsr_bahdanau_dkeys(const float* keys, const float* pq, int64_t pq_sb, int64_t pq_sl, const float* dscores,
                        const float* v, const float* bq, const int32_t* len, float* dkeys, float* dv_part,
                        int32_t B, int32_t L, int32_t T, int32_t H, void* stream);

typedef struct avsr_transpose_job {
  const float* src;
  float* dst;
  int32_t rows, cols;
} avsr_transpose_job;
int avsr_transpose(const avsr_transpose_job* jobs, int32_t n, void* stream);

int avsr_colsum(const avsr_mat* a, const avsr_mat* b, int32_t rows, int32_t F, float alpha, float beta, float* out,
                float* scratch, int64_t scratch_floats, void* stream);

int avsr_batchnorm_fwd(const float* x, float* y, int32_t rows, int32_t F, const float* gamma, const float* beta,
                       float* moving_mean, float* moving_var, float* save_mean, float* save_invstd, int32_t training,
                       float* scratch, int64_t scratch_floats, void* stream);
int avsr_batchnorm_fwd_ex(const float* x, float* y, int32_t rows, int32_t F, const float* gamma, const float* beta,
                          float* moving_mean, float* moving_var, float* save_mean, float* save_invstd, int32_t training,
                          float eps, float momentum, int32_t relu, int32_t bessel, float* scratch, int64_t scratch_floats,
                          void* stream);
int avsr_batchnorm_sync_sum(const float* x, int32_t rows, int32_t F, float* sum_out, float* scratch, int64_t scratch_floats,
                            void* stream);
int avsr_batchnorm_sync_sqsum(const float* x, int32_t rows, int32_t F, const float* sum_global, const float* total_rows,
                              float* mean_out, float* sq_out, float* scratch, int64_t scratch_floats, void* stream);
int avsr_batchnorm_sync_moments(const float* x, int32_t rows, int32_t F, double* out64, float* scratch, int64_t scratch_floats, void* stream);
int avsr_dp_sync_unpack(const double* buf, float* dp_norm, int32_t nstream, const int32_t* off, const int32_t* F, float* const* mean,
                        float* const* sq, float* const* rows, void* stream);
int avsr_batchnorm_sync_apply(const float* x, float* y, int32_t rows, int32_t F, const float* gamma, const float* beta,
                              float* moving_mean, float* moving_var, const float* mean, const float* sq_global,
                              const float* total_rows, float* invstd_out, float eps, float momentum, int32_t relu, void* stream);
int avsr_batchnorm_bwd(const float* x, const float* dy, const float* gamma, const float* beta, const float* mean,
                       const float* invstd, float* dx, float* dgamma, float* dbeta, int32_t rows, int32_t F, int32_t relu,
                       float dx_beta, float* scratch, int64_t scratch_floats, void* stream);

int avsr_im2col(const float* x, float* col, int32_t N, int32_t H, int32_t W, int32_t C, int32_t kh, int32_t kw, int32_t stride,
                int32_t pad_t, int32_t pad_l, int32_t Ho, int32_t Wo, void* stream);
int avsr_col2im(const float* dcol, float* dx, int32_t N, int32_t H, int32_t W, int32_t C, int32_t kh, int32_t kw, int32_t stride,
                int32_t pad_t, int32_t pad_l, int32_t Ho, int32_t Wo, float beta, void* stream);
int avsr_conv3x3_supported(int32_t Ci, int32_t Co, int32_t H, int32_t W);
int avsr_conv_set_mfma(int32_t on);
typedef struct avsr_conv_desc {
  int32_t N, H, W, Ci, Co, k, stride, pad_t, pad_l, Ho, Wo, pad_;
  const float* bn_scale;
  const float* bn_shift;
} avsr_conv_desc;
int avsr_conv_supported(const avsr_conv_desc* c);
int avsr_conv_fwd(const avsr_conv_desc* c, const float* x, const float* w, const float* bias, const float* res, const float* res_scale,
                  const float* res_shift, float* y, float* stats, int32_t* nparts, void* stream);
int avsr_conv_bwd_data(const avsr_conv_desc* c, const float* dy, const float* w, float* dx, float beta, void* stream);
int avsr_conv_bwd_weight(const avsr_conv_desc* c, const float* x, const float* dy, float* dw, float* dbias, float beta, float* scratch,
                         int64_t scratch_floats, void* stream);
int avsr_conv_bwd_data_bn(const avsr_conv_desc* c, const float* dy, const float* w, float* dx, float beta, const float* acc,
                          const float* bn_x, const float* bn_scale, const float* bn_shift, float* stats, int32_t* nparts, void* stream);
int avsr_conv_bwd_data_bn_supported(const avsr_conv_desc* c);
int avsr_conv_bwd_weight_bn(const avsr_conv_desc* c, const float* x, const float* dz, const float* y, const float* k, float* dx_out,
                            float* dw, float* dbias, float beta, float* scratch, int64_t scratch_floats, void* stream);
int avsr_conv_bwd_weight_bn_supported(const avsr_conv_desc* c);
#define AVSR_CONV_PLAN_BIAS 1
#define AVSR_CONV_PLAN_RES 2
#define AVSR_CONV_PLAN_STATS 4
#define AVSR_CONV_PLAN_BETA 8
#define AVSR_CONV_PLAN_ACC 16
#define AVSR_CONV_PLAN_BNB 32
#define AVSR_CONV_PLAN_FOLD 64
#define AVSR_CONV_PLAN_FOLD_DX 128
#define AVSR_CONV_PLAN_DBIAS 256
typedef struct avsr_conv_launch {
  int32_t kernel, m, ntc, ch4, rs, fold, ep, nsp;
  int32_t ntap, t0, F, grid, CsP, lds_bytes, slab, pad_;
} avsr_conv_launch;
int avsr_conv_plan(const avsr_conv_desc* c, int32_t op, int32_t flags, int64_t scratch_floats, avsr_conv_launch* out, int32_t cap);
int avsr_bn_bwd_finalize(const float* part, int32_t nparts, int32_t C, int64_t count, const float* mean, const float* invstd,
                         const float* gamma, float* dgamma, float* dbeta, float grad_beta, float* k, void* stream);
int avsr_bn_bwd_apply(const float* dz, const float* x, const float* k, float* dx, int64_t rows, int32_t C, float beta, void* stream);
int avsr_bn_bwd_stage1(const float* dy, const float* x, const float* scale, const float* shift, const float* y, float* dz, int64_t rows,
                       int32_t C, float* part, int32_t* nparts, void* stream);
int avsr_bn_finalize(const float* part, int32_t nparts, int32_t C, int64_t count, float eps, float momentum, float* mean, float* invstd,
                     float* mov_mean, float* mov_var, const float* gamma, const float* beta, float* scale, float* shift, void* stream);
int avsr_bn_partials_f64(const float* part, int32_t nparts, int32_t C, double* out64, void* stream);
int avsr_bn_finalize_f64(const double* sums, int32_t C, float eps, float momentum, float* mean, float* invstd, float* mov_mean,
                         float* mov_var, const float* gamma, const float* beta, float* scale, float* shift, void* stream);
int avsr_bn_bwd_finalize_f64(const double* local, const double* global, int32_t C, const float* mean, const float* invstd,
                             const float* gamma, float* dgamma, float* dbeta, float grad_beta, float* k, void* stream);
int avsr_bn_eval_affine(const float* gamma, const float* beta, const float* mov_mean, const float* mov_var, float eps, float* scale,
                        float* shift, int32_t C, void* stream);
int avsr_batchnorm_apply(const float* x, float* y, int32_t rows, int32_t F, const float* gamma, const float* beta, const float* mean,
                         const float* invstd, int32_t relu, void* stream);
int avsr_conv3x3(const float* x, const float* w, const float* bias, float* y, int32_t N, int32_t H, int32_t W, int32_t Ci, int32_t Co,
                 int32_t stride, int32_t pad_t, int32_t pad_l, int32_t Ho, int32_t Wo, int32_t flip, float beta, void* stream);
int avsr_conv3x3_bwd_data_s2(const float* dy, const float* w, float* dx, int32_t N, int32_t H, int32_t W, int32_t Ci, int32_t Co,
                             int32_t pad_t, int32_t pad_l, int32_t Ho, int32_t Wo, float beta, void* stream);
int avsr_conv3x3_bwd_weight(const float* x, const float* dy, float* dw, int32_t N, int32_t H, int32_t W, int32_t Ci, int32_t Co,
                            int32_t stride, int32_t pad_t, int32_t pad_l, int32_t Ho, int32_t Wo, float beta, float* scratch,
                            int64_t scratch_floats, void* stream);
typedef struct avsr_conv3d_desc {
  int32_t B, T, H, W, Ci, Co;
  int32_t kt, kh, kw, stride;
  int32_t pad_f, pad_t, pad_l, Ho, Wo, relu;
  const float* scale;
  const float* shift;
} avsr_conv3d_desc;
int avsr_conv3d_supported(const avsr_conv3d_desc* c);
int64_t avsr_conv3d_wgrad_scratch_floats(const avsr_conv3d_desc* c);
int avsr_conv3d_fwd(const avsr_conv3d_desc* c, const float* x, const float* w, const float* res, const float* res_scale, const float* res_shift,
                    float* y, float* stats, int32_t* nparts, void* stream);
int avsr_conv3d_bwd_data(const avsr_conv3d_desc* c, const float* dy, const float* w, float* dx, float beta, void* stream);
int avsr_conv3d_bwd_weight(const avsr_conv3d_desc* c, const float* x, const float* dy, float* dw, float beta, float* scratch,
                           int64_t scratch_floats, void* stream);
int avsr_conv3d_bn_finalize(const float* part, int32_t nparts, int32_t C, int64_t count, float eps, float momentum, float* mean,
                            float* invstd, float* mov_mean, float* mov_var, const float* gamma, const float* beta, float* scale,
                            float* shift, void* stream);
typedef struct avsr_logmel_args {
  int32_t B, N, T_out, F;
  int32_t frame_length, frame_step, fft_length, num_mel_bins;
  int32_t window, stride, mel_nnz, pad_;
  const float* wav;
  const int32_t* wav_len;
  const float* hann;
  const float* twiddle;
  const int32_t* mel_lo;
  const int32_t* mel_cnt;
  const int32_t* mel_ptr;
  const float* mel_w;
  float* out;
  int32_t* out_len;
} avsr_logmel_args;
int avsr_logmel_supported(int32_t frame_length, int32_t fft_length, int32_t num_mel_bins, int32_t window, int32_t stride);
int avsr_logmel_fwd(const avsr_logmel_args* a, void* stream);
#define AVSR_SPEC_AUGMENT_MAX_MASKS 8
#define AVSR_SPEC_AUGMENT_MAX_T 65535
typedef struct avsr_spec_augment_args {
  int32_t B, T, F_in, F;
  int32_t freq_masks, freq_width, freq_bins, time_masks;
  int32_t time_width, ratio_q16, video, mean_fill;
  int64_t ld;
  const float* x;
  const int32_t* len;
  const int32_t* seed;
  float* y;
  float* ws;
  int64_t ws_floats;
} avsr_spec_augment_args;
int avsr_spec_augment_supported(int32_t B, int32_t T, int32_t F, int32_t freq_masks, int32_t time_masks);
int64_t avsr_spec_augment_ws_floats(int32_t B, int32_t T, int32_t F_in);
int avsr_spec_augment(const avsr_spec_augment_args* a, void* stream);
typedef struct avsr_ctc_args {
  int32_t B, T, L, C;
  int64_t ld;
  const float* z;
  const int32_t* labels;
  const int32_t* labels_len;
  const int32_t* in_len;
  const float* denom;
  float weight;
  int32_t pad_;
  float* nll;
  int32_t* status;
  float* utt_loss;
  float* dz;
  float* ws;
  int64_t ws_floats;
} avsr_ctc_args;
int avsr_ctc_loss(const avsr_ctc_args* a, void* stream);
int64_t avsr_ctc_ws_floats(int32_t B, int32_t T, int32_t L);
int avsr_ctc_best_path(const float* z, int64_t ld, const int32_t* in_len, int32_t B, int32_t T, int32_t C, int32_t* ids, void* stream);
int avsr_relu(const float* x, float* y, int64_t n, void* stream);
int avsr_relu_bwd(const float* y, const float* dy, float* dx, int64_t n, void* stream);
int avsr_add(const float* a, const float* b, float* out, int64_t n, void* stream);
int avsr_selu(const float* z, float* y, int64_t n, void* stream);
int avsr_selu_bwd(const float* z, const float* dy, float* dz, int64_t n, void* stream);

int avsr_batchnorm_xhat(const float* x, const float* mean, const float* invstd, float* xhat, int32_t rows, int32_t F,
                        void* stream);

int avsr_embed_labels(const float* emb, const int32_t* labels, int32_t go_id, float* out, int32_t* fed, int32_t B,
                      int32_t L, int32_t E, int32_t n_steps, void* stream);
int avsr_embed_grad(const float* dx, const int32_t* fed, float* demb, int32_t B, int32_t L, int32_t E, int32_t V,
                    float* scratch, int64_t scratch_floats, void* stream);

int avsr_dropout_rows(const avsr_mat* x, const avsr_mat* y, int32_t rows, int32_t cols, const int32_t* seed,
                      int32_t stream_id, float keep, int32_t idx_width, int32_t idx_coff, int32_t accumulate, void* stream);

int avsr_seq_loss(float* logits, const int32_t* labels, const int32_t* labels_len, float* denom,
                  int32_t compute_denom, float* row_loss, float* dlogits, int32_t B, int32_t L, int32_t V, void* stream);
int avsr_seq_loss_fun(float* logits, const int32_t* labels, const int32_t* labels_len, float* denom, int32_t compute_denom,
                      float* row_loss, float* dlogits, int32_t B, int32_t L, int32_t V, int32_t loss_fun,
                      float label_smoothing, void* stream);

int avsr_seq_loss_per_utterance(const float* row_loss, const int32_t* labels_len, const float* denom, float* out, int32_t B,
                                int32_t L, void* stream);
int avsr_instnorm_fwd(const float* x, float* y, int32_t B, int32_t T, int32_t F, const float* gamma, const float* beta,
                      float* mean_out, float* invstd_out, float eps, void* stream);
int avsr_instnorm_bwd(const float* x, const float* dy, const float* gamma, const float* mean, const float* invstd, float* dx,
                      float* dgamma_part, float* dbeta_part, int32_t B, int32_t T, int32_t F, void* stream);
int avsr_highway_fwd(const avsr_mat* x, const avsr_mat* h, const avsr_mat* carry_pre, const avsr_mat* y, const int32_t* len,
                     int32_t B, int32_t T, int32_t H, void* stream);
int avsr_highway_bwd(const avsr_mat* x, const avsr_mat* h, const avsr_mat* carry_pre, const avsr_mat* dy, const avsr_mat* dh,
                     const avsr_mat* dcarry_pre, const avsr_mat* dx, const int32_t* len, int32_t B, int32_t T, int32_t H,
                     int32_t accumulate_dx, void* stream);
int avsr_copy_words(void* dst, const void* src, int64_t n_words, void* stream);
int avsr_zero_words(void* dst, int64_t n_words, void* stream);
int avsr_zero_multi(void* const* ptrs, const int64_t* n_words, int32_t count, void* stream);
int avsr_add_int(const int32_t* a, int32_t b, int32_t* out, void* stream);
typedef struct avsr_colsum_job {
  avsr_mat a;
  avsr_mat b;
  float* out;
  int32_t rows, F;
  float alpha, beta;
} avsr_colsum_job;
int avsr_colsum_multi(const avsr_colsum_job* jobs, int32_t n, float* scratch, int64_t scratch_floats, void* stream);
int avsr_slab_defer_begin(void);
int avsr_slab_defer_end(void* stream);
int avsr_au_loss(const float* z, const float* aus, const int32_t* len, float* row_loss, float* dz, int32_t B, int32_t T,
                 float weight, void* stream);
int avsr_au_loss_dp(const float* z, const float* aus, const int32_t* len, float* row_loss, float* dz, int32_t B, int32_t T,
                    float weight, const float* total_count, void* stream);

int avsr_normed_v(const float* v, const float* g, float* vn, int32_t H, void* stream);
int avsr_normed_v_bwd(const float* v, const float* g, const float* dvn, float* dv, float* dg, int32_t H, void* stream);

int avsr_reduce_scalar(const float* part, int32_t n, float* out, int32_t do_sqrt, int32_t accumulate, float scale,
                       void* stream);

int avsr_l2_regularise(const int64_t* seg_off, const int64_t* seg_n, int32_t nseg, const float* params, float* grads,
                       float l2, float* loss_accum, float* scratch, void* stream);
int avsr_global_norm(const float* grads, int64_t n, float grad_scale, float* norm_out, float* scratch, void* stream);
int avsr_adam_step(float* params, float* grads, float* m, float* v, int64_t n, const float* global_norm, int32_t* step,
                   float lr, int32_t warmup_steps, float clip_norm, float grad_scale, void* stream);
int avsr_adam_step_decay(float* params, float* grads, float* m, float* v, int64_t n, const float* global_norm,
                         int32_t* step, float lr, int32_t warmup_steps, int32_t first_decay_steps, float clip_norm,
                         float grad_scale, void* stream);
int avsr_optimiser_step(float* params, float* grads, float* m, float* v, int64_t n, const float* global_norm, int32_t* step,
                        float lr, int32_t warmup_steps, int32_t first_decay_steps, float clip_norm, float grad_scale,
                        int32_t optimiser, float weight_decay, void* stream);

#define AVSR_PROF_NKIND 15
int avsr_prof_begin(int32_t max_launches);
int avsr_prof_end(int32_t* out_count, float* out_ms, double* out_flops);

#if defined(__GNUC__) || defined(__clang__)
#pragma GCC visibility pop
#endif
#ifdef __cplusplus
}
#endif
#endif
```

Measured before the change: 5692 utterances/sec.

## Add K-split 512-thread variant of generic MFMA conv kernel for deep layers

Adds a K-split form of the generic conv kernel in which pairs of waves split the channel/tap reduction in half. The partner wave hands its partial accumulator over through an LDS slot guarded by workgroup-scope atomic flags, and the wave that owns the tile runs the epilogue. The goal is to halve per-wave register pressure (weights and koff arrays) and double the waves per workgroup, so latency is hidden better on deep 64-channel stride-2 backward-data layers. The cost is spin-wait handoffs between waves, extra LDS use and smaller prefetch depth. It is gated by a heuristic (wmode==1, stride-2, Cs==64) and a global mode switch that defaults to on.

New measurement: 5709 utterances/sec (median of 4 runs). Within noise of the previous version (+0.3%).

```diff
diff --git a/avsr-tf1_amd/_lib.py b/avsr-tf1_amd/_lib.py
--- a/avsr-tf1_amd/_lib.py
+++ b/avsr-tf1_amd/_lib.py
@@ -230,6 +230,7 @@
     "avsr_attn_rnn_set_fused": [_i32],
     "avsr_attn_rnn_set_beam_kernel": [_i32],
     "avsr_conv_set_mfma": [_i32],
+    "avsr_conv_set_ksplit": [_i32],
     "avsr_conv_supported": [C.POINTER(ConvDesc)],
     "avsr_conv_fwd": [C.POINTER(ConvDesc), _vp, _vp, _vp, _vp, _vp, _vp, _vp, _vp, C.POINTER(_i32), _vp],
     "avsr_conv_bwd_data": [C.POINTER(ConvDesc), _vp, _vp, _vp, _f32, _vp],
diff --git a/avsr-tf1_amd/csrc/conv_mfma.h b/avsr-tf1_amd/csrc/conv_mfma.h
--- a/avsr-tf1_amd/csrc/conv_mfma.h
+++ b/avsr-tf1_amd/csrc/conv_mfma.h
@@ -45,6 +45,8 @@
 }
 
 #define CG_MAXTAP 16
+#define CG_KS_FLAGS 16
+#define CG_KS_LDS (CG_KS_FLAGS * 4 + 4 * 64 * 16)
 #define CONV_MAX_PARTS 512
 struct CGTap { int da, db; short w[4]; };
 static inline CGTap cgtap1(int da, int db, int widx) { CGTap t; t.da = da; t.db = db; t.w[0] = (short)widx; t.w[1] = t.w[2] = t.w[3] = -1; return t; }
@@ -84,6 +86,7 @@
 
 
 extern int g_conv_mfma;
+extern int g_conv_ksplit;
 
 struct ConvPlanRec { avsr_conv_launch* out; int cap, n; };
 extern thread_local ConvPlanRec* g_conv_plan;
diff --git a/avsr-tf1_amd/csrc/conv_mfma.hip b/avsr-tf1_amd/csrc/conv_mfma.hip
--- a/avsr-tf1_amd/csrc/conv_mfma.hip
+++ b/avsr-tf1_amd/csrc/conv_mfma.hip
@@ -2,17 +2,21 @@
 
 namespace avsr {
 
-template <int MAXCH, bool CH4, int EP>
-__global__ __launch_bounds__(256, 2) void conv_gen_kernel(const CGArgs A) {
+template <int MAXCH, bool CH4, int EP, bool KS = false>
+__global__ __launch_bounds__(KS ? 512 : 256, KS ? 4 : 2) void conv_gen_kernel(const CGArgs A) {
+  static_assert(!KS || (CH4 && MAXCH > 6), "the K-split form serves the deep 4-channel-multiple layers");
+  constexpr int NTHR = KS ? 512 : 256;
+  constexpr int HC = KS ? (MAXCH + 1) / 2 : MAXCH;
   extern __shared__ __attribute__((aligned(16))) float lds[];
   const int tid = threadIdx.x, lane = tid & 63, wave = __builtin_amdgcn_readfirstlane(tid >> 6);
+  const int pair = KS ? wave >> 1 : wave, kh = KS ? (wave ^ pair ^ (pair >> 1)) & 1 : 0;
   const int i = lane & 15, q = lane >> 4;
   const int Cs = A.Cs, CsL = A.CsL, CsP = A.CsP, Cd = A.Cd, C4 = CsL >> 2;
   const int PH = A.SH + 2, PW = A.SW + 2, fstride = PH * PW * CsP;
   const int KQ = A.ntap * C4, nch = (KQ + 3) >> 2;
   const int NC = A.nsp * Cd;
   const int NT = (NC + 15) >> 4;
-  const int nt = wave % NT, mslot = wave / NT, mstep = 4 / NT;
+  const int nt = pair % NT, mslot = pair / NT, mstep = 4 / NT;
   const f32x4 zero4 = {0.f, 0.f, 0.f, 0.f};
   const bool lin = A.lin != 0;
   const int opf = A.OA * A.OB;
@@ -23,9 +27,13 @@
   int* const taptab = dsttab + rows_pad;
   const int tapword = reinterpret_cast<const int*>(A.tap)[tid & (CG_MAXTAP * 4 - 1)];
 
-  for (int idx = tid; idx < A.F * fstride; idx += 256) lds[idx] = 0.f;
+  for (int idx = tid; idx < A.F * fstride; idx += NTHR) lds[idx] = 0.f;
   if (tid < CG_MAXTAP * 4) taptab[tid] = tapword;
-  for (int m = tid; m < rows_pad; m += 256) {
+  int* const ks_flag = taptab + CG_MAXTAP * 4;
+  float* const ks_slot = reinterpret_cast<float*>(ks_flag + CG_KS_FLAGS) + (pair * 64 + lane) * 4;
+  if (KS && tid < CG_KS_FLAGS) ks_flag[tid] = 0;
+  int ks_seq = 0;
+  for (int m = tid; m < rows_pad; m += NTHR) {
     int ro = 0, dt = 4;
     if (m < rows_all) {
       const int f = fdiv(m, A.m_opf), r = m - f * opf, a = fdiv(r, A.m_ob), b = r - a * A.OB;
@@ -40,19 +48,21 @@
 
   __syncthreads();
   const __amdgpu_buffer_rsrc_t w_rs = make_rsrc(A.w);
-  f32x4 wreg[MAXCH];
-  int koff[MAXCH];
+  f32x4 wreg[HC];
+  int koff[HC];
   {
     const int cn = nt * 16 + i;
     const bool colok = cn < NC;
     const int sp = colok ? cn / Cd : 0, co = colok ? cn - sp * Cd : 0;
 #pragma unroll
-    for (int c = 0; c < MAXCH; ++c) {
-      const int kq = 4 * c + q;
-      const bool in = c < nch && kq < KQ;
+    for (int c = 0; c < HC; ++c) {
+      const int cg = KS ? 2 * c + kh : c;
+      const int kq = 4 * cg + q;
+      const bool in = cg < nch && kq < KQ;
       const int t = in ? kq / C4 : 0, cs4 = in ? kq - t * C4 : 0;
       const i32x4_ tp = *reinterpret_cast<const i32x4_*>(taptab + 4 * t);
       koff[c] = in ? (tp[0] * PW + tp[1]) * CsP + cs4 * 4 : 0;
+      if (KS) koff[c] = __builtin_amdgcn_readfirstlane(in ? koff[c] - q * 4 : 0);
       const int wpair = (sp & 2) ? tp[3] : tp[2];
       const int widx = (int)(short)((sp & 1) ? (wpair >> 16) : (wpair & 0xffff));
       f32x4 wv;
@@ -84,17 +94,18 @@
   const int lane_o = lin ? cD0 * 4 : ((sdh * A.DW + sdw) * Cd + coD) * 4;
 
   const int st_rq = (A.SW * Cs) >> 2;
-  const int st_rpp = st_rq > 0 ? (256 / st_rq > 0 ? 256 / st_rq : 1) : 1;
+  const int st_rpp = st_rq > 0 ? (NTHR / st_rq > 0 ? NTHR / st_rq : 1) : 1;
   const int st_row = (st_rq > 0 && st_rq <= 256) ? (tid < st_rpp * st_rq ? fdiv(tid, A.m_rq) : -1) : -1;
   const int st_p4 = st_row >= 0 ? tid - st_row * st_rq : 0;
   const int st_px = (CH4 && CsP != Cs) ? (st_p4 * 4) / Cs : 0;
   const int st_lo = (CH4 && CsP != Cs) ? st_px * CsP + (st_p4 * 4 - st_px * Cs) : st_p4 * 4;
   f32x4 bsc = {1.f, 1.f, 1.f, 1.f}, bsh = zero4;
   const bool bn_on = CH4 && A.bn_sc != nullptr;
-  if (bn_on && st_row >= 0) { const int cb = (st_p4 * 4) % Cs; bsc = ld4(A.bn_sc + cb); bsh = ld4(A.bn_sh + cb); }
+  const int bn_cb = (bn_on && st_row >= 0) ? (st_p4 * 4) % Cs : 0;
+  if (!KS && bn_on && st_row >= 0) { bsc = ld4(A.bn_sc + bn_cb); bsh = ld4(A.bn_sh + bn_cb); }
   const int rowf = A.SW * Cs;
 
-  constexpr int PF = CH4 ? (MAXCH > 9 ? 10 : 12) : 4;
+  constexpr int PF = KS ? (MAXCH > 9 ? 4 : 6) : CH4 ? (MAXCH > 9 ? 10 : 12) : 4;
   f32x4 pre[PF];
   constexpr bool c4 = CH4;
   const int ppf = c4 ? (A.SH + st_rpp - 1) / st_rpp : 0;
@@ -120,13 +131,18 @@
       const int tot4 = (fcur * per3) >> 2;
 #pragma unroll
       for (int u = 0; u < PF; ++u) {
-        const int idx = u * 256 + tid;
+        const int idx = u * NTHR + tid;
         ldb4_hidden(pre[u], src_rs, idx < tot4 ? (int)(so + idx * 16u) : P_OOB);
       }
     }
   };
   auto commit = [&](int n0) {
     const int fcur = min(FP, n_end - n0);
+    if (KS && bn_on && st_row >= 0) {
+      int z = 0;
+      asm volatile("" : "+v"(z));
+      bsc = ld4(A.bn_sc + bn_cb + z); bsh = ld4(A.bn_sh + bn_cb + z);
+    }
     vm_wait_all();
 #pragma unroll
     for (int u = 0; u < PF; ++u) vm_landed(pre[u]);
@@ -151,11 +167,11 @@
       };
 #pragma unroll
       for (int u = 0; u < PF; ++u) {
-        const int idx = u * 256 + tid;
+        const int idx = u * NTHR + tid;
         if (idx < tot4) { put(idx * 4, pre[u][0]); put(idx * 4 + 1, pre[u][1]); put(idx * 4 + 2, pre[u][2]); put(idx * 4 + 3, pre[u][3]); }
       }
       const float* sp = A.src + (long)n0 * per3;
-      for (int e = tot4 * 4 + tid; e < tot; e += 256) put(e, sp[e]);
+      for (int e = tot4 * 4 + tid; e < tot; e += NTHR) put(e, sp[e]);
     }
   };
   int n0 = n_begin;
@@ -168,8 +184,8 @@
     if (n0 + n_step < n_end) fetch(n0 + n_step);
     const int Mtot = fcur * opf, mtiles = (Mtot + 15) >> 4;
     const unsigned pass_o = (unsigned)((long)n0 * pixf * Cd * 4);
-    constexpr int CB = MAXCH <= 6 ? MAXCH : 3;
-    constexpr bool XT = MAXCH <= 6;
+    constexpr int CB = HC <= 6 && !KS ? HC : 3;
+    constexpr bool XT = MAXCH <= 6 && !KS;
     f32x4 bufa[CB], bufb[CB];
     const int last = mtiles - 1;
     int rb_cur = rowtab[(mslot < mtiles ? mslot : 0) * 16 + i];
@@ -204,26 +220,32 @@
       return (int)(pass_o + (unsigned)((dt & ~15) + lane_o)) | (ok ? 0 : P_OOB);
     };
     auto tile = [&](f32x4 (&cur)[CB], f32x4 (&nxt)[CB], const int mt) {
+      if (KS) { rb_cur = rowtab[mt * 16 + i]; dt_cur = dsttab[mt * 16 + i]; }
       const int t1 = mt + mstep < mtiles ? mt + mstep : last;
-      const int dt_nxt = dsttab[t1 * 16 + i];
-      const float* base = lds + rb_cur;
+      const int dt_nxt = KS ? 0 : dsttab[t1 * 16 + i];
+      const float* base = lds + rb_cur + (KS ? q * 4 : 0);
       bool ok;
       const int dbo = dest(mt, dt_cur, ok);
       f32x4 ev = zero4, ov = zero4;
-      if (EP & 1) ev = ldb4(e_rs, dbo);
-      if (EP & 2) ov = ldb4(acc_rs, dbo);
+      const int ebo = KS ? dbo | (kh ? P_OOB : 0) : dbo;
+      if (EP & 1) ev = ldb4(e_rs, ebo);
+      if (EP & 2) ov = ldb4(acc_rs, ebo);
       f32x4 acc0 = zero4, acc1 = zero4;
-#pragma unroll
-      for (int c = 0; c < CB; ++c) cur[c] = ld4(base + koff[c]);
-#pragma unroll
-      for (int b0 = 0; b0 < MAXCH; b0 += CB) {
+      if (!KS) {
+#pragma unroll
+        for (int c = 0; c < CB; ++c) cur[c] = ld4(base + koff[c]);
+      }
+#pragma unroll
+      for (int b0 = 0; b0 < HC; b0 += CB) {
+#pragma unroll
+        for (int c = 0; c < CB; ++c) {
+          if (KS) { if (b0 + c < HC) cur[c] = ld4(base + koff[b0 + c]); }
+          else if (b0 + CB + c < HC) nxt[c] = ld4(base + koff[b0 + CB + c]);
+        }
+        __builtin_amdgcn_sched_barrier(0);
 #pragma unroll
         for (int c = 0; c < CB; ++c)
-          if (b0 + CB + c < MAXCH) nxt[c] = ld4(base + koff[b0 + CB + c]);
-        __builtin_amdgcn_sched_barrier(0);
-#pragma unroll
-        for (int c = 0; c < CB; ++c)
-          if (b0 + c < MAXCH) {
+          if (b0 + c < HC) {
 #pragma unroll
             for (int e = 0; e < 4; ++e) {
               if (e & 1) acc1 = __builtin_amdgcn_mfma_f32_16x16x4f32(wreg[b0 + c][e], cur[c][e], acc1, 0, 0, 0);
@@ -232,13 +254,30 @@
             }
           }
         __builtin_amdgcn_sched_barrier(0);
-#pragma unroll
-        for (int c = 0; c < CB; ++c) cur[c] = nxt[c];
-      }
-      epilogue(acc0, acc1, dbo, ok, ev, ov);
-      rb_cur = rb_nxt;
-      rb_nxt = rowtab[(mt + 2 * mstep < mtiles ? mt + 2 * mstep : last) * 16 + i];
-      dt_cur = dt_nxt;
+        if (!KS) {
+#pragma unroll
+          for (int c = 0; c < CB; ++c) cur[c] = nxt[c];
+        }
+      }
+      if constexpr (KS) {
+        ++ks_seq;
+        const f32x4 part = acc0 + acc1;
+        if (kh) {
+          while (__hip_atomic_load(ks_flag + 4 + pair, __ATOMIC_ACQUIRE, __HIP_MEMORY_SCOPE_WORKGROUP) < ks_seq - 1) {}
+          st4(ks_slot, part);
+          __hip_atomic_store(ks_flag + pair, ks_seq, __ATOMIC_RELEASE, __HIP_MEMORY_SCOPE_WORKGROUP);
+        } else {
+          while (__hip_atomic_load(ks_flag + pair, __ATOMIC_ACQUIRE, __HIP_MEMORY_SCOPE_WORKGROUP) < ks_seq) {}
+          const f32x4 other = ld4(ks_slot);
+          __hip_atomic_store(ks_flag + 4 + pair, ks_seq, __ATOMIC_RELEASE, __HIP_MEMORY_SCOPE_WORKGROUP);
+          epilogue(part, other, dbo, ok, ev, ov);
+        }
+      } else epilogue(acc0, acc1, dbo, ok, ev, ov);
+      if (!KS) {
+        rb_cur = rb_nxt;
+        rb_nxt = rowtab[(mt + 2 * mstep < mtiles ? mt + 2 * mstep : last) * 16 + i];
+        dt_cur = dt_nxt;
+      }
     };
     f32x4 pa0 = zero4, pa1 = zero4, pev = zero4, pov = zero4;
     int pdbo = P_OOB, poki = 0;
@@ -311,9 +350,9 @@
 #pragma unroll
     for (int r = 0; r < 4; ++r) { ssum[r] = group16_sum(ssum[r]); ssq[r] = group16_sum(ssq[r]); }
     float* red = lds;
-    if (i == 0) {
-#pragma unroll
-      for (int r = 0; r < 4; ++r) { red[((wave * 4 + q) * 2) * 4 + r] = ssum[r]; red[((wave * 4 + q) * 2 + 1) * 4 + r] = ssq[r]; }
+    if (i == 0 && kh == 0) {
+#pragma unroll
+      for (int r = 0; r < 4; ++r) { red[((pair * 4 + q) * 2) * 4 + r] = ssum[r]; red[((pair * 4 + q) * 2 + 1) * 4 + r] = ssq[r]; }
     }
     __syncthreads();
     if (tid < Cd) {
@@ -553,6 +592,7 @@
 }
 
 int g_conv_mfma = 1;
+int g_conv_ksplit = 1;
 thread_local ConvPlanRec* g_conv_plan = nullptr;
 
 }
@@ -560,6 +600,11 @@
 using namespace avsr;
 
 extern "C" int avsr_conv_set_mfma(int32_t on) { g_conv_mfma = on ? 1 : 0; return AVSR_OK; }
+extern "C" int avsr_conv_set_ksplit(int32_t mode) {
+  if (mode < 0 || mode > 2) return AVSR_ERR_ARG;
+  g_conv_ksplit = mode;
+  return AVSR_OK;
+}
 
 static bool cg_q4_ok(const CGArgs& A, int ntaps) {
   return A.Cd == 8 && A.S == 1 && A.OS == 1 && !A.oh0 && !A.ow0 && A.DH == A.OA && A.DW == A.OB && ntaps == 9 &&
@@ -570,14 +615,14 @@
     if (A.tap[t].db != (A.wmode ? 1 - t % 3 : t % 3 - 1)) return false;
   return true;
 }
-static int cg_dry(const CGArgs& A, int kernel, int m, int c4t, int grid, size_t lds) {
+static int cg_dry(const CGArgs& A, int kernel, int m, int c4t, int grid, size_t lds, int waves = 4) {
   if (!g_conv_plan) return grid;
   if (A.res && A.bnb_x) return AVSR_ERR_ARG;
   const int ep = ((A.res || A.bnb_x) ? 1 : 0) | (A.beta != 0.f ? 2 : 0);
   if (A.Cs % 4 && ep) return AVSR_ERR_UNSUPPORTED;
   avsr_conv_launch L = {};
   L.kernel = kernel; L.m = m; L.ntc = c4t; L.ch4 = A.Cs % 4 == 0; L.ep = ep; L.nsp = A.nsp; L.ntap = A.ntap; L.F = A.F; L.grid = grid;
-  L.CsP = kernel == 0 ? A.CsP : A.CsL; L.lds_bytes = (int32_t)lds;
+  L.CsP = kernel == 0 ? A.CsP : A.CsL; L.lds_bytes = (int32_t)lds; L.pad_ = waves;
   conv_plan_note(L);
   return grid;
 }
@@ -634,6 +679,9 @@
   return grid;
 }
 
+static bool cg_ksplit_built(int inst, int ep) { return inst == 9 || (inst == 18 && ep != 3) || (inst == 20 && !(ep & 1)); }
+static bool cg_ksplit_pays(const CGArgs& A) { return A.wmode == 1 && A.nsp == 1 && A.OS == 2 && A.Cs == 64; }
+
 static int cg_launch(CGArgs& A, hipStream_t s, int kind, double flops, bool dry = false) {
   if (A.nsp == 0) {
     A.nsp = 1; A.SB = A.S; A.OSA = A.OS; A.OSB = A.OS;
@@ -644,58 +692,70 @@
   const int NT = (A.nsp * A.Cd + 15) / 16;
   if (!(NT == 1 || NT == 2 || NT == 4) || nch > 20) return AVSR_ERR_UNSUPPORTED;
   if (A.Cs % 4 && nch > 5) return AVSR_ERR_UNSUPPORTED;
-  int Fcap = 16;
   if (A.Cs % 4 == 0) {
     const int rq = A.SW * A.Cs / 4;
     if (rq > 256 || rq < 1) return AVSR_ERR_UNSUPPORTED;
-    const int rpp = 256 / rq, pfmax = nch > 9 ? 10 : 12;
-    Fcap = pfmax / ((A.SH + rpp - 1) / rpp);
     A.m_rq = fmagic(rq); A.m_per = fmagic(A.SH * rq); A.m_sw = fmagic(A.SW);
   } else {
-    Fcap = (4 * 256 * 4) / (A.SH * A.SW * A.Cs);
-    while (Fcap > 0 && (long)Fcap * A.SH * A.SW * A.Cs >= 65536) --Fcap;
     A.m_rq = fmagic(A.Cs); A.m_per = fmagic(A.SH * A.SW * A.Cs); A.m_sw = fmagic(A.SW);
   }
-  if (Fcap < 1) return AVSR_ERR_UNSUPPORTED;
   if ((long)A.N * A.DH * A.DW * A.Cd * 4 >= (1L << 31)) return AVSR_ERR_UNSUPPORTED;
   if ((long)A.N * A.SH * A.SW * A.Cs * 4 >= (1L << 31)) return AVSR_ERR_UNSUPPORTED;
   A.m_opf = fmagic(A.OA * A.OB); A.m_ob = fmagic(A.OB);
   const int opf = A.OA * A.OB, mstep = 4 / NT;
-  A.CsP = A.CsL;
-  if (A.Cs % 4 == 0) {
-    for (int p = 0; p < 4; ++p)
-      if ((A.SB * (A.CsL / 4 + p)) % 4 == 2) { A.CsP = A.CsL + 4 * p; break; }
-  }
-  size_t frame_b = sizeof(float) * (size_t)(A.SH + 2) * (A.SW + 2) * A.CsP;
-  auto lds_bytes = [&](int F) {
-    const size_t rows_pad = (((size_t)F * opf + 15) / 16) * 16;
-    return F * frame_b + 4 * rows_pad * 2 + sizeof(CGTap) * CG_MAXTAP;
+  const int inst = A.Cs % 4 ? 5 : (nch <= 2 ? 2 : (nch <= 6 ? 6 : (nch <= 9 ? 9 : (nch <= 18 ? 18 : 20))));
+  size_t lds = 0;
+  auto plan = [&](const bool ks) {
+    int Fcap = 16;
+    if (A.Cs % 4 == 0) {
+      const int rq = A.SW * A.Cs / 4;
+      const int rpp = (ks ? 512 : 256) / rq, pfmax = ks ? (inst > 9 ? 4 : 6) : (nch > 9 ? 10 : 12);
+      Fcap = pfmax / ((A.SH + rpp - 1) / rpp);
+    } else {
+      Fcap = (4 * 256 * 4) / (A.SH * A.SW * A.Cs);
+      while (Fcap > 0 && (long)Fcap * A.SH * A.SW * A.Cs >= 65536) --Fcap;
+    }
+    if (Fcap < 1) return 0;
+    A.CsP = A.CsL;
+    if (A.Cs % 4 == 0) {
+      for (int p = 0; p < 4; ++p)
+        if ((A.SB * (A.CsL / 4 + p)) % 4 == 2) { A.CsP = A.CsL + 4 * p; break; }
+    }
+    size_t frame_b = sizeof(float) * (size_t)(A.SH + 2) * (A.SW + 2) * A.CsP;
+    auto lds_bytes = [&](int F) {
+      const size_t rows_pad = (((size_t)F * opf + 15) / 16) * 16;
+      return F * frame_b + 4 * rows_pad * 2 + sizeof(CGTap) * CG_MAXTAP + (ks ? CG_KS_LDS : 0);
+    };
+    auto pick = [&](size_t budget, int slots) {
+      double best = -1.0;
+      int bestF = 0;
+      for (int F = (Fcap < 16 ? Fcap : 16); F >= 1; --F) {
+        if (lds_bytes(F) > budget || (long)F * opf >= 65536) continue;
+        const long units = (A.N + F - 1) / F, grid = units < slots ? units : slots;
+        const long cnt = (A.N + grid - 1) / grid, np = (cnt + F - 1) / F, fp = (cnt + np - 1) / np;
+        const long tiles = (fp * opf + 15) / 16, per_wave = (tiles + mstep - 1) / mstep;
+        const double cost = (double)np * (double)(per_wave * 8 + 16);
+        if (best < 0.0 || cost < 0.97 * best) { best = cost; bestF = F; }
+      }
+      return bestF;
+    };
+    A.F = pick(64 * 1024, CONV_MAX_PARTS);
+    if (!A.F && A.CsP != A.CsL) {
+      A.CsP = A.CsL;
+      frame_b = sizeof(float) * (size_t)(A.SH + 2) * (A.SW + 2) * A.CsP;
+      A.F = pick(64 * 1024, CONV_MAX_PARTS);
+    }
+    lds = A.F ? lds_bytes(A.F) : 0;
+    return A.F;
   };
-  auto pick = [&](size_t budget, int slots) {
-    double best = -1.0;
-    int bestF = 0;
-    for (int F = (Fcap < 16 ? Fcap : 16); F >= 1; --F) {
-      if (lds_bytes(F) > budget || (long)F * opf >= 65536) continue;
-      const long units = (A.N + F - 1) / F, grid = units < slots ? units : slots;
-      const long cnt = (A.N + grid - 1) / grid, np = (cnt + F - 1) / F, fp = (cnt + np - 1) / np;
-      const long tiles = (fp * opf + 15) / 16, per_wave = (tiles + mstep - 1) / mstep;
-      const double cost = (double)np * (double)(per_wave * 8 + 16);
-      if (best < 0.0 || cost < 0.97 * best) { best = cost; bestF = F; }
-    }
-    return bestF;
-  };
-  A.F = pick(64 * 1024, CONV_MAX_PARTS);
-  if (!A.F && A.CsP != A.CsL) {
-    A.CsP = A.CsL;
-    frame_b = sizeof(float) * (size_t)(A.SH + 2) * (A.SW + 2) * A.CsP;
-    A.F = pick(64 * 1024, CONV_MAX_PARTS);
-  }
-  if (!A.F) return AVSR_ERR_UNSUPPORTED;
-  size_t lds = lds_bytes(A.F);
+  const int ep_ks = ((A.res || A.bnb_x) ? 1 : 0) | (A.beta != 0.f ? 2 : 0);
+  bool ks = g_conv_ksplit && A.Cs % 16 == 0 && cg_ksplit_built(inst, ep_ks) && (g_conv_ksplit == 2 || cg_ksplit_pays(A));
+  if (ks && !plan(true)) ks = false;
+  if (!ks && !plan(false)) return AVSR_ERR_UNSUPPORTED;
   if (lds < sizeof(float) * 4 * 4 * 2 * 4) lds = sizeof(float) * 4 * 4 * 2 * 4;
   int grid = (A.N + A.F - 1) / A.F;
   if (grid > CONV_MAX_PARTS) grid = CONV_MAX_PARTS;
-  if (dry) return cg_dry(A, 0, A.Cs % 4 ? 5 : (nch <= 2 ? 2 : (nch <= 6 ? 6 : (nch <= 9 ? 9 : (nch <= 18 ? 18 : 20)))), 0, grid, lds);
+  if (dry) return cg_dry(A, 0, inst, 0, grid, lds, ks ? 8 : 4);
   ProfScope ps(kind, s, flops);
   const bool emap = A.res != nullptr || A.bnb_x != nullptr;
   if (A.res && A.bnb_x) return AVSR_ERR_ARG;
@@ -705,6 +765,17 @@
   {                                                                                                                 \
     hipLaunchKernelGGL((conv_gen_kernel<M_, C_, E_>), dim3(grid), dim3(256), lds, s, A);                            \
   }
+#define CG_KS(M_, E_)                                                                                               \
+  {                                                                                                                 \
+    hipLaunchKernelGGL((conv_gen_kernel<M_, true, E_, true>), dim3(grid), dim3(512), lds, s, A);                    \
+  }
+#define CG_GO_KS(M_)                                                                                               \
+  switch (ep) {                                                                                                    \
+    case 0: CG_KS(M_, 0) break;                                                                                    \
+    case 1: CG_KS(M_, 1) break;                                                                                    \
+    case 2: CG_KS(M_, 2) break;                                                                                    \
+    default: CG_KS(M_, 3) break;                                                                                   \
+  }
 #define CG_GO(M_, C_)                                                                                              \
   switch (ep) {                                                                                                    \
     case 0: CG_ONE(M_, C_, 0) break;                                                                               \
@@ -712,13 +783,25 @@
     case 2: CG_ONE(M_, C_, 2) break;                                                                               \
     default: CG_ONE(M_, C_, 3) break;                                                                              \
   }
-  if (A.Cs % 4) CG_ONE(5, false, 0)
+  if (ks) {
+    if (inst == 9) { CG_GO_KS(9) }
+    else if (inst == 18) switch (ep) {
+      case 0: CG_KS(18, 0) break;
+      case 1: CG_KS(18, 1) break;
+      default: CG_KS(18, 2) break;
+    }
+    else if (ep == 0) CG_KS(20, 0)
+    else CG_KS(20, 2)
+  }
+  else if (A.Cs % 4) CG_ONE(5, false, 0)
   else if (nch <= 2) { CG_GO(2, true) }
   else if (nch <= 6) { CG_GO(6, true) }
   else if (nch <= 9) { CG_GO(9, true) }
   else if (nch <= 18) { CG_GO(18, true) }
   else if (nch <= 20) { CG_GO(20, true) }
   else return AVSR_ERR_UNSUPPORTED;
+#undef CG_GO_KS
+#undef CG_KS
 #undef CG_GO
 #undef CG_ONE
   if (hipGetLastError() != hipSuccess) return AVSR_ERR_HIP;
diff --git a/avsr-tf1_amd/csrc/conv_wgrad.hip b/avsr-tf1_amd/csrc/conv_wgrad.hip
--- a/avsr-tf1_amd/csrc/conv_wgrad.hip
+++ b/avsr-tf1_amd/csrc/conv_wgrad.hip
@@ -301,7 +301,7 @@
   if (!g_conv_plan) return;
   avsr_conv_launch L = {};
   L.kernel = 2; L.m = m; L.ntc = ntc; L.ch4 = A.Ci % 4 == 0; L.rs = rs; L.fold = fold; L.nsp = nsp; L.ntap = A.nt; L.t0 = A.t0; L.F = A.F;
-  L.grid = grid; L.CsP = A.CiL + A.pad; L.lds_bytes = (int32_t)lds; L.slab = A.slab;
+  L.grid = grid; L.CsP = A.CiL + A.pad; L.lds_bytes = (int32_t)lds; L.slab = A.slab; L.pad_ = 4;
   conv_plan_note(L);
 }
 
diff --git a/avsr-tf1_amd/ops.py b/avsr-tf1_amd/ops.py
--- a/avsr-tf1_amd/ops.py
+++ b/avsr-tf1_amd/ops.py
@@ -643,6 +643,10 @@
     check(_L().avsr_conv_set_mfma(int(on)), "avsr_conv_set_mfma")
 
 
+def conv_set_ksplit(mode):
+    check(_L().avsr_conv_set_ksplit(int(mode)), "avsr_conv_set_ksplit")
+
+
 def conv_desc(N, H, W, Ci, Co, k, stride, pad_t, pad_l, Ho, Wo, bn=None):
     from ._lib import ConvDesc
     d = ConvDesc(N, H, W, Ci, Co, k, stride, pad_t, pad_l, Ho, Wo, 0, None, None)
@@ -738,7 +742,7 @@
     if n < 0:
         check(n, "avsr_conv_plan")
     assert n <= cap
-    return [{f: getattr(out[i], f) for f, _ in ConvLaunch._fields_ if f != "pad_"} for i in range(n)]
+    return [{("waves" if f == "pad_" else f): getattr(out[i], f) for f, _ in ConvLaunch._fields_} for i in range(n)]
 
 
 def slab_defer_begin():
diff --git a/include/avsr_hip.h b/include/avsr_hip.h
--- a/include/avsr_hip.h
+++ b/include/avsr_hip.h
@@ -426,6 +426,7 @@
                 int32_t pad_t, int32_t pad_l, int32_t Ho, int32_t Wo, float beta, void* stream);
 int avsr_conv3x3_supported(int32_t Ci, int32_t Co, int32_t H, int32_t W);
 int avsr_conv_set_mfma(int32_t on);
+int avsr_conv_set_ksplit(int32_t mode);
 typedef struct avsr_conv_desc {
   int32_t N, H, W, Ci, Co, k, stride, pad_t, pad_l, Ho, Wo, pad_;
   const float* bn_scale;
```
